# z-prize/2022-entries

Hardware: AMD Instinct MI355X
Metric: BLS12-377 G1 MSM point-scalar pairs/s (higher is better)
Workload: dtype u32

## Files before the change

### 2022-entries_amd/csrc/host_test_api.cpp

```cpp
#include <stdint.h>
#include <stdio.h>

static long g_check_failures = 0;
static char g_first_failure[256];
static void msm_check_fail(const char* file, int line, const char* cond) {
  if (g_check_failures++ == 0) snprintf(g_first_failure, sizeof g_first_failure, "%s:%d %s", file, line, cond);
}
#define MSM_CHECK(cond) do { if (!(cond)) msm_check_fail(__FILE__, __LINE__, #cond); } while (0)
#define MSM_CHECK_COL_BEGIN() unsigned __int128 chk_col_ = col
#define MSM_CHECK_COL_ADD(x) chk_col_ += (x)
#define MSM_CHECK_COL_END(col) MSM_CHECK(chk_col_ == (unsigned __int128)(col))

#include "host_curve.hpp"
#include "te.hpp"

using namespace msm;

template <class F>
static void t_fe_mul(const uint8_t* a, const uint8_t* b, uint8_t* out) {
  Modulus<F> md;
  Fe x, y, z;
  uint32_t wa[12], wb[12], wo[12];
  memcpy(wa, a, 48);
  memcpy(wb, b, 48);
// ... 2498 lines not shown
}
}

#include "expr.hpp"

template <class FR>
static int t_expr(unsigned flags, const uint32_t* nodes, uint64_t n_nodes, const uint8_t* consts, uint64_t n_consts, uint64_t n_chal, uint64_t n_cols,
                  const uint8_t* const* cols, const uint64_t* lens, uint64_t len, uint64_t rot_step, const uint8_t* challenges, uint8_t* out, uint64_t* info,
                  char* msg, uint64_t msg_len) {
  const bool normal = (flags & kExprNormal) != 0;
  ExprProgram pr;
  if (!expr_check_dag(nodes, n_nodes, n_consts, n_chal, n_cols, msg, msg_len)) return -1;
  const bool ok = expr_compile(pr, nodes, n_nodes, n_consts, n_chal, n_cols, expr_store_limit<FR>(), msg, msg_len);
  if (info) {
    info[0] = pr.n_nodes;
    info[1] = pr.ninstr();
    info[2] = pr.slots;
    info[3] = pr.products;
    info[4] = pr.reduces;
    info[5] = expr_lds_bytes(pr.slots);
    info[6] = pr.used_cols;
    info[7] = pr.rot0_only;
  }
  if (!ok) return -1;
  if (!out || len == 0) return 0;
  for (uint64_t j = 0; j < n_cols; j++)
    if (lens[j] == 0 || len % lens[j]) return -3;
  std::vector<uint32_t> cw(n_consts * 8 + 1), hw(n_chal * 8 + 1), dst(len * 8), slots((size_t)pr.slots * 8 + 1);
  std::vector<std::vector<uint32_t>> colw(n_cols);
  auto words = [&](uint32_t* w8, const uint8_t* b32) {
    Fr x;
    uint32_t w[8];
    poly_scalar<FR>(x, b32, normal);
    fr_pack(w, x);
    memcpy(w8, w, 32);
  };
  for (uint64_t k = 0; k < n_consts; k++) words(cw.data() + k * 8, consts + k * 32);
  for (uint64_t k = 0; k < n_chal; k++) words(hw.data() + k * 8, challenges + k * 32);
  for (uint64_t j = 0; j < n_cols; j++) {
    colw[j].resize(lens[j] * 8);
    memcpy(colw[j].data(), cols[j], lens[j] * 32);
  }
  std::vector<ExprColRef> refs(pr.refs.size() + 1);
  for (size_t k = 0; k < pr.refs.size(); k++)
    refs[k] = ExprColRef{colw[pr.refs[k].first].data(), (uint32_t)lens[pr.refs[k].first], expr_shift(pr.refs[k].second, rot_step, len)};
  ExprRun p{};
  p.prog = pr.code.data();
  p.refs = refs.data();
  p.consts = cw.data();
  p.chals = hw.data();
  p.out = dst.data();
  p.ninstr = pr.ninstr();
  p.len = (uint32_t)len;
  p.normal = normal ? 1u : 0u;
  const ExprSlots<1> st{slots.data()};
  for (uint64_t i = 0; i < len; i++) expr_row<FR>(st, p, (uint32_t)i);
  memcpy(out, dst.data(), len * 32);
  return 0;
}

extern "C" {
int ht_expr(int field, unsigned flags, const uint32_t* nodes, uint64_t n_nodes, const uint8_t* consts, uint64_t n_consts, uint64_t n_chal, uint64_t n_cols,
            const uint8_t* const* cols, const uint64_t* lens, uint64_t len, uint64_t rot_step, const uint8_t* challenges, uint8_t* out, uint64_t* info,
            char* msg, uint64_t msg_len) {
  if ((flags & ~kExprNormal) || !nodes || !msg || msg_len < 64 || len > ((uint64_t)1 << 22) || (n_consts && !consts)) return -2;
  if (out && len && ((n_cols && (!cols || !lens)) || (n_chal && !challenges))) return -2;
  msg[0] = 0;
  return POLY_FIELD(t_expr, flags, nodes, n_nodes, consts, n_consts, n_chal, n_cols, cols, lens, len, rot_step, challenges, out, info, msg, msg_len);
}
unsigned ht_expr_max_slots(void) { return EXPR_MAX_SLOTS; }
}

#include "seg_msm.hpp"

template <class C>
static int t_sm_segments(const uint8_t* points, size_t stride, const uint8_t* scalars, const uint64_t* offsets, size_t nseg, uint64_t shared_len, uint32_t c,
                         uint32_t tile, unsigned flags, uint8_t* out, size_t out_stride) {
  using E = typename C::E;
  using El = typename E::T;
  typename E::Md md;
  std::vector<XyzzDevT<El>> res(nseg);
  std::vector<uint32_t> sc;
  for (size_t s = 0; s < nseg; s++) {
    uint64_t p0, s0, len;
    sm_segment_span(p0, s0, len, offsets, s, shared_len, 0);
    if (len == 0) {
      xyzz_set_inf<E>(res[s].p);
      continue;
    }
    sc.resize(8 * len);
    memcpy(sc.data(), scalars + 32 * s0, 32 * len);
    sm_serial_segment<E>(res[s].p, points + p0 * stride, stride, sc.data(), len, c ? c : sm_window_for(len), tile, (flags & 1) != 0, md);
  }
  pm_host_output<E>(res, (flags & 8) ? 2u : 0u, out, out_stride, md);
  return 0;
}

extern "C" {
int ht_sm_digits(const uint8_t* scalar, int c, int32_t* out, int32_t* out_mem) {
  if (!scalar || !out || !out_mem || c < 1 || c > (int)SM_MAX_WINDOW) return -1;
  uint32_t s[8];
  memcpy(s, scalar, 32);
  const uint32_t nd = sm_digits((uint32_t)c);
  for (uint32_t j = 0; j < nd; j++) {
    out[j] = sm_digit(s, j, (uint32_t)c);
    out_mem[j] = sm_digit_mem(s, j, (uint32_t)c);
  }
  return (int)nd;
}
int ht_sm_segments(int curve, const uint8_t* points, size_t stride, const uint8_t* scalars, const uint64_t* offsets, size_t nseg, uint64_t shared_len, int c,
                   int tile, unsigned flags, uint8_t* out, size_t out_stride) {
  if ((flags & ~13u) || c < 0 || c > (int)SM_MAX_WINDOW || tile < (int)SM_MIN_TILE || (tile & (tile - 1)) || out_stride % 4 || (nseg && !out)) return -1;
  if (((flags & 4) != 0) != (offsets == nullptr)) return -1;
  DISPATCH_C(curve, t_sm_segments, points, stride, scalars, offsets, nseg, shared_len, (uint32_t)c, (uint32_t)tile, flags, out, out_stride)
}
long ht_sm_plan(const uint64_t* offsets, size_t nseg, uint64_t shared_len, int force_c, int tile_opt, size_t max_segs, size_t work_limit, size_t xyzz_bytes,
                size_t el_bytes, uint64_t* classes, size_t max_classes, uint32_t* ids, size_t max_ids, uint64_t* chunk_bounds, size_t max_chunks,
                uint64_t* summary) {
  if (force_c < 0 || force_c > (int)SM_MAX_WINDOW || !classes || !ids || !summary || !chunk_bounds) return -1;
  SmPlan plan;
  sm_plan(plan, offsets, nseg, shared_len, (uint32_t)force_c, (uint32_t)tile_opt, max_segs, work_limit, xyzz_bytes, el_bytes);
  if (!plan.fits) return -2;
  size_t nc = 0, ni = 0;
  if (plan.chunks.size() > max_chunks) return -1;
  for (size_t k = 0; k < plan.chunks.size(); k++) {
    const SmChunk& ch = plan.chunks[k];
    chunk_bounds[3 * k] = ch.s0;
    chunk_bounds[3 * k + 1] = ch.s1;
    chunk_bounds[3 * k + 2] = ch.work_bytes;
    if (ni + ch.ids.size() > max_ids) return -1;
    for (const SmClass& cl : ch.classes) {
      if (nc >= max_classes) return -1;
      const uint64_t row[11] = {k, ch.s0, ch.s1, cl.c, cl.nwin, cl.tile, cl.nseg, ni + cl.ids_at, cl.wsum_at, ch.work_bytes, ch.wsum_records};
      memcpy(classes + 11 * nc++, row, sizeof row);
    }
    if (!ch.ids.empty()) memcpy(ids + ni, ch.ids.data(), 4 * ch.ids.size());
    ni += ch.ids.size();
  }
  summary[0] = plan.chunks.size();
  summary[1] = plan.max_segs;
  summary[2] = plan.max_wsum_records;
  return (long)nc;
}
int ht_sm_geometry(int c, int tile_opt, uint64_t maxlen, int xyzz_words, uint32_t* out) {
  if (c < 1 || c > (int)SM_MAX_WINDOW || !out) return -1;
  out[0] = sm_slices((uint32_t)c);
  out[1] = sm_block_threads((uint32_t)c);
  out[3] = sm_tile_for((uint32_t)c, (uint32_t)tile_opt, maxlen);
  out[2] = sm_lds_words((uint32_t)c, out[3], (uint32_t)xyzz_words);
  return 0;
}
int ht_sm_window_for(uint64_t len) { return (int)sm_window_for(len); }
}
```

### 2022-entries_amd/csrc/launch.hpp

```cpp
#pragma once
#include <hip/hip_runtime.h>

#include "host_curve.hpp"
#include "msm_types.hpp"
#include "partition_plan.hpp"
#include "te.hpp"

namespace msm {

template <class E>
struct SwLaw;
template <class F>
struct TeLaw;
template <class F, int NB>
struct SwPairLaw;

template <class G>
struct LawMem;
template <class E>
struct LawMem<SwLaw<E>> {
  using MemT = typename E::T;
  using BaseDev = AffineDevT<MemT>;
};
template <class F>
struct LawMem<TeLaw<F>> {
  using MemT = Fe;
  using BaseDev = TeAffineDev;
};
template <class F, int NB>
struct LawMem<SwPairLaw<F, NB>> {
  using MemT = Fe2;
  using BaseDev = AffineDevT<Fe2>;
};

template <class G>
struct PairedForm {
  using L = G;
};
template <class F, int NB>
struct PairedForm<SwLaw<Fp2El<F, NB>>> {
  using L = SwPairLaw<F, NB>;
};

template <class G>
struct WalkLaunch {
  using El = typename LawMem<G>::MemT;
  using BaseDev = typename LawMem<G>::BaseDev;
  static hipError_t accumulate(const uint2* entries, const uint32_t* n_real, uint32_t K, const BaseDev* bases, SegOutT<El> out, uint32_t nlanes,
                               uint32_t* flags, hipStream_t st);
  static hipError_t sum_bases(const BaseDev* bases, const uint8_t* inf, uint32_t first, uint32_t n, uint32_t per_lane, SegOutT<El> out, uint32_t nlanes,
                              uint32_t* flags, hipStream_t st);
  static hipError_t segreduce(const XyzzDevT<El>* in_slots, const uint32_t* in_keys, uint32_t n_in, uint32_t K, SegOutT<El> out, uint32_t nlanes,
                              uint32_t quad_limit, uint32_t* flags, hipStream_t st);
  static hipError_t bucket_reduce(bool first, const XyzzDevT<El>* in_a, const XyzzDevT<El>* in_x, uint32_t n_per_win, uint32_t L, uint32_t chunks,
                                  uint32_t windows, uint32_t out_stride, XyzzDevT<El>* out_a, XyzzDevT<El>* out_x, uint32_t* flags, hipStream_t st,
                                  uint32_t run_win = 0xffffffffu);
  static hipError_t reduce_scan_step(const XyzzDevT<El>* in, const XyzzDevT<El>* in2, XyzzDevT<El>* out, uint32_t nb, uint32_t windows, uint32_t d,
                                     uint32_t mode, uint32_t quad_limit, uint32_t* flags, hipStream_t st);
  static hipError_t bucket_merge(XyzzDevT<El>* total, const XyzzDevT<El>* part, uint32_t n, uint32_t* flags, hipStream_t st);
};

template <class E>
struct Launch {
  using El = typename E::T;
  static hipError_t convert_bases(const uint8_t* in, size_t stride, uint32_t n, bool serialized, AffineDevT<El>* out, uint8_t* inf,
                                  hipStream_t st);
  static hipError_t pre_double(const AffineDevT<El>* in, const uint8_t* inf_in, uint32_t n, uint32_t c, XyzzDevT<El>* out, hipStream_t st);
  static hipError_t pre_normalize(const XyzzDevT<El>* in, uint32_t n, uint32_t J, El* prefix, AffineDevT<El>* out, uint8_t* inf_out,
                                  hipStream_t st);
  static hipError_t check_points(const uint8_t* in, size_t stride, uint32_t n, bool serialized, bool exact, uint8_t* status, hipStream_t st);
};

struct LaunchTe {
  static constexpr uint32_t kDefaultQuadLimit = 1u << 18;
  static hipError_t convert(const AffineDev* in, const uint8_t* inf, uint32_t n, uint32_t J, Fe* prefix, TeAffineDev* out, uint32_t* flags,
                            hipStream_t st);
};

struct PartLaunch {
  static int run(int scalar_field, int scalar_mode, const uint32_t* d_scalars, const uint8_t* d_inf, const PartPlan& p, const PartBuffers& b,
                 hipStream_t st, hipEvent_t mid, hipError_t& err);
  static hipError_t debug_finish(const PartPlan& p, const PartBuffers& b, const uint32_t* slot_keys, uint32_t nslots, hipStream_t st, char* what,
                                 size_t what_len, uint64_t* checks_done);
};

extern template struct Launch<Bls12_377_G1::E>;
extern template struct Launch<Bls12_381_G1::E>;
extern template struct Launch<Bls12_377_G2::E>;
extern template struct Launch<Bls12_381_G2::E>;

}
```

### 2022-entries_amd/csrc/launch_impl.hpp

```cpp
#pragma once
#include <type_traits>
#include "launch.hpp"
#include "msm_kernels.hpp"

namespace msm {

inline uint32_t launch_blocks(uint64_t n) { return (uint32_t)((n + 255) / 256); }

template <class E>
hipError_t Launch<E>::convert_bases(const uint8_t* in, size_t stride, uint32_t n, bool serialized, AffineDevT<El>* out, uint8_t* inf,
                                    hipStream_t st) {
  if (serialized)
    hipLaunchKernelGGL((k_convert_bases<E, true>), dim3(launch_blocks(n)), dim3(256), 0, st, in, stride, n, out, inf);
  else
    hipLaunchKernelGGL((k_convert_bases<E, false>), dim3(launch_blocks(n)), dim3(256), 0, st, in, stride, n, out, inf);
  return hipGetLastError();
}

template <class E>
hipError_t Launch<E>::pre_double(const AffineDevT<El>* in, const uint8_t* inf_in, uint32_t n, uint32_t c, XyzzDevT<El>* out, hipStream_t st) {
  hipLaunchKernelGGL((k_pre_double<E>), dim3(launch_blocks(n)), dim3(256), 0, st, in, inf_in, n, c, out);
  return hipGetLastError();
}

template <class E>
hipError_t Launch<E>::pre_normalize(const XyzzDevT<El>* in, uint32_t n, uint32_t J, El* prefix, AffineDevT<El>* out, uint8_t* inf_out,
                                    hipStream_t st) {
  hipLaunchKernelGGL((k_pre_normalize<E>), dim3(launch_blocks(((uint64_t)n + J - 1) / J)), dim3(256), 0, st, in, n, J, prefix, out, inf_out);
  return hipGetLastError();
}

template <class G>
struct QuadOf {
  using Q = void;
};
template <class E>
struct QuadOf<SwLaw<E>> {
  using Q = SwQuad<E>;
};
template <class F>
struct QuadOf<TeLaw<F>> {
  using Q = TeQuad<F>;
};
template <class G>
inline constexpr bool kHasQuad = !std::is_void_v<typename QuadOf<G>::Q>;

template <class G>
inline constexpr bool kIsSwLaw = false;
template <class E>
inline constexpr bool kIsSwLaw<SwLaw<E>> = true;

template <class G>
uint32_t walk_blocks(uint64_t walkers) {
  static_assert(std::is_same_v<typename LawMem<G>::MemT, typename G::MemT> && std::is_same_v<typename LawMem<G>::BaseDev, typename G::BaseDev>,
                "LawMem (launch.hpp) restates the law's memory types");
  return launch_blocks(G::LANES * walkers);
}

template <class G>
hipError_t WalkLaunch<G>::accumulate(const uint2* entries, const uint32_t* n_real, uint32_t K, const BaseDev* bases, SegOutT<El> out, uint32_t nlanes,
                                     uint32_t* flags, hipStream_t st) {
#ifndef MSM_GATHER
#define MSM_GATHER 2
#endif
  if constexpr (MSM_GATHER == 2 || !kIsSwLaw<G>)
    hipLaunchKernelGGL((k_accumulate_glds<G>), dim3(walk_blocks<G>(nlanes)), dim3(256), 0, st, entries, n_real, K, bases, out, nlanes, flags);
  else
    hipLaunchKernelGGL((k_accumulate<G>), dim3(walk_blocks<G>(nlanes)), dim3(256), 0, st, entries, n_real, K, bases, out, nlanes, flags);
  return hipGetLastError();
}

template <class G>
hipError_t WalkLaunch<G>::sum_bases(const BaseDev* bases, const uint8_t* inf, uint32_t first, uint32_t n, uint32_t per_lane, SegOutT<El> out,
                                    uint32_t nlanes, uint32_t* flags, hipStream_t st) {
  if constexpr (G::LANES != 1) {
    return hipErrorNotSupported;
  } else {
    hipLaunchKernelGGL((k_sum_bases<G>), dim3(walk_blocks<G>(nlanes)), dim3(256), 0, st, bases, inf, first, n, per_lane, out, nlanes, flags);
    return hipGetLastError();
  }
}

template <class G>
hipError_t WalkLaunch<G>::segreduce(const XyzzDevT<El>* in_slots, const uint32_t* in_keys, uint32_t n_in, uint32_t K, SegOutT<El> out, uint32_t nlanes,
                                    uint32_t quad_limit, uint32_t* flags, hipStream_t st) {
  if constexpr (kHasQuad<G>) {
    if (nlanes <= quad_limit) {
      hipLaunchKernelGGL((k_segreduce_quad<typename QuadOf<G>::Q>), dim3(launch_blocks(4ull * nlanes)), dim3(256), 0, st, in_slots, in_keys, n_in, K, out,
                         nlanes, flags);
      return hipGetLastError();
    }
  }
  hipLaunchKernelGGL((k_segreduce<G>), dim3(walk_blocks<G>(nlanes)), dim3(256), 0, st, in_slots, in_keys, n_in, K, out, nlanes, flags);
  return hipGetLastError();
}

template <class G>
hipError_t WalkLaunch<G>::bucket_reduce(bool first, const XyzzDevT<El>* in_a, const XyzzDevT<El>* in_x, uint32_t n_per_win, uint32_t L, uint32_t chunks,
                                        uint32_t windows, uint32_t out_stride, XyzzDevT<El>* out_a, XyzzDevT<El>* out_x, uint32_t* flags, hipStream_t st,
                                        uint32_t run_win) {
  dim3 grid(walk_blocks<G>((uint64_t)windows * chunks));
  if (first)
    hipLaunchKernelGGL((k_bucket_reduce<G, true>), grid, dim3(256), 0, st, in_a, in_x, n_per_win, L, chunks, windows, out_stride, out_a, out_x, flags, run_win);
  else
    hipLaunchKernelGGL((k_bucket_reduce<G, false>), grid, dim3(256), 0, st, in_a, in_x, n_per_win, L, chunks, windows, out_stride, out_a, out_x, flags, run_win);
  return hipGetLastError();
}

template <class G>
hipError_t WalkLaunch<G>::reduce_scan_step(const XyzzDevT<El>* in, const XyzzDevT<El>* in2, XyzzDevT<El>* out, uint32_t nb, uint32_t windows, uint32_t d,
                                           uint32_t mode, uint32_t quad_limit, uint32_t* flags, hipStream_t st) {
  const uint64_t threads = (uint64_t)windows * (mode == 1 ? d : nb);
  if constexpr (kHasQuad<G>) {
    if (threads <= quad_limit) {
      hipLaunchKernelGGL((k_reduce_scan_step_quad<typename QuadOf<G>::Q>), dim3(launch_blocks(4 * threads)), dim3(256), 0, st, in, in2, out, nb, windows, d,
                         mode, flags);
      return hipGetLastError();
    }
  }
  hipLaunchKernelGGL((k_reduce_scan_step<G>), dim3(walk_blocks<G>(threads)), dim3(256), 0, st, in, in2, out, nb, windows, d, mode, flags);
  return hipGetLastError();
}

template <class G>
hipError_t WalkLaunch<G>::bucket_merge(XyzzDevT<El>* total, const XyzzDevT<El>* part, uint32_t n, uint32_t* flags, hipStream_t st) {
  if constexpr (G::CARRY_IN) {
    return hipErrorNotSupported;
  } else {
    hipLaunchKernelGGL((k_bucket_merge<G>), dim3(walk_blocks<G>(n)), dim3(256), 0, st, total, part, n, flags);
    return hipGetLastError();
  }
}

#define MSM_INSTANTIATE_SW_LAUNCHERS(E)                                                                                                          \
  using A_ = AffineDevT<E::T>;                                                                                                                   \
  using X_ = XyzzDevT<E::T>;                                                                                                                     \
  using S_ = SegOutT<E::T>;                                                                                                                      \
  using W_ = WalkLaunch<SwLaw<E>>;                                                                                                               \
  template hipError_t Launch<E>::convert_bases(const uint8_t*, size_t, uint32_t, bool, A_*, uint8_t*, hipStream_t);                              \
  template hipError_t W_::accumulate(const uint2*, const uint32_t*, uint32_t, const A_*, S_, uint32_t, uint32_t*, hipStream_t);                  \
  template hipError_t W_::segreduce(const X_*, const uint32_t*, uint32_t, uint32_t, S_, uint32_t, uint32_t, uint32_t*, hipStream_t);             \
  template hipError_t Launch<E>::pre_double(const A_*, const uint8_t*, uint32_t, uint32_t, X_*, hipStream_t);                                    \
  template hipError_t Launch<E>::pre_normalize(const X_*, uint32_t, uint32_t, E::T*, A_*, uint8_t*, hipStream_t);                                \
  template hipError_t W_::bucket_reduce(bool, const X_*, const X_*, uint32_t, uint32_t, uint32_t, uint32_t, uint32_t, X_*, X_*, uint32_t*, hipStream_t, uint32_t); \
  template hipError_t W_::reduce_scan_step(const X_*, const X_*, X_*, uint32_t, uint32_t, uint32_t, uint32_t, uint32_t, uint32_t*, hipStream_t); \
  template hipError_t W_::bucket_merge(X_*, const X_*, uint32_t, uint32_t*, hipStream_t);                                                        \
  template hipError_t W_::sum_bases(const A_*, const uint8_t*, uint32_t, uint32_t, uint32_t, S_, uint32_t, uint32_t*, hipStream_t);

}
```

### 2022-entries_amd/csrc/msm_engine.hip

```cpp
#include <hip/hip_runtime.h>

#include <algorithm>
#include <cstdarg>
#include <cstdio>
#include <cstdlib>
#include <cstring>
#include <string.h>
#include <strings.h>

#include <dlfcn.h>

#include <chrono>
#include <condition_variable>
#include <deque>
#include <functional>
#include <memory>
#include <mutex>
#include <stdexcept>
#include <thread>
#include <type_traits>
#include <string>
#include <vector>

#include "../../include/mi355_msm.h"
// ... 116 lines not shown
      if (e == hipSuccess) {
        e = hipMemMap(g->va, g->mapped, 0, g->handle, 0);
        if (e == hipSuccess) {
          hipMemAccessDesc acc{};
          acc.location = prop.location;
          acc.flags = hipMemAccessFlagsProtReadWrite;
          e = hipMemSetAccess(g->va, g->mapped, &acc, 1);
          if (e != hipSuccess) (void)hipMemUnmap(g->va, g->mapped);
        }
        if (e != hipSuccess) (void)hipMemRelease(g->handle);
      }
      if (e != hipSuccess) (void)hipMemAddressFree(g->va, g->va_bytes);
    }
    if (e != hipSuccess) {
      delete g;
      return e;
    }
    guard = g;
    p = (char*)g->va + (g->mapped - used);
    return hipSuccess;
  }
  void reserve(size_t need) {
    if (need <= bytes) return;
    release();
    hipError_t e = guard_tail_mode() ? guarded_alloc(need) : hipMalloc(&p, need);
    if (e == hipErrorOutOfMemory) {
      (void)hipGetLastError();
      if (reclaim_idle_device_memory()) e = guard_tail_mode() ? guarded_alloc(need) : hipMalloc(&p, need);
    }
    if (e != hipSuccess) {
      p = nullptr;
      (void)hipGetLastError();
      char buf[256];
      snprintf(buf, sizeof buf, "hipMalloc of %zu MiB failed: %s", need >> 20, hipGetErrorString(e));
      throw HipFailure((int)e, buf);
    }
    bytes = need;
  }
  void release() {
    if (guard) {
      (void)hipMemUnmap(guard->va, guard->mapped);
      (void)hipMemRelease(guard->handle);
      delete guard;
      guard = nullptr;
    } else if (p) {
      (void)hipFree(p);
    }
    p = nullptr;
    bytes = 0;
  }
  template <class T>
  T* as() const { return reinterpret_cast<T*>(p); }
};

struct ScratchBuf : private DevBuf {
  using DevBuf::as;
  using DevBuf::bytes;
  using DevBuf::p;
  using DevBuf::reserve;
  ScratchBuf() = default;
  explicit ScratchBuf(hipStream_t st) : stream(st), in_flight(true) {}
  ScratchBuf(const ScratchBuf&) = delete;
  ScratchBuf& operator=(const ScratchBuf&) = delete;
  ~ScratchBuf() {
    if (!p) return;
    if (in_flight) (void)hipStreamSynchronize(stream);
    release();
  }
  DevBuf detach() {
    const DevBuf b = *this;
    p = nullptr;
    bytes = 0;
    guard = nullptr;
    return b;
  }

 private:
  hipStream_t stream = nullptr;
  bool in_flight = false;
};

inline uint32_t ceil_div(uint64_t a, uint64_t b) { return (uint32_t)((a + b - 1) / b); }
inline uint32_t ilog2_floor(uint64_t v) { uint32_t r = 0; while (v >>= 1) r++; return r; }

constexpr uint32_t kNoAnchor = 0xffffffffu;
void eff_windows(int scalar_bits, int c, double& plain, double& anchored) {
  const int full = scalar_bits / c, rem = scalar_bits - full * c;
  const double q = scalar_bits == 253 ? 0.857 : 0.552;
  const double top_clear = rem == 0 ? 1.0 : std::min(1.0, q * std::ldexp(1.0, 1 - rem));
  plain = full + (rem == 0 ? 1.0 - q : 1.0 - 0.5 * top_clear);
  anchored = full + (1.0 - top_clear);
}
uint32_t anchor_window(int c, int scalar_bits, bool always = false) {
  const int full = scalar_bits / c;
  if (full < 1) return kNoAnchor;
  double plain, anchored;
  eff_windows(scalar_bits, c, plain, anchored);
  return (always || (plain - anchored) >= 0.01 * plain) ? (uint32_t)(full - 1) : kNoAnchor;
}

bool anchor_wide_fits(uint32_t anchor, int c, int scalar_bits) {
  if (anchor == kNoAnchor) return false;
  return scalar_bits - (int)(anchor + 1) * c == 1 && (257 + c - 1) / c == (int)anchor + 2;
}
double wide_eff_windows(uint32_t anchor, int c) { return (double)(anchor + 1) * (1.0 - std::ldexp(1.0, -c)); }

int choose_window_bits(size_t n, int scalar_bits, bool shared_buckets, bool fold = false, int levels = 0, int anchor_min_c = 0, bool anchor_wide = false) {
  if (!shared_buckets && n > ((size_t)1 << 12)) {
    if (n < ((size_t)3 << 14)) return 8;
    if (n < ((size_t)3 << (scalar_bits > 253 ? 16 : 17))) return 11;
  }
  const int free_wins = shared_buckets ? (257 + choose_window_bits(n, scalar_bits, false, fold) - 1) / choose_window_bits(n, scalar_bits, false, fold) : 0;
  int best = 2;
  double best_cost = 1e300;
  for (int c = 2; c <= (shared_buckets ? 24 : 23); c++) {
    if (shared_buckets && c < 24 && (257 + c - 1) / c >= free_wins) continue;
    if (shared_buckets && c == 22) continue;
    const int bits = (fold && n >= ((size_t)1 << 25)) ? scalar_bits - 1 : scalar_bits;
    const int full = bits / c, rem = bits - full * c;
    double eff = full + (rem >= 2 ? 1.0 : (bits != scalar_bits && rem == 0 ? (scalar_bits == 253 ? 0.145 : 0.448) : 0.55));
    if (anchor_min_c > 0 && !fold && c >= anchor_min_c && anchor_window(c, scalar_bits) != kNoAnchor) {
      double plain;
      eff_windows(scalar_bits, c, plain, eff);
      if (anchor_wide && !shared_buckets && anchor_wide_fits(anchor_window(c, scalar_bits), c, scalar_bits)) eff = wide_eff_windows(anchor_window(c, scalar_bits), c);
    }
    const int wins = (257 + c - 1) / c;
    const double alloc = shared_buckets ? (double)(levels > 0 ? (wins + std::min(levels, wins) - 1) / std::min(levels, wins) : 1) : (double)wins;
    const double group = c >= 22 ? 0.06 : 0.0;
    const double cost = (eff + group * wins) * (double)n * 10.0 + alloc * (double)(1ull << (c - 1)) * 50.0;
    if (cost < best_cost) { best_cost = cost; best = c; }
  }
  return best;
}

struct TableShape {
  uint32_t c, levels, bsets;
};
TableShape table_shape(size_t n, int scalar_bits, long opt_window_bits, int want_levels) {
  TableShape t{};
  t.c = opt_window_bits ? (uint32_t)opt_window_bits : (uint32_t)choose_window_bits(n, scalar_bits, true, false, want_levels);
  const uint32_t all_windows = (257 + t.c - 1) / t.c;
  t.levels = want_levels > 0 ? std::min<uint32_t>((uint32_t)want_levels, all_windows) : all_windows;
  t.bsets = ceil_div(all_windows, t.levels);
  t.levels = ceil_div(all_windows, t.bsets);
  return t;
}

struct Plan {
  uint32_t c, windows, half, keybits;
  uint32_t bucket_windows;
  uint32_t levels;
  uint32_t anchor;
  bool wide;
  uint64_t entries;
  uint32_t K, nlanes;
  uint32_t segK;
  uint32_t logL0, logL;
  uint32_t T0;
  uint32_t L0;
  uint32_t scan_nb;
  bool reduce_scan;
  bool scan_direct;
};

}

#ifndef MSM_G2_PAIRED_DEFAULT
#define MSM_G2_PAIRED_DEFAULT 31
#endif
constexpr long kDefaultG2Paired = MSM_G2_PAIRED_DEFAULT;

struct RcclState;

struct mi355_msm_ctx {
  int curve = 0;
  int device = 0;
  hipStream_t own_stream = nullptr;
  hipStream_t copy_stream = nullptr;
  struct AsyncWorker* async = nullptr;
  hipEvent_t copy_ev[9] = {};
  size_t nbases = 0;
  DevBuf bases, inf;
  DevBuf stateless_raw[3];
  DevBuf scalars, entries[2], buckets, slots[2], slot_keys[2], red_a[2], red_x[2];
  DevBuf carry_buckets;
  std::vector<hipEvent_t> carry_ev;
  long opt_first_piece_div = 0;
  long opt_carry = 1;
  DevBuf part_matrix, part_partial, part_segs[2], part_subjobs, part_counts, part_totals;
  void* pinned = nullptr;
  size_t pinned_bytes = 0;
  hipEvent_t ev[8] = {};
  long opt_window_bits = 0, opt_lane_entries = 0, opt_max_chunk = 0, opt_seg_entries = 0, opt_scalars_montgomery = 0, opt_reduce_scan_log = 0;
  long opt_scalars_to_montgomery = 0;
  long opt_precompute = 0;
  long opt_table_levels = 0;
  long opt_validate_bases = 0;
  bool bases_validated = false;
  long opt_codec_chunk = 0;
  DevBuf codec_in, codec_out, codec_stat[2];
  long opt_mul_chunk = 0, opt_mul_window = 0;
  DevBuf pm_stage, pm_rec, pm_prefix, pm_inf;
  DevBuf pm_points, pm_scalars, pm_out;
  hipEvent_t pm_ev[2] = {nullptr, nullptr};
  uint64_t last_mul_us = 0, last_mul_device_us = 0;
  long opt_seg_window = 0, opt_seg_tile = 0, opt_seg_chunk = 0;
  DevBuf sg_wsum, sg_stage, sg_prefix, sg_ids, sg_offs;
  DevBuf sg_points, sg_scalars, sg_out;
  hipEvent_t sg_ev[2] = {nullptr, nullptr};
  uint64_t last_segments_us = 0, last_segments_device_us = 0;
  long opt_fft_points_chunk = 0;
  DevBuf gf_stage, gf_rec, gf_prefix, gf_inf;
  DevBuf gf_vec[2];
  DevBuf gf_points, gf_out;
  hipEvent_t gf_ev[2] = {nullptr, nullptr};
  uint64_t last_fft_points_us = 0, last_fft_points_device_us = 0;
  long opt_assume_subgroup = 0;
  long opt_anchor = 1;
  bool anchor_armed = false;
  struct AnchorSum {
    size_t n;
    int shift;
    std::vector<uint8_t> pt;
  };
  std::vector<AnchorSum> anchor_sums;
  uint64_t anchor_sums_computed = 0;
  float anchor_sum_ms = 0;
  uint32_t last_anchor = kNoAnchor;
  long opt_anchor_wide = 1;
  bool wide_suppress = false;
  bool wide_overflowed = false;
  bool wide_off = false;
  uint32_t wide_streak = 0;
  uint64_t wide_fallbacks = 0, wide_demotions = 0;
  bool last_wide = false;
  DevBuf wide_flag, wide_r;
  uint32_t* h_wide_flag = nullptr;
  long opt_reduce_log_chunk = 0, opt_reduce_log_chunk0 = 0;
  long opt_reduce_scan = -1;
  long opt_reduce_fill = 0;
  long opt_twisted_edwards = 1;
  DevBuf te_bases, flags;
  uint32_t* h_flags = nullptr;
  bool te_active = false;
  bool sw_level0_only = false;
  uint64_t te_fallbacks = 0;
  uint32_t te_fallback_streak = 0;
  uint64_t te_demotions = 0;
  uint64_t oom_backoffs = 0;
  uint64_t peer_stagings = 0;
  long opt_force_peer_staging = 0;
  uint32_t last_bucket_windows = 0, last_l1_bits = 0, last_l1_bins = 0, last_passes = 0;
  uint32_t last_reduce_path = 0, last_reduce_chunks = 0, last_reduce_row = 0;
  uint32_t auto_levels = 0;
  uint64_t debug_checks = 0;
  size_t chunk_cap = 0;
  size_t fitted_chunk = 0;
  bool fitted_tables = false;
  uint32_t fitted_c = 0;
  long opt_mem_limit = 0;
  long inject_alloc_failures = 0;
  uint32_t quad_limit = LaunchTe::kDefaultQuadLimit;
  long opt_g2_paired = kDefaultG2Paired;
  std::vector<mi355_msm_ctx*> shards;
  std::vector<size_t> shard_lo;
  long opt_combine = 0;
  RcclState* rccl = nullptr;
  uint64_t rccl_exchanges = 0;
  uint32_t pre_c = 0, pre_windows = 0;
  bool bases_serialized = false;
  float last_ms[MI355_T_COUNT] = {};
  uint64_t last_info[8] = {};

  int scalar_bits() const { return (curve == MI355_BLS12_381_G1 || curve == MI355_BLS12_381_G2) ? 255 : 253; }
  int anchor_min_c() const { return curve == MI355_BLS12_381_G1 ? 2 : 21; }
  bool anchor_wanted(size_t n_batch) const {
    return opt_anchor != 0 && opt_carry != 0 && opt_assume_subgroup == 0 && n_batch >= (opt_anchor == 2 ? (size_t)1 : (size_t)1 << 20);
  }
  bool wide_wanted() const { return opt_anchor_wide != 0 && !wide_off && !wide_suppress; }

  Plan plan(size_t n, bool use_tables = true, uint32_t force_c = 0) const {
    Plan p{};
    const bool tables = pre_c && use_tables;
    if (tables)
      p.c = pre_c;
    else if (force_c)
      p.c = force_c;
    else
      p.c = (opt_window_bits && !pre_c) ? (uint32_t)opt_window_bits
                                        : (uint32_t)choose_window_bits(n, scalar_bits(), false, opt_assume_subgroup != 0, 0, anchor_wanted(n) ? anchor_min_c() : 0, wide_wanted());
    p.anchor = anchor_armed ? anchor_window((int)p.c, scalar_bits(), opt_anchor == 2) : kNoAnchor;
    p.wide = wide_wanted() && !tables && anchor_wide_fits(p.anchor, (int)p.c, scalar_bits());
    p.windows = (257 + p.c - 1) / p.c;
    p.levels = tables ? std::min<uint32_t>(pre_windows, p.windows) : 1;
    p.bucket_windows = ceil_div(p.windows, p.levels);
    p.levels = ceil_div(p.windows, p.bucket_windows);
    p.half = 1u << (p.c - 1);
    p.keybits = ilog2_floor(p.bucket_windows * p.half) + 1;
    p.entries = (uint64_t)p.windows * n;
    const uint64_t k_auto = std::max<uint64_t>({p.entries >= (3u << 20) ? 24u : (p.entries < (1u << 18) ? 4u : 8u), p.entries >> 20, std::min<uint64_t>(64, p.entries >> 19)});
    uint32_t K = opt_lane_entries ? (uint32_t)opt_lane_entries : (uint32_t)std::min<uint64_t>(512, k_auto);
    if (!opt_lane_entries && !opt_assume_subgroup && K >= 64) {
      K = (K + 7) & ~7u;
      double plain, anchored;
      eff_windows(scalar_bits(), (int)p.c, plain, anchored);
      const bool anchor_expected = (anchor_armed || anchor_wanted(n)) && anchor_window((int)p.c, scalar_bits(), opt_anchor == 2) != kNoAnchor;
      const uint32_t a_expected = anchor_expected ? anchor_window((int)p.c, scalar_bits(), opt_anchor == 2) : kNoAnchor;
      const bool wide_expected = wide_wanted() && !tables && anchor_wide_fits(a_expected, (int)p.c, scalar_bits());
      const double adds = (wide_expected ? wide_eff_windows(a_expected, (int)p.c) : anchor_expected ? anchored : plain) * (double)n;
      const double per_group = ((curve == MI355_BLS12_377_G2 || curve == MI355_BLS12_381_G2) && (opt_g2_paired & 1) ? 128.0 : 256.0) * 256.0;
      auto fill = [&](long k) {
        const double g = adds / ((double)k * per_group);
        return g / std::ceil(g);
      };
      if (adds / ((double)K * per_group) >= 6.0) {
        long best = (long)K;
        double best_fill = fill(best);
        for (long step = 8; step <= 96 && best_fill < 0.985; step += 8)
          for (long k : {(long)K - step, (long)K + step})
            if (k >= 64 && fill(k) > best_fill + 0.004) {
              best = k;
              best_fill = fill(k);
            }
        K = (uint32_t)best;
      }
    }
    p.K = K >= 8 ? (K + 7) & ~7u : (K + 3) & ~3u;
    p.nlanes = ceil_div(p.entries, p.K);
    p.segK = opt_seg_entries >= 4 ? (uint32_t)opt_seg_entries : (p.entries < (2u << 20) ? 4 : 8);
    uint64_t nb = (uint64_t)p.bucket_windows * p.half;
    uint32_t l0 = nb > (1u << 18) ? ilog2_floor(nb >> 18) : 0;
    p.logL0 = std::min<uint32_t>(7, std::max<uint32_t>(2, l0));
    p.logL = 2;
    if (opt_reduce_log_chunk) p.logL0 = p.logL = (uint32_t)opt_reduce_log_chunk;
    if (opt_reduce_log_chunk0) p.logL0 = (uint32_t)opt_reduce_log_chunk0;
    p.logL0 = std::min<uint32_t>(p.logL0, p.c - 1 ? p.c - 1 : 1);
    p.reduce_scan = opt_reduce_scan != 0;
    const uint32_t scan_log = opt_reduce_scan_log ? (uint32_t)opt_reduce_scan_log : 12;
    p.scan_direct = p.reduce_scan && p.half <= (1u << scan_log);
    if (p.reduce_scan && !p.scan_direct) {
      const uint32_t need = ilog2_floor(p.half) - scan_log;
      if (need > 9 || (need > 8 && p.bucket_windows < 8))
        p.reduce_scan = false;
      else if (p.logL0 < need)
        p.logL0 = need;
    }
    p.L0 = 1u << p.logL0;
    p.T0 = ceil_div(p.half, p.L0);
    p.scan_nb = p.T0;
    if (p.reduce_scan && !p.scan_direct && !opt_reduce_log_chunk && !opt_reduce_log_chunk0) {
      const uint64_t kSimds = 1024;
      const uint64_t fill = opt_reduce_fill > 0 ? (uint64_t)opt_reduce_fill : 1;
      const uint64_t waves = ((uint64_t)p.bucket_windows * p.T0 + 63) / 64;
      if (waves < fill * kSimds && p.T0 >= 1024) {
        const uint32_t t_fit = (uint32_t)(fill * kSimds * 64 / p.bucket_windows);
        if (t_fit > p.T0 && t_fit < 2 * fill * p.T0) {
          const uint32_t L = ceil_div(p.half, t_fit);
          if (L >= 8 && L < p.L0) {
            p.L0 = L;
            p.T0 = ceil_div(p.half, L);
            while (p.scan_nb < p.T0) p.scan_nb *= 2;
          }
        }
      }
    }
    return p;
  }
};

namespace {

void ensure_device(mi355_msm_ctx* ctx) { HIP_OK(hipSetDevice(ctx->device)); }

uint32_t pmul_window(const mi355_msm_ctx* ctx);
size_t pmul_chunk(const mi355_msm_ctx* ctx);
size_t gfft_chunk(const mi355_msm_ctx* ctx);

int require_device() {
  int count = 0;
  hipError_t e = hipGetDeviceCount(&count);
  if (e != hipSuccess || count == 0) {
    (void)hipGetLastError();
    throw HipFailure((int)(e != hipSuccess ? e : hipErrorNoDevice), "mi355_msm: no HIP device visible (this library has no CPU fallback)");
  }
  return count;
}

hipStream_t create_copy_stream() {
  hipStream_t s = nullptr;
  int least = 0, greatest = 0;
  if (hipDeviceGetStreamPriorityRange(&least, &greatest) == hipSuccess && greatest < least &&
      hipStreamCreateWithPriority(&s, hipStreamNonBlocking, greatest) == hipSuccess)
    return s;
  (void)hipGetLastError();
  HIP_OK(hipStreamCreateWithFlags(&s, hipStreamNonBlocking));
  return s;
}

uint64_t work_bytes(const Plan& p, uint64_t el, bool carry = false) {
  const PartPlan pp = part_plan((uint32_t)(p.entries / p.windows), p.c, p.windows, p.levels, 0, 0);
  const PartScratchSizes ps = part_scratch_sizes(pp);
  return p.entries * 16 + ps.matrix + ps.partial + ps.segs_a + ps.segs_b + ps.subjob_first + ps.counts + ps.totals +
         (uint64_t)p.bucket_windows * p.half * 224 * el * (carry ? 2 : 1) + 2 * (2ull * p.nlanes) * (224 * el + 4) + (p.scan_direct ? (uint64_t)p.bucket_windows * p.half : 4ull * (p.bucket_windows + (p.wide ? 1 : 0)) * p.scan_nb) * 224 * el;
}

DevBuf* const* work_buffers(mi355_msm_ctx* ctx, size_t& count) {
  static thread_local DevBuf* bufs[24];
  DevBuf* list[] = {&ctx->entries[0], &ctx->entries[1], &ctx->part_matrix, &ctx->part_partial, &ctx->part_segs[0], &ctx->part_segs[1],
                    &ctx->part_subjobs, &ctx->part_counts, &ctx->part_totals, &ctx->buckets, &ctx->slots[0], &ctx->slots[1],
                    &ctx->slot_keys[0], &ctx->slot_keys[1], &ctx->red_a[0], &ctx->red_a[1], &ctx->red_x[0], &ctx->red_x[1], &ctx->carry_buckets};
  count = sizeof list / sizeof list[0];
  for (size_t i = 0; i < count; i++) bufs[i] = list[i];
  return bufs;
}

struct WorkBytes {
  size_t b[19] = {};
  void max_with(const WorkBytes& o) {
    for (int i = 0; i < 19; i++) b[i] = std::max(b[i], o.b[i]);
  }
};

WorkBytes chunk_work_bytes(const Plan& p, size_t n, bool use_tables, size_t xyzz, bool carry = false) {
  WorkBytes w;
  const PartPlan gp = part_plan((uint32_t)n, p.c, p.windows, use_tables ? p.levels : 1, 0, 0);
  const PartScratchSizes gs = part_scratch_sizes(gp);
  const size_t nbuckets = (size_t)p.bucket_windows * p.half, nslots0 = 2 * (size_t)p.nlanes;
  const size_t red0 = p.scan_direct ? nbuckets : (size_t)(p.bucket_windows + (p.wide ? 1 : 0)) * p.scan_nb;
  w.b[0] = w.b[1] = p.entries * 8 + 64;
  w.b[2] = gs.matrix;
  w.b[3] = gs.partial;
  w.b[4] = gs.segs_a;
  w.b[5] = gs.segs_b;
  w.b[6] = gs.subjob_first;
  w.b[7] = gs.counts;
  w.b[8] = gs.totals;
  w.b[9] = nbuckets * xyzz;
  w.b[10] = w.b[11] = nslots0 * xyzz;
  w.b[12] = w.b[13] = nslots0 * 4;
  w.b[14] = red0 * xyzz;
  w.b[15] = p.scan_direct ? 0 : red0 * xyzz;
  w.b[16] = w.b[17] = p.scan_direct ? 0 : red0 * xyzz;
  w.b[18] = carry ? nbuckets * xyzz : 0;
  return w;
}

void reserve_work(mi355_msm_ctx* ctx, const WorkBytes& w) {
  size_t nb = 0;
  DevBuf* const* wb = work_buffers(ctx, nb);
  for (size_t i = 0; i < nb; i++)
    if (w.b[i]) wb[i]->reserve(w.b[i]);
}

size_t fit_chunk(mi355_msm_ctx* ctx, size_t want, bool use_tables, uint32_t force_c = 0) {
  size_t free_b = 0, total_b = 0;
  HIP_OK(hipMemGetInfo(&free_b, &total_b));
  size_t held = 0, nb = 0;
  DevBuf* const* wb = work_buffers(ctx, nb);
  for (size_t i = 0; i < nb; i++) held += wb[i]->bytes;
  uint64_t avail = (uint64_t)free_b + held;
  if (ctx->opt_mem_limit > 0 && (uint64_t)ctx->opt_mem_limit < avail) avail = (uint64_t)ctx->opt_mem_limit;
  const uint64_t el = is_g2(ctx->curve) ? 2 : 1;
  size_t cn = want;
  while (cn > 1024) {
    const Plan p = ctx->plan(cn, use_tables, force_c);
    if (p.entries < (1ull << 32) && work_bytes(p, el, force_c != 0) + (work_bytes(p, el, force_c != 0) >> 5) <= avail) break;
    cn = (cn + 1) / 2;
  }
  return cn;
}

void release_work_buffers(mi355_msm_ctx* ctx, bool keep_carry = false) {
  ctx->fitted_chunk = 0;
  size_t nb = 0;
  DevBuf* const* wb = work_buffers(ctx, nb);
  for (size_t i = 0; i < nb; i++)
    if (!(keep_carry && (wb[i] == &ctx->carry_buckets || wb[i] == &ctx->buckets))) wb[i]->release();
}

size_t ctx_device_bytes(mi355_msm_ctx* ctx) {
  size_t nb = 0, total = 0;
  DevBuf* const* wb = work_buffers(ctx, nb);
  for (size_t i = 0; i < nb; i++) total += wb[i]->bytes;
  total += ctx->bases.bytes + ctx->inf.bytes + ctx->scalars.bytes;
  for (const DevBuf& r : ctx->stateless_raw) total += r.bytes;
  return total;
}

template <class Fn>
void with_curve(int curve, Fn&& fn) {
  switch (curve) {
    case MI355_BLS12_377_G1: fn.template operator()<Bls12_377_G1>(); break;
    case MI355_BLS12_381_G1: fn.template operator()<Bls12_381_G1>(); break;
    case MI355_BLS12_377_G2: fn.template operator()<Bls12_377_G2>(); break;
    case MI355_BLS12_381_G2: fn.template operator()<Bls12_381_G2>(); break;
    default: bad_arg("unknown curve id %d", curve);
  }
}
bool known_curve(int c) { return c >= MI355_BLS12_377_G1 && c <= MI355_BLS12_381_G2; }
size_t coord_bytes(int curve) { return is_g2(curve) ? 96 : 48; }

template <class C>
void convert_bases(mi355_msm_ctx* ctx, const uint8_t* d_raw, size_t n, size_t stride, hipStream_t st) {
  using E = typename C::E;
  using AD = AffineDevT<typename E::T>;
  ctx->bases.reserve(n * sizeof(AD));
  ctx->inf.reserve(n);
  HIP_OK(Launch<E>::convert_bases(d_raw, stride, (uint32_t)n, ctx->bases_serialized, ctx->bases.as<AD>(), ctx->inf.as<uint8_t>(), st));
}

template <class C>
void build_tables(mi355_msm_ctx* ctx, const uint8_t* d_raw, size_t n, size_t stride, int want_levels, hipStream_t st) {
  using E = typename C::E;
  using El = typename E::T;
  using AD = AffineDevT<El>;
  using XD = XyzzDevT<El>;
  if (ctx->opt_precompute == 2 && ctx->inject_alloc_failures > 0) {
    ctx->inject_alloc_failures--;
    throw HipFailure((int)hipErrorOutOfMemory, "table allocation failed: out of memory (injected by the inject_alloc_failures test hook)");
  }
  const TableShape ts = table_shape(n, C::SCALAR_BITS, ctx->opt_window_bits, want_levels);
  const uint32_t c = ts.c, windows = ts.levels , bsets = ts.bsets;
  const uint32_t level_shift = c * bsets;
  if ((uint64_t)windows * n >= (1ull << 31)) bad_arg("precompute: %u tables of %zu points exceed the 2^31 index range", windows, n);
  const size_t table_bytes = (size_t)windows * n * sizeof(AD);
  size_t free_b = 0, total_b = 0;
  HIP_OK(hipMemGetInfo(&free_b, &total_b));
  if (table_bytes + n * (sizeof(XD) + sizeof(El)) > free_b + ctx->bases.bytes)
    bad_arg("precompute: %u tables of %zu points need %zu MiB, only %zu MiB free", windows, n, table_bytes >> 20, free_b >> 20);
  ctx->bases.reserve(table_bytes);
  ctx->inf.reserve((size_t)windows * n);
  HIP_OK(Launch<E>::convert_bases(d_raw, stride, (uint32_t)n, ctx->bases_serialized, ctx->bases.as<AD>(), ctx->inf.as<uint8_t>(), st));
  ScratchBuf xyzz(st), prefix(st);
  xyzz.reserve(n * sizeof(XD));
  prefix.reserve(n * sizeof(El));
  const uint32_t J = 64;
  for (uint32_t w = 1; w < windows; w++) {
    AD* prev = ctx->bases.as<AD>() + (size_t)(w - 1) * n;
    AD* next = ctx->bases.as<AD>() + (size_t)w * n;
    uint8_t* inf_prev = ctx->inf.as<uint8_t>() + (size_t)(w - 1) * n;
    uint8_t* inf_next = ctx->inf.as<uint8_t>() + (size_t)w * n;
    HIP_OK(Launch<E>::pre_double(prev, inf_prev, (uint32_t)n, level_shift, xyzz.as<XD>(), st));
    HIP_OK(Launch<E>::pre_normalize(xyzz.as<XD>(), (uint32_t)n, J, prefix.as<El>(), next, inf_next, st));
  }
  HIP_OK(hipStreamSynchronize(st));
  ctx->pre_c = c;
  ctx->pre_windows = windows;
}

void build_te(mi355_msm_ctx* ctx, size_t n, hipStream_t st) {
  const size_t levels = ctx->pre_c ? ctx->pre_windows : 1;
  const size_t total = levels * n;
  size_t free_b = 0, total_b = 0;
  HIP_OK(hipMemGetInfo(&free_b, &total_b));
  const size_t need = total * sizeof(TeAffineDev) + n * sizeof(Fe) + ((size_t)1 << 30);
  if (need > free_b + ctx->te_bases.bytes) return;
  ctx->te_bases.reserve(total * sizeof(TeAffineDev));
  ctx->flags.reserve(2 * sizeof(uint32_t));
  if (!ctx->h_flags) HIP_OK(hipHostMalloc((void**)&ctx->h_flags, 2 * sizeof(uint32_t), hipHostMallocDefault));
  HIP_OK(hipMemsetAsync(ctx->flags.p, 0, 2 * sizeof(uint32_t), st));
  {
    ScratchBuf prefix(st);
    prefix.reserve(n * sizeof(Fe));
    for (size_t w = 0; w < levels; w++)
      HIP_OK(LaunchTe::convert(ctx->bases.as<AffineDev>() + w * n, ctx->inf.as<uint8_t>() + w * n, (uint32_t)n, 64, prefix.as<Fe>(),
                               ctx->te_bases.as<TeAffineDev>() + w * n, ctx->flags.as<uint32_t>(), st));
    HIP_OK(hipMemcpyAsync(ctx->h_flags, ctx->flags.p, 2 * sizeof(uint32_t), hipMemcpyDeviceToHost, st));
    HIP_OK(hipStreamSynchronize(st));
  }
  if (ctx->h_flags[0] != 0) {
    ctx->te_bases.release();
    return;
  }
  ctx->te_active = true;
  if (levels > 1) {
    ScratchBuf level0(st);
    level0.reserve(n * sizeof(AffineDev));
    HIP_OK(hipMemcpyAsync(level0.p, ctx->bases.p, n * sizeof(AffineDev), hipMemcpyDeviceToDevice, st));
    HIP_OK(hipStreamSynchronize(st));
    ctx->bases.release();
    ctx->bases = level0.detach();
    ctx->sw_level0_only = true;
  }
}

int precompute_auto_levels(mi355_msm_ctx* ctx, size_t n) {
  const bool mid = n < ((size_t)1 << 24);
  if (mid) {
    const size_t upper = is_g2(ctx->curve) ? ((size_t)3 << 20) : (is_381(ctx->curve) ? ((size_t)3 << 18) : ((size_t)3 << 19));
    if (n < ((size_t)1 << 18) || n >= upper) return -1;
  }
  size_t free_b = 0, total_b = 0;
  HIP_OK(hipMemGetInfo(&free_b, &total_b));
  size_t held = ctx->bases.bytes + ctx->te_bases.bytes + ctx->inf.bytes, nb = 0;
  DevBuf* const* wb = work_buffers(ctx, nb);
  for (size_t i = 0; i < nb; i++) held += wb[i]->bytes;
  uint64_t avail = (uint64_t)free_b + held;
  const uint64_t reserve = total_b / 10;
  avail = avail > reserve ? avail - reserve : 0;
  if (ctx->opt_mem_limit > 0 && (uint64_t)ctx->opt_mem_limit < avail) avail = (uint64_t)ctx->opt_mem_limit;
  const uint64_t el = is_g2(ctx->curve) ? 2 : 1;
  const bool te = ctx->curve == MI355_BLS12_377_G1 && ctx->opt_twisted_edwards;
  static const int kG1[] = {0, 6, 4, 3}, kG2[] = {0, 6}, kMid[] = {6};
  const int* cand = mid ? kMid : (el == 2 ? kG2 : kG1);
  const int ncand = mid ? 1 : (el == 2 ? 2 : 4);
  for (int ci = 0; ci < ncand; ci++) {
    const int want = cand[ci];
    const TableShape ts = table_shape(n, ctx->scalar_bits(), ctx->opt_window_bits, want);
    if (want > 0 && ts.levels > (uint32_t)want) continue;
    if ((uint64_t)ts.levels * n >= (1ull << 31) || ts.levels < 2) continue;
    const uint64_t sw = (uint64_t)ts.levels * n * 128 * el, inf = (uint64_t)ts.levels * n;
    const uint64_t te_b = te ? (uint64_t)ts.levels * n * sizeof(TeAffineDev) : 0;
    const uint64_t build = te ? 3 * n * 128 + te_b + n * (224 + 56) : sw + n * (224 + 56) * el;
    mi355_msm_ctx tmp;
    tmp.curve = ctx->curve;
    tmp.pre_c = ts.c;
    tmp.pre_windows = ts.levels;
    tmp.opt_window_bits = ctx->opt_window_bits;
    tmp.opt_assume_subgroup = ctx->opt_assume_subgroup;
    tmp.opt_anchor = ctx->opt_anchor;
    tmp.opt_anchor_wide = ctx->opt_anchor_wide;
    tmp.opt_carry = ctx->opt_carry;
    tmp.opt_lane_entries = ctx->opt_lane_entries;
    tmp.opt_seg_entries = ctx->opt_seg_entries;
    tmp.opt_reduce_scan = ctx->opt_reduce_scan;
    tmp.opt_reduce_fill = ctx->opt_reduce_fill;
    const Plan p = tmp.plan(std::min(n, (size_t)1 << 26));
    const uint64_t steady = (te ? n * 128 * el + te_b : sw) + inf + work_bytes(p, el) + n * 32;
    const uint64_t need = std::max(build + inf, steady);
    if (need + (need >> 4) <= avail) return want;
  }
  return -1;
}

bool build_tables_te_streamed(mi355_msm_ctx* ctx, const uint8_t* d_raw, size_t n, size_t stride, int want_levels, hipStream_t st) {
  using C = Bls12_377_G1;
  using E = C::E;
  if (ctx->opt_precompute == 2 && ctx->inject_alloc_failures > 0) {
    ctx->inject_alloc_failures--;
    throw HipFailure((int)hipErrorOutOfMemory, "table allocation failed: out of memory (injected by the inject_alloc_failures test hook)");
  }
  const TableShape ts = table_shape(n, C::SCALAR_BITS, ctx->opt_window_bits, want_levels);
  const uint32_t levels = ts.levels, level_shift = ts.c * ts.bsets;
  if ((uint64_t)levels * n >= (1ull << 31)) bad_arg("precompute: %u tables of %zu points exceed the 2^31 index range", levels, n);
  if (levels < 2) return false;
  const size_t need = (size_t)levels * n * sizeof(TeAffineDev) + 3 * n * sizeof(AffineDev) + n * (sizeof(XyzzDev) + sizeof(Fe)) + (size_t)levels * n;
  size_t free_b = 0, total_b = 0;
  HIP_OK(hipMemGetInfo(&free_b, &total_b));
  if (need > free_b + ctx->bases.bytes + ctx->te_bases.bytes + ctx->inf.bytes)
    bad_arg("precompute: %u table levels of %zu points need %zu MiB, only %zu MiB free", levels, n, need >> 20, free_b >> 20);
  bool ok = false;
  try {
    ScratchBuf xyzz(st), prefix(st), level0(st);
    ctx->te_bases.reserve((size_t)levels * n * sizeof(TeAffineDev));
    ctx->bases.reserve(3 * n * sizeof(AffineDev));
    ctx->inf.reserve((size_t)levels * n);
    ctx->flags.reserve(2 * sizeof(uint32_t));
    if (!ctx->h_flags) HIP_OK(hipHostMalloc((void**)&ctx->h_flags, 2 * sizeof(uint32_t), hipHostMallocDefault));
    HIP_OK(hipMemsetAsync(ctx->flags.p, 0, 2 * sizeof(uint32_t), st));
    xyzz.reserve(n * sizeof(XyzzDev));
    prefix.reserve(n * sizeof(Fe));
    AffineDev* const slots = ctx->bases.as<AffineDev>();
    uint8_t* const inf = ctx->inf.as<uint8_t>();
    auto slot_of = [&](uint32_t w) { return slots + (size_t)(w == 0 ? 0 : 1 + ((w - 1) & 1)) * n; };
    HIP_OK(Launch<E>::convert_bases(d_raw, stride, (uint32_t)n, ctx->bases_serialized, slot_of(0), inf, st));
    for (uint32_t w = 0; w < levels; w++) {
      if (w > 0) {
        HIP_OK(Launch<E>::pre_double(slot_of(w - 1), inf + (size_t)(w - 1) * n, (uint32_t)n, level_shift, xyzz.as<XyzzDev>(), st));
        HIP_OK(Launch<E>::pre_normalize(xyzz.as<XyzzDev>(), (uint32_t)n, 64, prefix.as<Fe>(), slot_of(w), inf + (size_t)w * n, st));
      }
      HIP_OK(LaunchTe::convert(slot_of(w), inf + (size_t)w * n, (uint32_t)n, 64, prefix.as<Fe>(), ctx->te_bases.as<TeAffineDev>() + (size_t)w * n,
                               ctx->flags.as<uint32_t>(), st));
    }
    HIP_OK(hipMemcpyAsync(ctx->h_flags, ctx->flags.p, 2 * sizeof(uint32_t), hipMemcpyDeviceToHost, st));
    HIP_OK(hipStreamSynchronize(st));
    ok = ctx->h_flags[0] == 0;
    if (ok) {
      level0.reserve(n * sizeof(AffineDev));
      HIP_OK(hipMemcpyAsync(level0.p, ctx->bases.p, n * sizeof(AffineDev), hipMemcpyDeviceToDevice, st));
      HIP_OK(hipStreamSynchronize(st));
      ctx->bases.release();
      ctx->bases = level0.detach();
    }
  } catch (...) {
    ctx->te_bases.release();
    throw;
  }
  if (!ok) {
    ctx->te_bases.release();
    return false;
  }
  ctx->pre_c = ts.c;
  ctx->pre_windows = levels;
  ctx->te_active = true;
  ctx->sw_level0_only = true;
  return true;
}

void anchor_prepare(mi355_msm_ctx* ctx, size_t n, hipStream_t st);

void set_bases_device(mi355_msm_ctx* ctx, const void* d_affine, size_t n, size_t stride) {
  ensure_device(ctx);
  const size_t min_stride = 2 * coord_bytes(ctx->curve) + (ctx->bases_serialized ? 0 : 1);
  if (stride < min_stride || (stride & 3)) bad_arg("affine stride %zu is not a 4-byte multiple >= %zu", stride, min_stride);
  if (n >= (1ull << 31)) bad_arg("npoints %zu exceeds 2^31-1", n);
  ctx->pre_c = ctx->pre_windows = 0;
  ctx->nbases = 0;
  ctx->anchor_sums.clear();
  ctx->fitted_chunk = 0;
  ctx->te_active = false;
  ctx->te_fallback_streak = 0;
  ctx->sw_level0_only = false;
  ctx->auto_levels = 0;
  ctx->bases.release();
  ctx->te_bases.release();
  ctx->inf.release();
  bool te_done = false;
  if (n) {
    bool tables = ctx->opt_precompute == 1;
    int want_levels = (int)ctx->opt_table_levels;
    if (ctx->opt_precompute == 2) {
      want_levels = precompute_auto_levels(ctx, n);
      tables = want_levels >= 0;
    }
    if (tables) {
      try {
        if (ctx->curve == MI355_BLS12_377_G1 && ctx->opt_twisted_edwards)
          te_done = build_tables_te_streamed(ctx, (const uint8_t*)d_affine, n, stride, want_levels, ctx->own_stream);
        if (!te_done)
          with_curve(ctx->curve, [&]<class C>() { build_tables<C>(ctx, (const uint8_t*)d_affine, n, stride, want_levels, ctx->own_stream); });
      } catch (const HipFailure& e) {
        if (ctx->opt_precompute != 2 || (e.code != (int)hipErrorOutOfMemory && e.code != -1)) throw;
        (void)hipGetLastError();
        ctx->pre_c = ctx->pre_windows = 0;
        ctx->bases.release();
        ctx->inf.release();
        tables = false;
      }
    }
    if (!tables)
      with_curve(ctx->curve, [&]<class C>() { convert_bases<C>(ctx, (const uint8_t*)d_affine, n, stride, ctx->own_stream); });
    if (ctx->opt_precompute == 2 && tables) ctx->auto_levels = ctx->pre_windows;
    HIP_OK(hipStreamSynchronize(ctx->own_stream));
    if (ctx->curve == MI355_BLS12_377_G1 && ctx->opt_twisted_edwards && !te_done) build_te(ctx, n, ctx->own_stream);
  }
  ctx->nbases = n;
  if (n) anchor_prepare(ctx, n, ctx->own_stream);
}

template <class F>
const Fp64& fp64_of() {
  static const Fp64 ctx = [] {
    Fp64 f{};
    f.init<F>();
    if constexpr (std::is_same_v<F, Bls12_377_Fq>) {
      f.const_from_device<F>(f.two_d, Bls12_377_Te::K2D);
      f.const_from_device<F>(f.sqrt3, Bls12_377_Te::SQRT3);
      f.const_from_device<F>(f.fsc_sqrt3, Bls12_377_Te::FSC_SQRT3);
    }
    return f;
  }();
  return ctx;
}

template <class F, int NB>
const Fp2_64<NB>& fp2_64_of() {
  static const Fp2_64<NB> ctx{&fp64_of<F>()};
  return ctx;
}

template <class E>
struct HostTail;
template <class F, int NB>
struct HostTail<Fp2El<F, NB>> {
  using Pt = XyzzG64<F2_64>;
  static void set_inf(Pt& a) { sw64_set_inf(a); }
  static void add(Pt& a, const Pt& b) { sw64_add(fp2_64_of<F, NB>(), a, b); }
  static void dbl(Pt& a) { sw64_dbl(fp2_64_of<F, NB>(), a); }
  static void fold(Pt& out, const XyzzT<Fe2>* sums, int windows, int c, int wide_a = -1) { fold_windows64<F>(fp2_64_of<F, NB>(), out, sums, windows, c, wide_a); }
  static void to_abi(uint8_t* out, const Pt& a) { sw64_to_abi(fp2_64_of<F, NB>(), out, a); }
};
template <class F>
struct HostTail<FpEl<F>> {
  using Pt = Xyzz64;
  static void set_inf(Pt& a) { sw64_set_inf(a); }
  static void add(Pt& a, const Pt& b) { sw64_add(fp64_of<F>(), a, b); }
  static void dbl(Pt& a) { sw64_dbl(fp64_of<F>(), a); }
  static void fold(Pt& out, const Xyzz* sums, int windows, int c, int wide_a = -1) { fold_windows64<F>(fp64_of<F>(), out, sums, windows, c, wide_a); }
  static bool fold_te(Pt& out, const Xyzz* sums, int windows, int c, int wide_a = -1) {
    if constexpr (std::is_same_v<F, Bls12_377_Fq>)
      return fold_windows_te64<F, TeFq>(fp64_of<F>(), out, sums, windows, c, wide_a);
    else
      return fold_windows_te64<F>(fp64_of<F>(), out, sums, windows, c, wide_a);
  }
  static void to_abi(uint8_t* out, const Pt& a) { sw64_to_abi(fp64_of<F>(), out, a); }
};

__global__ void __launch_bounds__(256) k_collect_sums(const uint4* __restrict__ src, uint32_t row_stride_u4, uint32_t row_u4, uint32_t rows,
                                                      uint4* __restrict__ dst_host, uint32_t* __restrict__ flags, uint32_t* __restrict__ flags_host,
                                                      const uint4* __restrict__ extra = nullptr, uint32_t* __restrict__ wide_flag = nullptr,
                                                      uint32_t* __restrict__ wide_flag_host = nullptr) {
  const uint32_t i = blockIdx.x * 256 + threadIdx.x;
  if (i < rows * row_u4) {
    const uint32_t r = i / row_u4, c = i - r * row_u4;
    dst_host[i] = src[(size_t)r * row_stride_u4 + c];
  } else if (extra && i < (rows + 1) * row_u4) {
    dst_host[i] = extra[i - rows * row_u4];
  }
  if (wide_flag && i == 0) {
    wide_flag_host[0] = wide_flag[0];
    wide_flag[0] = 0;
  }
  if (flags_host && i == 0) {
    flags_host[0] = flags[0];
    flags_host[1] = flags[1];
    flags[1] = 0;
  }
}

struct BucketCarry {
  uint32_t c;
  uint32_t index;
  bool first, last;
};

hipEvent_t* carry_events(mi355_msm_ctx* ctx, uint32_t index) {
  while (ctx->carry_ev.size() < 7 * ((size_t)index + 1)) {
    hipEvent_t e = nullptr;
    HIP_OK(hipEventCreate(&e));
    ctx->carry_ev.push_back(e);
  }
  return ctx->carry_ev.data() + 7 * (size_t)index;
}

template <class G>
inline constexpr bool kEdwards = false;
template <class F>
inline constexpr bool kEdwards<TeLaw<F>> = true;

template <class G>
const typename LawMem<G>::BaseDev* law_bases(const mi355_msm_ctx* ctx) {
  if constexpr (kEdwards<G>)
    return ctx->te_bases.as<TeAffineDev>();
  else
    return ctx->bases.as<typename LawMem<G>::BaseDev>();
}
template <class G>
uint32_t* law_flags(const mi355_msm_ctx* ctx) {
  return kEdwards<G> ? ctx->flags.as<uint32_t>() : nullptr;
}

template <class G, class Fn>
hipError_t walk_form(const mi355_msm_ctx* ctx, long bit, bool small, Fn&& launch) {
  using P = typename PairedForm<G>::L;
  if constexpr (!std::is_same_v<P, G>) {
    if ((ctx->opt_g2_paired & bit) != 0 && !small) return launch.template operator()<P>();
  }
  return launch.template operator()<G>();
}

void reserve_pinned(mi355_msm_ctx* ctx, size_t rows, size_t row_bytes) {
  const size_t need = std::max<size_t>(64, rows) * row_bytes;
  if (ctx->pinned_bytes >= need) return;
  if (ctx->pinned) (void)hipHostFree(ctx->pinned);
  ctx->pinned_bytes = need;
  HIP_OK(hipHostMalloc(&ctx->pinned, ctx->pinned_bytes, hipHostMallocDefault));
}

const uint2* group_chunk(mi355_msm_ctx* ctx, const uint32_t* d_scalars, const PartPlan& gp, PartBuffers& gb, hipStream_t st, hipEvent_t mid) {
  gb.entries[0] = ctx->entries[0].as<uint2>();
  gb.entries[1] = ctx->entries[1].as<uint2>();
  gb.matrix = ctx->part_matrix.as<uint32_t>();
  gb.partial = ctx->part_partial.as<uint32_t>();
  gb.segs[0] = ctx->part_segs[0].as<PartSeg>();
  gb.segs[1] = ctx->part_segs[1].as<PartSeg>();
  gb.subjob_first = ctx->part_subjobs.as<uint32_t>();
  gb.counts = ctx->part_counts.as<uint32_t>();
  gb.totals = ctx->part_totals.as<uint32_t>();
  hipError_t gerr = hipSuccess;
  const int scalar_mode = ctx->opt_scalars_montgomery ? SCALARS_FROM_MONT : ctx->opt_scalars_to_montgomery ? SCALARS_TO_MONT : SCALARS_PLAIN;
  const int sorted = PartLaunch::run(is_381(ctx->curve) ? 1 : 0, scalar_mode, d_scalars, ctx->inf.as<uint8_t>(), gp, gb, st, mid, gerr);
  HIP_OK(gerr);
  return gb.entries[sorted];
}

template <class G>
void merge_fragments(mi355_msm_ctx* ctx, uint32_t nlanes, uint32_t K, long paired_bit, hipStream_t st) {
  using XyzzDev = XyzzDevT<typename LawMem<G>::MemT>;
  uint32_t n_in = 2 * nlanes;
  for (int cur = 0;; cur ^= 1) {
    const uint32_t nl = ceil_div(n_in, K);
    if (nl > 1 && 2 * (uint64_t)nl >= n_in) bad_arg("fragment merge would not shrink (%u slots, fan-in %u)", n_in, K);
    SegOutT<typename LawMem<G>::MemT> o{ctx->buckets.as<XyzzDev>(), ctx->slots[cur ^ 1].as<XyzzDev>(), ctx->slot_keys[cur ^ 1].as<uint32_t>()};
    HIP_OK(walk_form<G>(ctx, paired_bit, nl <= ctx->quad_limit, [&]<class L>() {
      return WalkLaunch<L>::segreduce(ctx->slots[cur].as<XyzzDev>(), ctx->slot_keys[cur].as<uint32_t>(), n_in, K, o, nl, ctx->quad_limit, law_flags<G>(ctx), st);
    }));
    if (nl == 1) break;
    n_in = 2 * nl;
  }
}

template <class G>
XyzzDevT<typename LawMem<G>::MemT>* accumulate_chunk(mi355_msm_ctx* ctx, const Plan& p, const PartPlan& gp, const PartBuffers& gb, const uint2* entries,
                                                     const BucketCarry* carry, hipStream_t st, hipEvent_t* ev) {
  using El = typename LawMem<G>::MemT;
  using XyzzDev = XyzzDevT<El>;
  const size_t nbuckets = (size_t)p.bucket_windows * p.half;
  const bool carry_in = kEdwards<G> && carry && !carry->first;
  if (!carry_in) HIP_OK(hipMemsetAsync(ctx->buckets.p, 0, nbuckets * sizeof(XyzzDev), st));
  HIP_OK(hipEventRecord(ev[2], st));

  SegOutT<El> so{ctx->buckets.as<XyzzDev>(), ctx->slots[0].as<XyzzDev>(), ctx->slot_keys[0].as<uint32_t>()};
  so.carry_in = carry_in ? 1u : 0u;
  HIP_OK(walk_form<G>(ctx, 1, false, [&]<class L>() {
    return WalkLaunch<L>::accumulate(entries, gb.totals, p.K, law_bases<G>(ctx), so, p.nlanes, law_flags<G>(ctx), st);
  }));
  HIP_OK(hipEventRecord(ev[3], st));
#ifdef MSM_DEBUG
  {
    char what[320];
    HIP_OK(PartLaunch::debug_finish(gp, gb, ctx->slot_keys[0].as<uint32_t>(), 2 * p.nlanes, st, what, sizeof what, &ctx->debug_checks));
    if (what[0]) throw HipFailure(-2, what);
  }
#endif
  if (p.nlanes > 1) merge_fragments<G>(ctx, p.nlanes, p.segK, 4, st);
  if constexpr (!kEdwards<G>) {
    if (carry) {
      if (carry->first) {
        std::swap(ctx->buckets, ctx->carry_buckets);
      } else {
        HIP_OK(walk_form<G>(ctx, 16, false, [&]<class L>() {
          return WalkLaunch<L>::bucket_merge(ctx->carry_buckets.as<XyzzDev>(), ctx->buckets.as<XyzzDev>(), (uint32_t)nbuckets, law_flags<G>(ctx), st);
        }));
      }
      return ctx->carry_buckets.as<XyzzDev>();
    }
  }
  return ctx->buckets.as<XyzzDev>();
}

template <class G>
const XyzzDevT<typename LawMem<G>::MemT>* reduce_buckets(mi355_msm_ctx* ctx, const Plan& p, XyzzDevT<typename LawMem<G>::MemT>* bucket_src, hipStream_t st,
                                                         uint32_t& sums_stride, const XyzzDevT<typename LawMem<G>::MemT>*& r_src) {
  using XyzzDev = XyzzDevT<typename LawMem<G>::MemT>;
  uint32_t* const flags = law_flags<G>(ctx);
  r_src = nullptr;
  const uint32_t run_win = p.wide ? p.anchor + 1 : 0xffffffffu;
  const uint32_t rows = p.bucket_windows + (p.wide ? 1 : 0);
  auto bucket_reduce = [&](bool first, const XyzzDev* in_a, const XyzzDev* in_x, uint32_t n_per_win, uint32_t L, uint32_t chunks, uint32_t out_stride, int to) {
    HIP_OK(walk_form<G>(ctx, 2, false, [&]<class W>() {
      return WalkLaunch<W>::bucket_reduce(first, in_a, in_x, n_per_win, L, chunks, first ? p.bucket_windows : rows, out_stride, ctx->red_a[to].as<XyzzDev>(),
                                          ctx->red_x[to].as<XyzzDev>(), flags, st, first ? run_win : 0xffffffffu);
    }));
  };
  if (p.reduce_scan) {
    uint32_t nb = p.half;
    XyzzDev* bufs[2] = {bucket_src, ctx->red_a[0].as<XyzzDev>()};
    const XyzzDev* a_sums = nullptr;
    if (!p.scan_direct) {
      if (p.scan_nb != p.T0) {
        HIP_OK(hipMemsetAsync(ctx->red_a[0].p, 0, (size_t)rows * p.scan_nb * sizeof(XyzzDev), st));
        HIP_OK(hipMemsetAsync(ctx->red_x[0].p, 0, (size_t)rows * p.scan_nb * sizeof(XyzzDev), st));
      } else if (p.wide) {
        HIP_OK(hipMemsetAsync(ctx->red_x[0].as<XyzzDev>() + (size_t)p.bucket_windows * p.scan_nb, 0, (size_t)p.scan_nb * sizeof(XyzzDev), st));
      }
      bucket_reduce(true, nullptr, bucket_src, p.half, p.L0, p.T0, p.scan_nb, 0);
      nb = p.scan_nb;
      a_sums = ctx->red_a[0].as<XyzzDev>();
      bufs[0] = ctx->red_x[0].as<XyzzDev>();
      bufs[1] = ctx->red_x[1].as<XyzzDev>();
    }
    int cur = 0;
    const uint32_t scan_rows = a_sums ? rows : p.bucket_windows;
    auto step = [&](uint32_t d, uint32_t mode) {
      const bool small = (uint64_t)scan_rows * (mode == 1 ? d : nb) <= ctx->quad_limit;
      HIP_OK(walk_form<G>(ctx, 8, small, [&]<class W>() {
        return WalkLaunch<W>::reduce_scan_step(bufs[cur], a_sums, bufs[cur ^ 1], nb, scan_rows, d, mode, ctx->quad_limit, flags, st);
      }));
      cur ^= 1;
    };
    for (uint32_t d = 1; d < nb; d <<= 1) step(d, 0);
    if (a_sums) step(0, 2);
    if (p.wide && !a_sums) {
      ctx->wide_r.reserve(sizeof(XyzzDev));
      HIP_OK(hipMemcpyAsync(ctx->wide_r.p, bufs[cur] + (size_t)run_win * nb, sizeof(XyzzDev), hipMemcpyDeviceToDevice, st));
      r_src = ctx->wide_r.as<XyzzDev>();
    }
    if (nb & (nb - 1)) bad_arg("scan reduction needs a power-of-two element count per window (%u)", nb);
    for (uint32_t h = nb >> 1; h >= 1; h >>= 1) step(h, 1);
    if (nb == 1 && !a_sums) step(1, 0);
    sums_stride = nb;
    if (p.wide && a_sums) r_src = bufs[cur] + (size_t)p.bucket_windows * nb;
    return bufs[cur];
  }
  uint32_t n_per_win = p.half, logL = p.logL0, chunks = p.T0;
  int rb = 0;
  bucket_reduce(true, nullptr, bucket_src, n_per_win, 1u << logL, chunks, chunks, 0);
  if (p.wide && chunks > 1) HIP_OK(hipMemsetAsync(ctx->red_x[0].as<XyzzDev>() + (size_t)p.bucket_windows * chunks, 0, (size_t)chunks * sizeof(XyzzDev), st));
  while (chunks > 1) {
    n_per_win = chunks;
    logL = p.logL;
    chunks = ceil_div(n_per_win, 1u << logL);
    bucket_reduce(false, ctx->red_a[rb].as<XyzzDev>(), ctx->red_x[rb].as<XyzzDev>(), n_per_win, 1u << logL, chunks, chunks, rb ^ 1);
    rb ^= 1;
  }
  sums_stride = 1;
  if (p.wide) r_src = ctx->red_a[rb].as<XyzzDev>() + p.bucket_windows;
  return ctx->red_a[rb].as<XyzzDev>();
}

template <class G>
void collect_sums(mi355_msm_ctx* ctx, const XyzzDevT<typename LawMem<G>::MemT>* src, uint32_t stride, uint32_t rows, hipStream_t st,
                  const XyzzDevT<typename LawMem<G>::MemT>* r_src = nullptr) {
  using XyzzDev = XyzzDevT<typename LawMem<G>::MemT>;
  static_assert(sizeof(XyzzDev) % 16 == 0, "window sums are collected in 16-byte pieces");
  const uint32_t row_u4 = sizeof(XyzzDev) / 16, total = (rows + (r_src ? 1 : 0)) * row_u4;
  hipLaunchKernelGGL(k_collect_sums, dim3((total + 255) / 256), dim3(256), 0, st, reinterpret_cast<const uint4*>(src), stride * row_u4, row_u4, rows,
                     reinterpret_cast<uint4*>(ctx->pinned), law_flags<G>(ctx), kEdwards<G> ? ctx->h_flags : nullptr,
                     reinterpret_cast<const uint4*>(r_src), r_src ? ctx->wide_flag.as<uint32_t>() : nullptr, r_src ? ctx->h_wide_flag : nullptr);
  HIP_OK(hipGetLastError());
}

template <class C, class G>
bool fold_sums(mi355_msm_ctx* ctx, typename HostTail<typename C::E>::Pt& out, const XyzzT<typename C::E::T>* sums, int windows, int c, int wide_a = -1) {
  if constexpr (kEdwards<G>) {
    return ctx->h_flags[1] == 0 && HostTail<typename C::E>::fold_te(out, sums, windows, c, wide_a);
  } else {
    HostTail<typename C::E>::fold(out, sums, windows, c, wide_a);
    return true;
  }
}

template <class C, class G>
bool finish_chunk(mi355_msm_ctx* ctx, const Plan& p, const XyzzDevT<typename C::E::T>* sums_src, uint32_t sums_stride,
                  const XyzzDevT<typename C::E::T>* r_src, hipStream_t st, hipEvent_t* ev,
                  const BucketCarry* carry, const std::function<void()>* while_gpu_busy, typename HostTail<typename C::E>::Pt& out) {
  using XyzzDev = XyzzDevT<typename C::E::T>;
  collect_sums<G>(ctx, sums_src, sums_stride, p.bucket_windows, st, r_src);
  HIP_OK(hipEventRecord(ev[6], st));
  if (while_gpu_busy) (*while_gpu_busy)();
  if (p.entries < (1ull << 26)) {
    const auto t_spin = std::chrono::steady_clock::now();
    while (hipEventQuery(ev[6]) == hipErrorNotReady) {
      if (std::chrono::steady_clock::now() - t_spin > std::chrono::milliseconds(4)) break;
    }
    (void)hipGetLastError();
  }
  HIP_OK(hipStreamSynchronize(st));

  const uint32_t nsums = p.bucket_windows + (r_src ? 1 : 0);
  std::vector<XyzzT<typename C::E::T>> sums(nsums);
  const XyzzDev* hs = reinterpret_cast<const XyzzDev*>(ctx->pinned);
  for (uint32_t w = 0; w < nsums; w++) sums[w] = hs[w].p;
  const auto t_fold = std::chrono::steady_clock::now();
  ctx->wide_overflowed = r_src && ctx->h_wide_flag[0] != 0;
  const bool ok = !ctx->wide_overflowed && fold_sums<C, G>(ctx, out, sums.data(), (int)p.bucket_windows, (int)p.c, r_src ? (int)p.anchor : -1);
  ctx->last_ms[MI355_T_HOST_FOLD] += std::chrono::duration<float, std::milli>(std::chrono::steady_clock::now() - t_fold).count();

  for (uint32_t k = 0, nk = carry ? carry->index + 1 : 1; k < nk; k++) {
    hipEvent_t* const e = carry ? carry_events(ctx, k) : ctx->ev;
    float ms = 0;
    for (int s = 0; s < 5; s++) {
      HIP_OK(hipEventElapsedTime(&ms, e[s], e[s + 1]));
      ctx->last_ms[s] += ms;
    }
    HIP_OK(hipEventElapsedTime(&ms, e[0], e[6]));
    ctx->last_ms[MI355_T_TOTAL] += ms;
  }
  return ok;
}

template <class C, class G>
bool run_chunk_impl(mi355_msm_ctx* ctx, const uint32_t* d_scalars, size_t base0, size_t n, hipStream_t st,
                    typename HostTail<typename C::E>::Pt& out, const std::function<void()>* while_gpu_busy, const BucketCarry* carry = nullptr) {
  using XyzzDev = XyzzDevT<typename C::E::T>;
  static_assert(std::is_same_v<typename LawMem<G>::MemT, typename C::E::T>, "a law of this curve's coordinates");
  const bool use_tables = ctx->pre_c && (kEdwards<G> || !ctx->sw_level0_only);
  const Plan p = ctx->plan(n, use_tables, carry ? carry->c : 0);
  if (p.entries >= (1ull << 32)) bad_arg("chunk of %zu pairs needs %llu sort entries (>= 2^32)", n, (unsigned long long)p.entries);
  hipEvent_t* const ev = carry ? carry_events(ctx, carry->index) : ctx->ev;
  if (ctx->inject_alloc_failures != 0) {
    const bool fail = ctx->inject_alloc_failures > 0 ? (ctx->inject_alloc_failures--, true) : (++ctx->inject_alloc_failures == 0);
    if (fail) throw HipFailure((int)hipErrorOutOfMemory, "work-buffer reservation failed: out of memory (injected by the inject_alloc_failures test hook)");
  }
  reserve_work(ctx, chunk_work_bytes(p, n, use_tables, sizeof(XyzzDev), carry != nullptr));
  const uint32_t table_stride = use_tables ? (uint32_t)ctx->nbases : 0u;
  const PartPlan gp = part_plan((uint32_t)n, p.c, p.windows, use_tables ? p.levels : 1, (uint32_t)base0, table_stride, ctx->opt_assume_subgroup != 0, p.anchor, p.wide);
  if ((gp.wide != 0) != p.wide) throw HipFailure(-2, "mi355_msm: the plan and the grouping disagree about the wide anchored window (internal error)");
  ctx->last_anchor = gp.anchor;
  ctx->last_wide = p.wide;
  reserve_pinned(ctx, p.windows + 1, sizeof(XyzzDev));
  if (p.wide) {
    if (!ctx->h_wide_flag) {
      HIP_OK(hipHostMalloc((void**)&ctx->h_wide_flag, sizeof(uint32_t), hipHostMallocDefault));
      ctx->h_wide_flag[0] = 0;
    }
    ctx->wide_flag.reserve(sizeof(uint32_t));
    if (!carry || carry->first) HIP_OK(hipMemsetAsync(ctx->wide_flag.p, 0, sizeof(uint32_t), st));
  }

  HIP_OK(hipEventRecord(ev[0], st));
  PartBuffers gb{};
  gb.wide_flag = p.wide ? ctx->wide_flag.as<uint32_t>() : nullptr;
  const uint2* entries = group_chunk(ctx, d_scalars, gp, gb, st, ev[1]);
  XyzzDev* const bucket_src = accumulate_chunk<G>(ctx, p, gp, gb, entries, carry, st, ev);
  HIP_OK(hipEventRecord(ev[4], st));
  ctx->last_info[0] = p.c;
  ctx->last_info[1] = p.windows;
  ctx->last_info[6] = ctx->pre_c ? 1 : 0;
  ctx->last_info[2] = p.entries;
  ctx->last_info[3] = p.K;
  ctx->last_info[4] += 1;
  ctx->last_info[5] = p.nlanes;
  ctx->last_info[7] = kEdwards<G> ? 1 : 0;
  ctx->last_bucket_windows = p.bucket_windows;
  ctx->last_reduce_path = !p.reduce_scan ? 0 : p.scan_direct ? 1 : p.scan_nb == p.T0 ? 2 : 3;
  ctx->last_reduce_chunks = p.T0;
  ctx->last_reduce_row = p.scan_nb;
  ctx->last_l1_bits = gp.hb;
  ctx->last_l1_bins = gp.nbins;
  {
    uint32_t rb_[4];
    ctx->last_passes = (uint32_t)part_pass_bits(gp.lb, rb_);
  }
  if (carry && !carry->last) {
    HIP_OK(hipEventRecord(ev[5], st));
    HIP_OK(hipEventRecord(ev[6], st));
    if (while_gpu_busy) (*while_gpu_busy)();
    HostTail<typename C::E>::set_inf(out);
    return true;
  }
  uint32_t sums_stride = 1;
  const XyzzDev* r_src = nullptr;
  const XyzzDev* sums_src = reduce_buckets<G>(ctx, p, bucket_src, st, sums_stride, r_src);
  HIP_OK(hipEventRecord(ev[5], st));
  return finish_chunk<C, G>(ctx, p, sums_src, sums_stride, r_src, st, ev, carry, while_gpu_busy, out);
}

void te_fell_back(mi355_msm_ctx* ctx) {
  if (++ctx->te_fallback_streak >= 2) {
    ctx->te_active = false;
    ctx->te_demotions++;
    ctx->te_bases.release();
  }
}

void wide_fell_back(mi355_msm_ctx* ctx) {
  ctx->fitted_chunk = 0;
  if (++ctx->wide_streak >= 2) {
    ctx->wide_off = true;
    ctx->wide_demotions++;
  }
}

template <class C>
bool run_chunk_law(mi355_msm_ctx* ctx, const uint32_t* d_scalars, size_t base0, size_t n, hipStream_t st,
               typename HostTail<typename C::E>::Pt& out, const std::function<void()>* while_gpu_busy = nullptr,
               const BucketCarry* carry = nullptr, bool allow_te = true) {
  if constexpr (std::is_same_v<C, Bls12_377_G1>) {
    if (ctx->te_active && allow_te) {
      if (run_chunk_impl<C, TeLaw<TeFq>>(ctx, d_scalars, base0, n, st, out, while_gpu_busy, carry)) {
        if (!carry || carry->last) ctx->te_fallback_streak = 0;
        return true;
      }
      if (ctx->wide_overflowed) return false;
      ctx->te_fallbacks++;
      if (carry) return false;
      run_chunk_impl<C, SwLaw<typename C::E>>(ctx, d_scalars, base0, n, st, out, nullptr);
      te_fell_back(ctx);
      return true;
    }
  }
  return run_chunk_impl<C, SwLaw<typename C::E>>(ctx, d_scalars, base0, n, st, out, while_gpu_busy, carry) || !ctx->wide_overflowed;
}

template <class C>
bool run_chunk(mi355_msm_ctx* ctx, const uint32_t* d_scalars, size_t base0, size_t n, hipStream_t st,
               typename HostTail<typename C::E>::Pt& out, const std::function<void()>* while_gpu_busy = nullptr,
               const BucketCarry* carry = nullptr, bool allow_te = true) {
  ctx->wide_overflowed = false;
  const bool ok = run_chunk_law<C>(ctx, d_scalars, base0, n, st, out, while_gpu_busy, carry, allow_te);
  if (!ctx->wide_overflowed) {
    if (ok && ctx->last_wide && (!carry || carry->last)) ctx->wide_streak = 0;
    return ok;
  }
  ctx->wide_fallbacks++;
  if (carry) return false;
  struct Suppress {
    mi355_msm_ctx* c;
    ~Suppress() { c->wide_suppress = false; }
  } suppress{ctx};
  ctx->wide_suppress = true;
  ctx->wide_overflowed = false;
  run_chunk_law<C>(ctx, d_scalars, base0, n, st, out, nullptr, nullptr, allow_te);
  wide_fell_back(ctx);
  return true;
}

template <class C, class G>
bool sum_bases_impl(mi355_msm_ctx* ctx, size_t n, hipStream_t st, typename HostTail<typename C::E>::Pt& S) {
  using El = typename C::E::T;
  using XyzzDev = XyzzDevT<El>;
  constexpr uint32_t kSegK = 8;
  const uint32_t kPerLane = (uint32_t)std::min<size_t>(512, std::max<size_t>(32, n >> 17));
  const uint32_t nlanes = ceil_div(n, kPerLane);
  ctx->buckets.reserve(sizeof(XyzzDev));
  for (int k = 0; k < 2; k++) {
    ctx->slots[k].reserve(2 * (size_t)nlanes * sizeof(XyzzDev));
    ctx->slot_keys[k].reserve(2 * (size_t)nlanes * sizeof(uint32_t));
  }
  reserve_pinned(ctx, 1, sizeof(XyzzDev));
  HIP_OK(hipMemsetAsync(ctx->buckets.p, 0, sizeof(XyzzDev), st));
  SegOutT<El> so{ctx->buckets.as<XyzzDev>(), ctx->slots[0].as<XyzzDev>(), ctx->slot_keys[0].as<uint32_t>()};
  HIP_OK(WalkLaunch<G>::sum_bases(law_bases<G>(ctx), ctx->inf.as<uint8_t>(), 0, (uint32_t)n, kPerLane, so, nlanes, law_flags<G>(ctx), st));
  merge_fragments<G>(ctx, nlanes, kSegK, 0, st);
  collect_sums<G>(ctx, ctx->buckets.as<XyzzDev>(), 1, 1, st);
  HIP_OK(hipStreamSynchronize(st));
  const XyzzDev* hs = reinterpret_cast<const XyzzDev*>(ctx->pinned);
  bool empty = true;
  for (size_t k = 0; k < sizeof(XyzzDev); k++) empty = empty && reinterpret_cast<const uint8_t*>(hs)[k] == 0;
  if (empty) {
    HostTail<typename C::E>::set_inf(S);
    return !kEdwards<G> || ctx->h_flags[1] == 0;
  }
  const XyzzT<El> sum = hs[0].p;
  return fold_sums<C, G>(ctx, S, &sum, 1, 1);
}

template <class C>
void anchor_sum_of_bases(mi355_msm_ctx* ctx, size_t n, hipStream_t st, typename HostTail<typename C::E>::Pt& S) {
  using E = typename C::E;
  using Pt = typename HostTail<E>::Pt;
  static_assert(std::is_trivially_copyable_v<Pt>, "cached as bytes");
  for (const auto& a : ctx->anchor_sums)
    if (a.n == n && a.shift < 0) {
      memcpy(&S, a.pt.data(), sizeof S);
      return;
    }
  const auto t0 = std::chrono::steady_clock::now();
  bool done = false;
  if constexpr (std::is_same_v<C, Bls12_377_G1>) {
    if (ctx->te_active) done = sum_bases_impl<C, TeLaw<TeFq>>(ctx, n, st, S);
  }
  if (!done) sum_bases_impl<C, SwLaw<typename C::E>>(ctx, n, st, S);
  if (ctx->anchor_sums.size() >= 12) ctx->anchor_sums.erase(ctx->anchor_sums.begin(), ctx->anchor_sums.begin() + 4);
  mi355_msm_ctx::AnchorSum a{n, -1, std::vector<uint8_t>(sizeof S)};
  memcpy(a.pt.data(), &S, sizeof S);
  ctx->anchor_sums.push_back(std::move(a));
  ctx->anchor_sums_computed++;
  ctx->anchor_sum_ms = std::chrono::duration<float, std::milli>(std::chrono::steady_clock::now() - t0).count();
}

template <class C>
bool anchor_ready(mi355_msm_ctx* ctx, size_t n, hipStream_t st, typename HostTail<typename C::E>::Pt& S) {
  if (!ctx->anchor_wanted(n)) return false;
  const bool tables0 = ctx->pre_c && (ctx->te_active || !ctx->sw_level0_only);
// ... 697 lines not shown
    if (!ctx->shards.empty()) return sharded_set_bases(ctx, d_affine, npoints, stride, false, true);
    ensure_device(ctx);
    HIP_OK(hipDeviceSynchronize());
    validate_new_bases(ctx, d_affine, npoints, stride, false, true);
    ctx->bases_validated = false;
    set_bases_device(ctx, d_affine, npoints, stride);
    ctx->bases_validated = ctx->opt_validate_bases != 0;
  });
}

RustError mi355_msm_check_bases(mi355_msm_ctx* ctx, const void* affine, size_t npoints, size_t stride, unsigned flags, uint8_t* status, uint64_t* out) {
  return guarded_dev([&] { check_bases_impl(ctx, affine, npoints, stride, flags, status, out, false); });
}

RustError mi355_msm_check_bases_device(mi355_msm_ctx* ctx, const void* d_affine, size_t npoints, size_t stride, unsigned flags, uint8_t* status,
                                       uint64_t* out) {
  return guarded_dev([&] {
    if (ctx && ctx->shards.empty() && npoints) {
      ensure_device(ctx);
      HIP_OK(hipDeviceSynchronize());
    }
    check_bases_impl(ctx, d_affine, npoints, stride, flags, status, out, true);
  });
}

RustError mi355_msm_run(mi355_msm_ctx* ctx, void* out, const void* scalars, size_t npoints, size_t batches) {
  return guarded_dev([&] {
    if (!ctx) bad_arg("null context");
    if (npoints * batches && !scalars) bad_arg("null scalars pointer");
    if (!ctx->shards.empty()) return sharded_run(ctx, out, scalars, npoints, batches, false, nullptr);
    run_host(ctx, out, scalars, npoints, batches, npoints);
  });
}

RustError mi355_msm_run_device(mi355_msm_ctx* ctx, void* out, const void* d_scalars, size_t npoints, size_t batches,
                               void* stream) {
  return guarded_dev([&] {
    if (!ctx) bad_arg("null context");
    if (npoints * batches && !d_scalars) bad_arg("null scalars pointer");
    if (!ctx->shards.empty()) return sharded_run(ctx, out, d_scalars, npoints, batches, true, (hipStream_t)stream);
    run_device(ctx, out, d_scalars, npoints, batches, npoints, (hipStream_t)stream);
  });
}

RustError mi355_msm_set_option(mi355_msm_ctx* ctx, const char* key, long value) {
  return guarded([&] {
    if (!ctx || !key) bad_arg("null argument");
    std::string k(key);
    if (k == "force_peer_staging") {
      ctx->opt_force_peer_staging = value != 0;
      return;
    }
    if (!ctx->shards.empty() && k == "validate_bases" && value != 0)
      bad_arg("validate_bases is not available on a sharded context (MI355_MSM_VALIDATE_BASES with several MI355_MSM_DEVICES): check the bases "
              "on a single-device context with mi355_msm_check_bases");
    if (!ctx->shards.empty() && k != "combine") {
      for (mi355_msm_ctx* sh : ctx->shards) {
        RustError e = mi355_msm_set_option(sh, key, value);
        if (e.code) {
          std::string m = e.message ? e.message : "";
          free(e.message);
          throw HipFailure(e.code, m);
        }
      }
      return;
    }
    ctx->fitted_chunk = 0;
    if (k == "window_bits") {
      if (value != 0 && (value < 2 || value > 24)) bad_arg("window_bits %ld out of range [2, 24]", value);
      if (ctx->pre_c && value != 0 && (uint32_t)value != ctx->pre_c)
        bad_arg("window_bits is fixed at %u by the precomputed tables of this context", ctx->pre_c);
      ctx->opt_window_bits = value;
    } else if (k == "lane_entries") {
      if (value < 0 || value > (1 << 20)) bad_arg("lane_entries %ld out of range", value);
      ctx->opt_lane_entries = value;
    } else if (k == "max_chunk") {
      if (value < 0 || value > (1L << 27)) bad_arg("max_chunk %ld out of range [1, 2^27]", value);
      ctx->opt_max_chunk = value;
    } else if (k == "seg_entries") {
      if (value != 0 && (value < 4 || value > 4096)) bad_arg("seg_entries %ld out of range [4, 4096]", value);
      ctx->opt_seg_entries = value;
    } else if (k == "reduce_log_chunk") {
      if (value < 0 || value > 7) bad_arg("reduce_log_chunk %ld out of range [1, 7]", value);
      ctx->opt_reduce_log_chunk = value;
    } else if (k == "reduce_scan_log") {
      if (value != 0 && (value < 6 || value > 18)) bad_arg("reduce_scan_log %ld out of range [6, 18]", value);
      ctx->opt_reduce_scan_log = value;
    } else if (k == "quad_limit") {
      if (value < 0 || value > (1L << 24)) bad_arg("quad_limit %ld out of range [0, 2^24]", value);
      ctx->quad_limit = (uint32_t)value;
    } else if (k == "g2_paired") {
      if (value < 0 || value > 31) bad_arg("g2_paired %ld out of range [0, 31]", value);
      ctx->opt_g2_paired = value;
    } else if (k == "reduce_scan") {
      if (value < -1 || value > 1) bad_arg("reduce_scan %ld out of range [-1, 1]", value);
      ctx->opt_reduce_scan = value;
    } else if (k == "reduce_fill") {
      if (value < 0 || value > 4) bad_arg("reduce_fill %ld out of range [0, 4]", value);
      ctx->opt_reduce_fill = value;
    } else if (k == "reduce_log_chunk0") {
      if (value < 0 || value > 7) bad_arg("reduce_log_chunk0 %ld out of range [1, 7]", value);
      ctx->opt_reduce_log_chunk0 = value;
    } else if (k == "twisted_edwards") {
      ctx->opt_twisted_edwards = value != 0;
    } else if (k == "precompute") {
      if (value < 0 || value > 2) bad_arg("precompute %ld out of range [0, 2]", value);
      ctx->opt_precompute = value;
    } else if (k == "table_levels") {
      if (value < 0 || value > 64) bad_arg("table_levels %ld out of range [0, 64]", value);
      ctx->opt_table_levels = value;
    } else if (k == "scalars_montgomery") {
      if (value != 0 && ctx->opt_scalars_to_montgomery) bad_arg("scalars_montgomery and scalars_to_montgomery exclude each other");
      ctx->opt_scalars_montgomery = value != 0;
    } else if (k == "scalars_to_montgomery") {
      if (value != 0 && ctx->opt_scalars_montgomery) bad_arg("scalars_to_montgomery and scalars_montgomery exclude each other");
      ctx->opt_scalars_to_montgomery = value != 0;
    } else if (k == "validate_bases") {
      ctx->opt_validate_bases = value != 0;
    } else if (k == "codec_chunk") {
      if (value < 0 || value >= (1l << 31)) bad_arg("codec_chunk %ld out of range [0, 2^31)", value);
      ctx->opt_codec_chunk = value;
    } else if (k == "mul_chunk") {
      if (value < 0 || value >= (1l << 31)) bad_arg("mul_chunk %ld out of range [0, 2^31)", value);
      ctx->opt_mul_chunk = value;
    } else if (k == "mul_window") {
      if (value < 0 || value > 6) bad_arg("mul_window %ld out of range [1, 6] (0 = the default)", value);
      ctx->opt_mul_window = value;
    } else if (k == "seg_window") {
      if (value < 0 || value > (long)SM_MAX_WINDOW) bad_arg("seg_window %ld out of range [1, %u] (0 = by length)", value, SM_MAX_WINDOW);
      ctx->opt_seg_window = value;
    } else if (k == "seg_tile") {
      if (value != 0 && (value < (long)SM_MIN_TILE || value > (long)SM_MAX_TILE || (value & (value - 1))))
        bad_arg("seg_tile %ld is not a power of two in [%u, %u] (0 = the default)", value, SM_MIN_TILE, SM_MAX_TILE);
      ctx->opt_seg_tile = value;
    } else if (k == "seg_chunk") {
      if (value < 0 || value >= (1l << 31)) bad_arg("seg_chunk %ld out of range [0, 2^31)", value);
      ctx->opt_seg_chunk = value;
    } else if (k == "fft_points_chunk") {
      if (value < 0 || value >= (1l << 31)) bad_arg("fft_points_chunk %ld out of range [0, 2^31)", value);
      ctx->opt_fft_points_chunk = value;
    } else if (k == "assume_subgroup") {
      ctx->opt_assume_subgroup = value != 0;
    } else if (k == "carry") {
      ctx->opt_carry = value != 0;
    } else if (k == "anchor") {
      if (value < 0 || value > 2) bad_arg("anchor %ld out of range [0, 2]", value);
      ctx->opt_anchor = value;
    } else if (k == "anchor_wide") {
      if (value < 0 || value > 1) bad_arg("anchor_wide %ld out of range [0, 1]", value);
      ctx->opt_anchor_wide = value;
      ctx->wide_off = false;
      ctx->wide_streak = 0;
      ctx->fitted_chunk = 0;
    } else if (k == "first_piece_div") {
      if (value != 0 && (value < 2 || value > 64)) bad_arg("first_piece_div %ld out of range [2, 64]", value);
      ctx->opt_first_piece_div = value;
    } else if (k == "combine") {
      if (value < 0 || value > 2) bad_arg("combine %ld out of range [0, 2]", value);
      ctx->opt_combine = value;
    } else if (k == "mem_limit") {
      if (value < 0) bad_arg("mem_limit must be >= 0");
      ctx->opt_mem_limit = value;
      ctx->chunk_cap = 0;
    } else if (k == "inject_alloc_failures") {
      ctx->inject_alloc_failures = value;
    } else {
      bad_arg("unknown option '%s'", key);
    }
  });
}

RustError mi355_msm_last_timings(mi355_msm_ctx* ctx, float* ms, uint64_t* info) {
  return guarded([&] {
    if (!ctx) bad_arg("null context");
    if (!ctx->shards.empty()) {
      memset(ctx->last_ms, 0, sizeof ctx->last_ms);
      for (mi355_msm_ctx* sh : ctx->shards)
        for (int i = 0; i < MI355_T_COUNT; i++) ctx->last_ms[i] = std::max(ctx->last_ms[i], sh->last_ms[i]);
      memcpy(ctx->last_info, ctx->shards[0]->last_info, sizeof ctx->last_info);
    }
    if (ms) memcpy(ms, ctx->last_ms, sizeof ctx->last_ms);
    if (info) memcpy(info, ctx->last_info, sizeof ctx->last_info);
  });
}

RustError mi355_msm_shard_timings(mi355_msm_ctx* ctx, int shard, float* ms, uint64_t* info) {
  return guarded([&] {
    if (!ctx) bad_arg("null context");
    if (ctx->shards.empty()) {
      if (shard != 0) bad_arg("shard %d of an unsharded context", shard);
      if (ms) memcpy(ms, ctx->last_ms, sizeof ctx->last_ms);
      if (info) memcpy(info, ctx->last_info, sizeof ctx->last_info);
      return;
    }
    if (shard < 0 || (size_t)shard >= ctx->shards.size()) bad_arg("shard %d of %zu", shard, ctx->shards.size());
    const mi355_msm_ctx* sh = ctx->shards[(size_t)shard];
    if (ms) memcpy(ms, sh->last_ms, sizeof sh->last_ms);
    if (info) memcpy(info, sh->last_info, sizeof sh->last_info);
  });
}

RustError mi355_msm_query(mi355_msm_ctx* ctx, const char* key, uint64_t* value) {
  return guarded([&] {
    if (!ctx || !key || !value) bad_arg("null argument");
    std::string k(key);
    if (k == "shards") {
      *value = ctx->shards.size();
      return;
    }
    if (k == "rccl_exchanges") {
      *value = ctx->rccl_exchanges;
      return;
    }
    if (k == "peer_stagings") {
      *value = ctx->peer_stagings;
      return;
    }
    if (k == "async_pending") {
      uint64_t v = 0;
      if (ctx->async) {
        std::lock_guard<std::mutex> lk(ctx->async->mu);
        v = ctx->async->submitted - ctx->async->completed;
      }
      *value = v;
      return;
    }
    if (!ctx->shards.empty()) {
      uint64_t sum = 0, all = 1;
      for (mi355_msm_ctx* sh : ctx->shards) {
        uint64_t v = 0;
        RustError e = mi355_msm_query(sh, key, &v);
        if (e.code) {
          std::string m = e.message ? e.message : "";
          free(e.message);
          throw HipFailure(e.code, m);
        }
        sum += v;
        all &= (v != 0);
      }
      static const char* const kAll[] = {"twisted_edwards", "assume_subgroup", "carry"};
      static const char* const kMean[] = {"table_levels", "table_window_bits"};
      static const char* const kFirst[] = {"precompute", "g2_paired", "guard_tail", "te_limb_bits", "anchor", "anchor_wide"};
      static const char* const kMax[] = {"bucket_windows", "l1_bits", "l1_bins", "group_passes", "anchored_window", "anchor_sum_us", "anchor_wide_active",
                                          "reduce_path", "reduce_chunks", "reduce_row"};
      auto in = [&](const char* const* set, size_t n) {
        for (size_t i = 0; i < n; i++)
          if (k == set[i]) return true;
        return false;
      };
      if (in(kAll, 3)) {
        *value = all;
      } else if (in(kMean, 2)) {
        *value = sum / ctx->shards.size();
      } else if (in(kFirst, 6) || in(kMax, 10)) {
        uint64_t first = 0, mx = 0;
        for (size_t g = 0; g < ctx->shards.size(); g++) {
          uint64_t v = 0;
          RustError e = mi355_msm_query(ctx->shards[g], key, &v);
          if (e.code) {
            std::string m = e.message ? e.message : "";
            free(e.message);
            throw HipFailure(e.code, m);
          }
          if (g == 0) first = v;
          mx = std::max(mx, v);
        }
        *value = in(kFirst, 6) ? first : mx;
      } else {
        *value = sum;
      }
      return;
    }
    if (k == "twisted_edwards")
      *value = ctx->te_active ? 1 : 0;
    else if (k == "twisted_edwards_fallbacks")
      *value = ctx->te_fallbacks;
    else if (k == "twisted_edwards_demotions")
      *value = ctx->te_demotions;
    else if (k == "assume_subgroup")
      *value = ctx->opt_assume_subgroup ? 1 : 0;
    else if (k == "validate_bases")
      *value = ctx->opt_validate_bases ? 1 : 0;
    else if (k == "codec_chunk")
      *value = ctx->opt_codec_chunk > 0 ? (uint64_t)ctx->opt_codec_chunk : (uint64_t)1 << 22;
    else if (k == "mul_window")
      *value = pmul_window(ctx);
    else if (k == "mul_chunk")
      *value = pmul_chunk(ctx);
    else if (k == "mul_work_bytes")
      *value = ctx->pm_stage.bytes + ctx->pm_rec.bytes + ctx->pm_prefix.bytes + ctx->pm_inf.bytes + ctx->pm_points.bytes + ctx->pm_scalars.bytes + ctx->pm_out.bytes;
    else if (k == "seg_window")
      *value = (uint64_t)ctx->opt_seg_window;
    else if (k == "seg_tile")
      *value = ctx->opt_seg_tile > 0 ? (uint64_t)ctx->opt_seg_tile : SM_DEFAULT_TILE;
    else if (k == "seg_chunk")
      *value = (uint64_t)ctx->opt_seg_chunk;
    else if (k == "seg_work_bytes")
      *value = ctx->sg_wsum.bytes + ctx->sg_stage.bytes + ctx->sg_prefix.bytes + ctx->sg_ids.bytes + ctx->sg_offs.bytes + ctx->sg_points.bytes +
               ctx->sg_scalars.bytes + ctx->sg_out.bytes;
    else if (k == "last_segments_us")
      *value = ctx->last_segments_us;
    else if (k == "last_segments_device_us")
      *value = ctx->last_segments_device_us;
    else if (k == "fft_points_chunk")
      *value = gfft_chunk(ctx);
    else if (k == "fft_points_work_bytes")
      *value = ctx->gf_stage.bytes + ctx->gf_rec.bytes + ctx->gf_prefix.bytes + ctx->gf_inf.bytes + ctx->gf_vec[0].bytes + ctx->gf_vec[1].bytes +
               ctx->gf_points.bytes + ctx->gf_out.bytes;
    else if (k == "last_fft_points_us")
      *value = ctx->last_fft_points_us;
    else if (k == "last_fft_points_device_us")
      *value = ctx->last_fft_points_device_us;
    else if (k == "last_mul_us")
      *value = ctx->last_mul_us;
    else if (k == "last_mul_device_us")
      *value = ctx->last_mul_device_us;
    else if (k == "bases_validated")
      *value = ctx->bases_validated ? 1 : 0;
    else if (k == "carry")
      *value = ctx->opt_carry ? 1 : 0;
    else if (k == "anchor")
      *value = (uint64_t)ctx->opt_anchor;
    else if (k == "anchor_wide")
      *value = (ctx->opt_anchor_wide && !ctx->wide_off) ? 1 : 0;
    else if (k == "anchor_wide_active")
      *value = ctx->last_wide ? 1 : 0;
    else if (k == "anchor_wide_fallbacks")
      *value = ctx->wide_fallbacks;
    else if (k == "anchor_wide_demotions")
      *value = ctx->wide_demotions;
    else if (k == "anchored_window")
      *value = ctx->last_anchor == kNoAnchor ? 0 : (uint64_t)ctx->last_anchor + 1;
    else if (k == "sorted_entries") {
      uint32_t v = 0;
      if (ctx->part_totals.p) {
        ensure_device(ctx);
        HIP_OK(hipDeviceSynchronize());
        HIP_OK(hipMemcpy(&v, ctx->part_totals.p, sizeof v, hipMemcpyDeviceToHost));
      }
      *value = v;
    } else if (k == "anchor_sums")
      *value = ctx->anchor_sums_computed;
    else if (k == "anchor_sum_us")
      *value = (uint64_t)(ctx->anchor_sum_ms * 1000.0f);
    else if (k == "oom_backoffs")
      *value = ctx->oom_backoffs;
    else if (k == "debug_checks")
      *value = ctx->debug_checks;
    else if (k == "chunk_cap")
      *value = ctx->chunk_cap;
    else if (k == "device")
      *value = (uint64_t)ctx->device;
    else if (k == "bases")
      *value = ctx->nbases;
    else if (k == "table_levels")
      *value = ctx->pre_c ? ctx->pre_windows : (ctx->nbases ? 1 : 0);
    else if (k == "table_window_bits")
      *value = ctx->pre_c;
    else if (k == "base_bytes")
      *value = ctx->bases.bytes + ctx->te_bases.bytes + ctx->inf.bytes;
    else if (k == "bucket_windows")
      *value = ctx->last_bucket_windows;
    else if (k == "reduce_path")
      *value = ctx->last_reduce_path;
    else if (k == "reduce_chunks")
      *value = ctx->last_reduce_chunks;
    else if (k == "reduce_row")
      *value = ctx->last_reduce_row;
    else if (k == "l1_bits")
      *value = ctx->last_l1_bits;
    else if (k == "l1_bins")
      *value = ctx->last_l1_bins;
    else if (k == "group_passes")
      *value = ctx->last_passes;
    else if (k == "precompute")
      *value = (uint64_t)ctx->opt_precompute;
    else if (k == "g2_paired")
      *value = (uint64_t)ctx->opt_g2_paired;
    else if (k == "guard_tail")
      *value = guard_tail_mode() ? 1 : 0;
    else if (k == "te_limb_bits")
      *value = (uint64_t)TeFq::B;
    else
      bad_arg("unknown query '%s'", key);
  });
}

RustError mi355_msm(int curve, void* out, const void* affine, size_t npoints, const void* scalars, size_t ffi_affine_sz) {
  return guarded_dev([&] {
    if (!known_curve(curve)) bad_arg("unknown curve id %d", curve);
    if (!out) bad_arg("null output pointer");
    (void)require_device();
    std::vector<int> devs{-1};
    const char* env = getenv("MI355_MSM_DEVICES");
    if (env && *env) {
      try {
        devs = parse_device_list(env);
      } catch (const std::exception& e) {
        throw HipFailure(-1, e.what());
      }
    }
    const size_t G = devs.size(), pb = 3 * coord_bytes(curve);
    const char* sub_env = getenv("MI355_MSM_ASSUME_SUBGROUP");
    const long assume_sub = (sub_env && *sub_env && atol(sub_env) != 0) ? 1 : 0;
    if (G == 1) {
      StatelessLease ws(curve, devs[0]);
      take(mi355_msm_set_option(ws.ctx, "assume_subgroup", assume_sub));
      stateless_run(ws.ctx, out, affine, npoints, scalars, ffi_affine_sz);
      ws.keep();
      return;
    }
    std::vector<uint8_t> partials(G * pb);
    std::vector<std::string> errors(G);
    std::vector<int> codes(G, 0);
    std::vector<StatelessStats> stats(G);
    std::vector<std::thread> threads;
    for (size_t g = 0; g < G; g++)
      threads.emplace_back([&, g] {
        try {
          size_t lo, hi;
          shard_bounds(npoints, G, g, lo, hi);
          StatelessLease ws(curve, devs[g]);
          take(mi355_msm_set_option(ws.ctx, "assume_subgroup", assume_sub));
          stateless_run(ws.ctx, partials.data() + g * pb, (const uint8_t*)affine + lo * ffi_affine_sz, hi - lo, (const uint8_t*)scalars + lo * 32,
                        ffi_affine_sz);
          ws.keep();
          stats[g] = g_last_stateless;
        } catch (const HipFailure& e) {
          codes[g] = e.code ? e.code : -1;
          errors[g] = e.what();
        } catch (const std::exception& e) {
          codes[g] = -1;
          errors[g] = e.what();
        }
      });
    for (auto& t : threads) t.join();
    for (size_t g = 0; g < G; g++)
      if (codes[g]) throw HipFailure(codes[g], "shard " + std::to_string(g) + " (device " + std::to_string(devs[g]) + "): " + errors[g]);
    take(mi355_msm_fold(curve, out, partials.data(), G));
    g_last_stateless = *std::max_element(stats.begin(), stats.end(), [](const StatelessStats& a, const StatelessStats& b) { return a.total_ms < b.total_ms; });
  });
}

RustError mi355_msm_last_stateless(double* out, size_t count) {
  return guarded([&] {
    if (!out) bad_arg("null output");
    const StatelessStats& s = g_last_stateless;
    const double v[10] = {s.total_ms, s.setup_ms, s.wait_upload_ms, s.compute_ms, s.tail_ms, s.slices, s.threads, s.bytes, s.dma_done_ms, s.first_dma_ms};
    for (size_t i = 0; i < count && i < 10; i++) out[i] = v[i];
  });
}

RustError mi355_msm_trim(void) {
  return guarded_dev([&] {
    std::vector<StageRing*> rings;
    {
      std::lock_guard<std::mutex> lk(g_ring_mu);
      rings.swap(g_rings_idle);
    }
    for (StageRing* r : rings) {
      (void)hipSetDevice(r->device);
      ring_destroy(r);
    }
    (void)reclaim_idle_device_memory();
  });
}

RustError mi355_msm_pool_stats(uint64_t* out, size_t count) {
  return guarded([&] {
    if (!out) bad_arg("null output");
    uint64_t v[4] = {0, 0, 0, 0};
    {
      std::lock_guard<std::mutex> lk(g_ring_mu);
      v[0] = g_stateless_idle.size();
      for (mi355_msm_ctx* c : g_stateless_idle) v[1] += ctx_device_bytes(c);
      v[2] = g_rings_idle.size();
      v[3] = v[2] * StageRing::SLOTS * StageRing::PIECE;
    }
    for (size_t i = 0; i < count && i < 4; i++) out[i] = v[i];
// ... 101 lines not shown
```

### 2022-entries_amd/csrc/msm_kernels.hpp

```cpp
#pragma once
#include "curve.hpp"
#include "laws.hpp"
#include "msm_types.hpp"

namespace msm {

template <class E, bool SERIALIZED>
__global__ void __launch_bounds__(256) k_convert_bases(const uint8_t* __restrict__ in, size_t stride, uint32_t n,
                                                       AffineDevT<typename E::T>* __restrict__ out, uint8_t* __restrict__ inf) {
  uint32_t i = blockIdx.x * 256 + threadIdx.x;
  if (i >= n) return;
  typename E::Md md;
  constexpr int W = E::WORDS;
  const uint32_t* src = reinterpret_cast<const uint32_t*>(in + (size_t)i * stride);
  uint32_t w[2 * W];
#pragma unroll
  for (int k = 0; k < 2 * W; k++) w[k] = src[k];
  uint8_t flag;
  if (SERIALIZED) {
    flag = (w[2 * W - 1] >> 30) & 1;
    w[2 * W - 1] &= 0x3fffffffu;
  } else {
    flag = in[(size_t)i * stride + 8 * W];
  }
  AffineDevT<typename E::T> o;
  if (flag) {
    E::zero(o.p.x);
    E::zero(o.p.y);
  } else if (SERIALIZED) {
    E::from_plain(o.p.x, w, md);
    E::from_plain(o.p.y, w + W, md);
    E::reduce(o.p.x);
    E::reduce(o.p.y);
  } else {
    E::from_abi(o.p.x, w, md);
    E::from_abi(o.p.y, w + W, md);
    E::reduce(o.p.x);
    E::reduce(o.p.y);
  }
  out[i] = o;
  inf[i] = flag ? 1 : 0;
}

template <class G>
__device__ __forceinline__ void seg_flush(const SegOutT<typename G::MemT>& o, uint32_t t, uint32_t nlanes, uint32_t key,
                                          const XyzzT<typename G::T>& acc, bool is_first, bool is_last, uint32_t half = 0) {
  const bool complete = (!is_first || t == 0) && (!is_last || t == nlanes - 1);
  if (complete) {
    G::store_pt(o.buckets + key, acc, half);
  } else {
    const size_t s = 2 * (size_t)t + (is_first ? 0 : 1);
    G::store_pt(o.slots + s, acc, half);
    o.slot_keys[s] = key;
  }
}

template <class G>
__device__ __forceinline__ void carry_begin_run(const SegOutT<typename G::MemT>& o, uint32_t key, XyzzT<typename G::T>& acc, bool& fresh, uint32_t half) {
  acc = G::load_pt(o.buckets + key, half);
  fresh = G::nothing(acc);
  if (fresh) G::begin_run(acc);
}

template <class G>
__global__ void __launch_bounds__(256, G::ACC_WAVES) k_accumulate(const uint2* __restrict__ entries, const uint32_t* __restrict__ n_real,
                                                    uint32_t K, const typename G::BaseDev* __restrict__ bases,
                                                    SegOutT<typename G::T> out, uint32_t nlanes, uint32_t* __restrict__ flags) {
  using E = typename G::E;
  static_assert(G::LANES == 1, "the one-lane-per-record walk has no paired form");
  const uint32_t t = blockIdx.x * 256 + threadIdx.x;
  if (t >= nlanes) return;
  typename E::Md md;
  out.slot_keys[2 * (size_t)t] = KEY_NONE;
  out.slot_keys[2 * (size_t)t + 1] = KEY_NONE;
  const uint32_t n_entries = *n_real;
  const uint64_t beg64 = (uint64_t)t * K;
  if (beg64 >= n_entries) return;
  const uint32_t beg = (uint32_t)beg64;
  const uint32_t end = (n_entries - beg > K) ? beg + K : n_entries;

  uint2 ent_c = entries[beg], ent_n = make_uint2(0, KEY_NONE);
  if (end - beg > 1) ent_n = entries[beg + 1];
  typename G::Base p_c;
  if (G::PREFETCH_BASE) p_c = G::from_dev(bases[ent_c.x & IDX_MASK]);

  uint32_t cur = KEY_NONE;
  bool first = true, fresh = true, bad = false;
  XyzzT<typename G::T> acc;
  G::set_identity(acc);
  for (uint32_t e = beg; e < end; e++) {
    const uint32_t key = ent_c.y, val = ent_c.x;
    if (!G::PREFETCH_BASE) p_c = G::from_dev(bases[val & IDX_MASK]);
    const typename G::Base p = p_c;
    ent_c = ent_n;
    if (G::PREFETCH_BASE && end - e > 1) p_c = G::from_dev(bases[ent_c.x & IDX_MASK]);
    if (end - e > 2) ent_n = entries[e + 2];
    if (key != cur) {
      if (cur != KEY_NONE) {
        seg_flush<G>(out, t, nlanes, cur, acc, first, false);
        first = false;
      }
      cur = key;
      fresh = true;
      G::begin_run(acc);
    }
    G::madd(acc, p, (val >> 31) != 0, fresh, md);
    if (G::CHECKS) bad |= G::failed(acc);
    fresh = false;
  }
  if (cur != KEY_NONE) seg_flush<G>(out, t, nlanes, cur, acc, first, true);
  if (G::CHECKS && bad) flags[1] = 1;
}

typedef __attribute__((address_space(3))) void* msm_lds_ptr_t;
typedef const __attribute__((address_space(1))) void* msm_gbl_ptr_t;

template <class G>
__global__ void __launch_bounds__(256, G::ACC_WAVES) k_accumulate_glds(const uint2* __restrict__ entries, const uint32_t* __restrict__ n_real,
                                                         uint32_t K, const typename G::BaseDev* __restrict__ bases,
                                                         SegOutT<typename G::MemT> out, uint32_t nlanes, uint32_t* __restrict__ flags) {
  using E = typename G::E;
  using Base = typename G::Base;
  constexpr int LANES = G::LANES, RPQ = 4 / LANES;
  constexpr int SECT = G::GATHER_SECTORS;
  constexpr int RS = 1024;
#ifndef MSM_ACC_LDS_PAD
#define MSM_ACC_LDS_PAD 0
#endif
#ifndef MSM_ACC_IDX_AND
#define MSM_ACC_IDX_AND 0xffffffffu
#endif
#ifndef MSM_ACC_IDX_SHL
#define MSM_ACC_IDX_SHL 0
#endif
#ifndef MSM_ACC_PRIO
#define MSM_ACC_PRIO 0
#endif
  constexpr int WAVE_LDS = RPQ * SECT * RS + 256 + MSM_ACC_LDS_PAD;
  static_assert(sizeof(typename G::BaseDev) % 64 == 0 && SECT >= 2 && SECT <= 4 && SECT * 64 <= (int)sizeof(typename G::BaseDev), "record layout");
  __shared__ __attribute__((aligned(16))) unsigned char lds[4 * WAVE_LDS];
  const uint32_t t = (blockIdx.x * 256 + threadIdx.x) / LANES, half = threadIdx.x % LANES;
  const uint32_t lane = threadIdx.x & 63, sub = lane & 3, quad = lane >> 2;
  const uint32_t wave = __builtin_amdgcn_readfirstlane(threadIdx.x >> 6);
  unsigned char* wave_lds = lds + wave * WAVE_LDS;
  const unsigned char* rec = wave_lds + (sub / LANES) * (SECT * RS + 64) + quad * 64;
  typename E::Md md;
  const bool lane_ok = t < nlanes;
  if (lane_ok) {
    out.slot_keys[2 * (size_t)t] = KEY_NONE;
    out.slot_keys[2 * (size_t)t + 1] = KEY_NONE;
  }
  const uint32_t n_entries = *n_real;
  const uint64_t beg64 = (uint64_t)t * K;
  const bool has_work = lane_ok && beg64 < n_entries;
  const uint32_t beg = has_work ? (uint32_t)beg64 : 0;
  const uint32_t end = has_work ? ((n_entries - beg > K) ? beg + K : n_entries) : 0;

  constexpr int EQ = G::ENTRY_Q;
  uint4 q[EQ > 0 ? EQ : 1];
  uint32_t q_left = 0;
#define MSM_Q_REFILL(first_entry)                                                   \
  do {                                                                              \
    const uint4* src_ = reinterpret_cast<const uint4*>(entries + (first_entry));    \
    _Pragma("unroll") for (int j_ = 0; j_ < EQ; j_++) q[j_] = src_[j_];             \
  } while (0)
#define MSM_Q_POP(key_out, val_out)                                                 \
  do {                                                                              \
    key_out = q[0].y;                                                               \
    val_out = q[0].x;                                                               \
    _Pragma("unroll") for (int j_ = 0; j_ < EQ; j_++) {                             \
      q[j_].x = q[j_].z;                                                            \
      q[j_].y = q[j_].w;                                                            \
      if (j_ + 1 < EQ) {                                                            \
        q[j_].z = q[j_ + 1].x;                                                      \
        q[j_].w = q[j_ + 1].y;                                                      \
      }                                                                             \
    }                                                                               \
  } while (0)
  uint32_t key_c = KEY_NONE, val_c = 0, key_n = KEY_NONE, val_n = 0;
  if constexpr (EQ > 0) {
    if (end > beg) MSM_Q_REFILL(beg);
    MSM_Q_POP(key_c, val_c);
    MSM_Q_POP(key_n, val_n);
    q_left = 2 * EQ - 2;
    if (q_left == 0) {
      if (end - beg > 2 && end > beg) MSM_Q_REFILL(beg + 2);
      q_left = 2 * EQ;
    }
    if (end <= beg) key_c = key_n = KEY_NONE;
  } else if (end > beg) {
    const uint2 e0 = entries[beg];
    key_c = e0.y;
    val_c = e0.x;
    if (end - beg > 1) {
      const uint2 e1 = entries[beg + 1];
      key_n = e1.y;
      val_n = e1.x;
    }
  }
  bool alive = end > beg;

#define MSM_GLDS_ONE(i, ctrl)                                                                                            \
  do {                                                                                                                   \
    const uint4* s_ = reinterpret_cast<const uint4*>(bases + (uint32_t)__builtin_amdgcn_update_dpp(0, mine_, ctrl, 0xf, 0xf, true)) + sub; \
    _Pragma("unroll") for (int c_ = 0; c_ < SECT; c_++)                                                                  \
      __builtin_amdgcn_global_load_lds((msm_gbl_ptr_t)(s_ + 4 * c_), (msm_lds_ptr_t)(wave_lds + (i) * (SECT * RS + 64) + c_ * RS), 16, 0, 0); \
  } while (0)
#define MSM_GLDS_ISSUE(val, valid)                                \
  do {                                                            \
    const int mine_ = (valid) ? (int)((((val) & IDX_MASK & MSM_ACC_IDX_AND)) << MSM_ACC_IDX_SHL) : 0; \
    if constexpr (LANES == 1) {                                   \
      MSM_GLDS_ONE(0, 0x00);                                      \
      MSM_GLDS_ONE(1, 0x55);                                      \
      MSM_GLDS_ONE(2, 0xaa);                                      \
      MSM_GLDS_ONE(3, 0xff);                                      \
    } else {    \
      MSM_GLDS_ONE(0, 0x00);                                      \
      MSM_GLDS_ONE(1, 0xaa);                                      \
    }                                                             \
  } while (0)

  MSM_GLDS_ISSUE(val_c, alive);
  uint32_t cur = KEY_NONE;
  bool first = true, fresh = true, bad = false;
  XyzzT<typename G::T> acc;
  G::set_identity(acc);
#if MSM_ACC_PRIO == 3
  if (wave & 1) __builtin_amdgcn_s_sleep(127);
#endif
  uint32_t trips = K;
  if constexpr (G::ITER_BARRIER) {
    const uint64_t b0 = (uint64_t)blockIdx.x * (256 / LANES) * K;
    trips = b0 < n_entries ? (uint32_t)((n_entries - b0 < K) ? n_entries - b0 : K) : 0;
  }
  for (uint32_t k = 0; k < trips; k++) {
    if constexpr (G::ITER_BARRIER)
      __builtin_amdgcn_s_barrier();
    else if (__builtin_amdgcn_ballot_w64(alive) == 0)
      break;
    Base p;
#if MSM_ACC_PRIO == 2
    __builtin_amdgcn_s_setprio(2);
#endif
    asm volatile("s_waitcnt vmcnt(0)" ::: "memory");
    __builtin_amdgcn_wave_barrier();
    G::load_sectors(p, rec, RS, alive && (val_c >> 31) != 0, half);
    asm volatile("s_waitcnt lgkmcnt(0)" ::: "memory");
    __builtin_amdgcn_wave_barrier();
    const uint32_t key = key_c, val = val_c, e = beg + k;
    const bool add_now = alive;
    key_c = key_n;
    val_c = val_n;
    alive = add_now && (end - e > 1);
#ifndef MSM_ACC_NO_GATHER
    MSM_GLDS_ISSUE(val_c, alive);
#endif
    if constexpr (EQ > 0) {
      MSM_Q_POP(key_n, val_n);
      if (--q_left == 0) {
        if (add_now && end - e > 3) MSM_Q_REFILL(e + 3);
        q_left = 2 * EQ;
      }
    } else if (add_now && end - e > 2) {
      const uint2 e2 = entries[e + 2];
      key_n = e2.y;
      val_n = e2.x;
    }
#if MSM_ACC_PRIO == 2
    __builtin_amdgcn_s_setprio(0);
#endif
    if (add_now) {
      if (key != cur) {
        const bool lane_first = cur == KEY_NONE;
        if (cur != KEY_NONE) {
#ifndef MSM_ACC_NO_FLUSH
          seg_flush<G>(out, t, nlanes, cur, acc, first, false, half);
#endif
          first = false;
        }
        cur = key;
        fresh = true;
        G::begin_run(acc);
        if constexpr (G::CARRY_IN) {
          if (out.carry_in && !(lane_first && t > 0 && entries[beg - 1].y == key)) carry_begin_run<G>(out, key, acc, fresh, half);
        }
      }
#if MSM_ACC_PRIO == 1
      __builtin_amdgcn_s_setprio(2);
#endif
      if (G::madd_loaded(acc, p, (val >> 31) != 0, fresh, md)) {
        const Base again = G::from_dev_lane(bases[val & IDX_MASK], half);
        G::madd_same_x(acc, again, (val >> 31) != 0, md);
      }
#if MSM_ACC_PRIO == 1
      __builtin_amdgcn_s_setprio(0);
#endif
      if (G::CHECKS) bad |= G::failed(acc);
      fresh = false;
    }
  }
  if (cur != KEY_NONE) seg_flush<G>(out, t, nlanes, cur, acc, first, true, half);
  if (G::CHECKS && bad) flags[1] = 1;
#undef MSM_GLDS_ISSUE
#undef MSM_GLDS_ONE
#undef MSM_Q_REFILL
#undef MSM_Q_POP
}

template <class G>
__global__ void __launch_bounds__(256, G::ACC_WAVES) k_sum_bases(const typename G::BaseDev* __restrict__ bases, const uint8_t* __restrict__ inf,
                                                   uint32_t first, uint32_t n, uint32_t per_lane, SegOutT<typename G::T> out, uint32_t nlanes,
                                                   uint32_t* __restrict__ flags) {
  using E = typename G::E;
  static_assert(G::LANES == 1, "one lane per point");
  const uint32_t t = blockIdx.x * 256 + threadIdx.x;
  if (t >= nlanes) return;
  typename E::Md md;
  const uint64_t beg64 = (uint64_t)t * per_lane;
  const uint32_t beg = beg64 < n ? (uint32_t)beg64 : n, end = (n - beg > per_lane) ? beg + per_lane : n;
  bool fresh = true, bad = false;
  XyzzT<typename G::T> acc;
  G::set_identity(acc);
  G::begin_run(acc);
  typename G::Base p_n;
  if (beg < end) p_n = G::from_dev(bases[first + beg]);
  for (uint32_t i = beg; i < end; i++) {
    const typename G::Base p = p_n;
    const bool dead = inf[first + i] != 0;
    if (i + 1 < end) p_n = G::from_dev(bases[first + i + 1]);
    if (dead) continue;
    G::madd(acc, p, false, fresh, md);
    if (G::CHECKS) bad |= G::failed(acc);
    fresh = false;
  }
  out.slot_keys[2 * (size_t)t + 1] = KEY_NONE;
  if (fresh) {
    out.slot_keys[2 * (size_t)t] = KEY_NONE;
  } else {
    G::store_pt(out.slots + 2 * (size_t)t, acc, 0);
    out.slot_keys[2 * (size_t)t] = 0;
  }
  if (G::CHECKS && bad) flags[1] = 1;
}

template <class G>
__global__ void __launch_bounds__(256) k_segreduce(const XyzzDevT<typename G::MemT>* __restrict__ in_slots,
                                                   const uint32_t* __restrict__ in_keys, uint32_t n_in, uint32_t K,
                                                   SegOutT<typename G::MemT> out, uint32_t nlanes, uint32_t* __restrict__ flags) {
  using E = typename G::E;
  const uint32_t t = (blockIdx.x * 256 + threadIdx.x) / G::LANES, half = threadIdx.x % G::LANES;
  if (t >= nlanes) return;
  typename E::Md md;
  out.slot_keys[2 * (size_t)t] = KEY_NONE;
  out.slot_keys[2 * (size_t)t + 1] = KEY_NONE;
  const uint64_t beg = (uint64_t)t * K;
  const uint64_t end = (beg + K < n_in) ? beg + K : n_in;
  uint32_t cur = KEY_NONE;
  bool first = true, bad = false;
  XyzzT<typename G::T> acc;
  G::set_identity(acc);
  for (uint64_t e = beg; e < end; e++) {
    const uint32_t key = in_keys[e];
    if (key == KEY_NONE) continue;
    const XyzzT<typename G::T> v = G::load_pt(in_slots + e, half);
    if (key != cur) {
      if (cur != KEY_NONE) {
        seg_flush<G>(out, t, nlanes, cur, acc, first, false, half);
        first = false;
      }
      cur = key;
      acc = v;
    } else {
      G::add(acc, v, md);
      if (G::CHECKS) bad |= G::failed(acc);
    }
  }
  if (cur != KEY_NONE) seg_flush<G>(out, t, nlanes, cur, acc, first, true, half);
  if (G::CHECKS && bad) flags[1] = 1;
}

template <class G, bool FIRST>
__global__ void __launch_bounds__(256, G::ACC_WAVES) k_bucket_reduce(const XyzzDevT<typename G::MemT>* __restrict__ in_a,
                                                       const XyzzDevT<typename G::MemT>* __restrict__ in_x,
                                                       uint32_t n_per_win, uint32_t L, uint32_t chunks_per_win,
                                                       uint32_t windows, uint32_t out_stride, XyzzDevT<typename G::MemT>* __restrict__ out_a,
                                                       XyzzDevT<typename G::MemT>* __restrict__ out_x, uint32_t* __restrict__ flags,
                                                       uint32_t run_win) {
  using E = typename G::E;
  using XD = XyzzDevT<typename G::MemT>;
  const uint32_t g = (blockIdx.x * 256 + threadIdx.x) / G::LANES, half = threadIdx.x % G::LANES;
  if (g >= windows * chunks_per_win) return;
  typename E::Md md;
  const uint32_t w = g / chunks_per_win, t = g % chunks_per_win;
  const uint32_t lo = t * L;
  const uint32_t hi = (lo + L < n_per_win) ? lo + L : n_per_win;
  const XD* x = in_x + (size_t)w * n_per_win;
  XyzzT<typename G::T> run, wsum;
  bool bad = false;
  G::set_identity(run);
  G::set_identity(wsum);
#ifndef MSM_REDUCE_PREFETCH
#define MSM_REDUCE_PREFETCH 0
#endif
#if MSM_REDUCE_PREFETCH
  XyzzT<typename G::T> v_next;
  if (hi > lo) v_next = G::load_pt(x + hi - 1, half);
  for (uint32_t j = hi; j-- > lo;) {
    const XyzzT<typename G::T> v = v_next;
    if (j > lo) v_next = G::load_pt(x + j - 1, half);
    G::add(run, v, md);
    if (G::CHECKS) bad |= G::failed(run);
    if (FIRST || j > lo) {
      G::add(wsum, run, md);
      if (G::CHECKS) bad |= G::failed(wsum);
    }
  }
#else
  for (uint32_t j = hi; j-- > lo;) {
    const XyzzT<typename G::T> v = G::load_pt(x + j, half);
    G::add(run, v, md);
    if (G::CHECKS) bad |= G::failed(run);
    if (FIRST || j > lo) {
      G::add(wsum, run, md);
      if (G::CHECKS) bad |= G::failed(wsum);
    }
  }
#endif
  if (!FIRST) {
    const XD* a = in_a + (size_t)w * n_per_win;
    for (uint32_t j = lo; j < hi; j++) {
      const XyzzT<typename G::T> v = G::load_pt(a + j, half);
      G::add(wsum, v, md);
      if (G::CHECKS) bad |= G::failed(wsum);
    }
  }
  const size_t at = (size_t)w * out_stride + t;
  G::store_pt(out_a + at, wsum, half);
  if (FIRST && w == run_win) G::store_pt(out_a + (size_t)windows * out_stride + t, run, half);
  if ((L & (L - 1)) == 0) {
    G::mul_pow2(run, 31 - __builtin_clz(L), md);
    if (G::CHECKS) bad |= G::failed(run);
  } else {
    const XyzzT<typename G::T> one = run;
    for (int b = 30 - __builtin_clz(L); b >= 0; b--) {
// ... 283 lines not shown
```

### 2022-entries_amd/csrc/msm_types.hpp

```cpp
#pragma once
#include "curve.hpp"

namespace msm {

constexpr uint32_t KEY_NONE = 0xffffffffu;
constexpr uint32_t IDX_MASK = 0x7fffffffu;

template <class T>
struct alignas(128) AffineDevT {
  AffineT<T> p;
};
template <class T>
struct alignas(16) XyzzDevT {
  XyzzT<T> p;
};
using AffineDev = AffineDevT<Fe>;
using XyzzDev = XyzzDevT<Fe>;
static_assert(sizeof(AffineDev) == 128 && sizeof(AffineDevT<Fe2>) == 256, "device affine layout");
static_assert(sizeof(XyzzDev) == 224 && sizeof(XyzzDevT<Fe2>) == 448, "device xyzz layout");

template <class T>
struct SegOutT {
  XyzzDevT<T>* buckets;
  XyzzDevT<T>* slots;
  uint32_t* slot_keys;
  uint32_t carry_in = 0;
};
using SegOut = SegOutT<Fe>;

}
```

### 2022-entries_amd/csrc/partition.hpp

```cpp
#pragma once
#include <hip/hip_runtime.h>
#include <stdint.h>

#include <algorithm>

#include "digits.hpp"
#include "partition_plan.hpp"

namespace msm {

__device__ __forceinline__ void lds_barrier() {
#ifdef PART_FULL_BARRIER
  __syncthreads();
#else
  asm volatile("s_waitcnt lgkmcnt(0)\n\ts_barrier" ::: "memory");
#endif
}

__device__ __forceinline__ uint32_t wave_incl_scan(uint32_t v) {
#pragma unroll
  for (int d = 1; d < 64; d <<= 1) {
    const uint32_t u = __shfl_up(v, d, 64);
    if ((int)(threadIdx.x & 63) >= d) v += u;
  }
  return v;
}
template <bool TAIL_BARRIER = true>
__device__ __forceinline__ uint32_t block_excl_scan(uint32_t v, uint32_t* tmp, uint32_t& total) {
  const uint32_t incl = wave_incl_scan(v);
  const uint32_t wave = threadIdx.x >> 6, lane = threadIdx.x & 63, nw = blockDim.x >> 6;
  if (lane == 63) tmp[wave] = incl;
  lds_barrier();
  if (wave == 0) {
    uint32_t w = lane < nw ? tmp[lane] : 0;
    const uint32_t wi = wave_incl_scan(w);
    if (lane < nw) tmp[lane] = wi - w;
    if (lane == nw - 1) tmp[16] = wi;
  }
  lds_barrier();
  const uint32_t r = tmp[wave] + incl - v;
  total = tmp[16];
  if (TAIL_BARRIER) lds_barrier();
  return r;
}

struct ScalarDigits {
  uint32_t s[8];
  uint32_t carry;
};
template <int L>
__device__ __forceinline__ uint32_t scalar_bits_at(const uint32_t (&s)[8], uint32_t sh) {
  if constexpr (L >= 8) {
    return 0;
  } else {
    const uint32_t hi = L < 7 ? s[L < 7 ? L + 1 : 7] : 0u;
    return __builtin_amdgcn_alignbit(hi, s[L], sh);
  }
}
__device__ __forceinline__ uint32_t scalar_window(const uint32_t (&s)[8], uint32_t o) {
  const uint32_t sh = o & 31;
  switch (o >> 5) {
    case 0: return scalar_bits_at<0>(s, sh);
    case 1: return scalar_bits_at<1>(s, sh);
    case 2: return scalar_bits_at<2>(s, sh);
    case 3: return scalar_bits_at<3>(s, sh);
    case 4: return scalar_bits_at<4>(s, sh);
    case 5: return scalar_bits_at<5>(s, sh);
    case 6: return scalar_bits_at<6>(s, sh);
    case 7: return scalar_bits_at<7>(s, sh);
    default: return 0;
  }
}
template <bool FOLD>
__device__ __forceinline__ void next_digit(ScalarDigits& st, uint32_t u, uint32_t c, uint32_t half, uint32_t wmask, bool flip, uint32_t rwin,
                                           uint32_t& mag, bool& neg, bool anchor = false, uint32_t wide = 0) {
  if constexpr (FOLD) {
    const uint32_t sub = u + ((st.carry >> 1) & 1u);
    const bool borrow = flip && rwin < sub;
    u = flip ? ((rwin - sub) & wmask) : u;
    const uint32_t v = u + (st.carry & 1u);
    const bool over = v > half;
    mag = over ? (1u << c) - v : v;
    neg = over != flip;
    st.carry = (over ? 1u : 0u) | (borrow ? 2u : 0u);
  } else {
    const uint32_t v = u + st.carry;
    if (wide) {
      const uint32_t full = 1u << c;
      neg = v < full;
      const uint32_t m = neg ? full - v : v - full;
      mag = wide == 1 ? (m <= half ? m : 0u) : (m > half ? m - half : 0u);
    } else if (anchor) {
      neg = v < half;
      mag = neg ? half - v : v - half;
      st.carry = 0;
    } else {
      neg = v > half;
      mag = neg ? (1u << c) - v : v;
      st.carry = neg ? 1u : 0u;
    }
  }
}

__device__ __forceinline__ uint32_t step_wide(const PartPlan& p, uint32_t w) { return (p.wide && w >= p.anchor) ? w - p.anchor + 1 : 0u; }
__device__ __forceinline__ uint32_t step_offset(const PartPlan& p, uint32_t w) { return (p.wide && w > p.anchor ? p.anchor : w) * p.c; }
__device__ __forceinline__ uint32_t step_mask(const PartPlan& p, uint32_t w) { return (p.wide && w >= p.anchor) ? (2u << p.c) - 1 : (1u << p.c) - 1; }
__device__ __forceinline__ bool scalar_bits_from(const uint32_t (&s)[8], uint32_t top) {
  uint32_t any = 0;
#pragma unroll
  for (int j = 0; j < 8; j++) {
    if ((uint32_t)j == (top >> 5)) any |= s[j] >> (top & 31);
    if ((uint32_t)j > (top >> 5)) any |= s[j];
  }
  return any != 0;
}

template <class FR>
__device__ __forceinline__ uint32_t fr_window(uint32_t w, uint32_t c, uint32_t wmask) {
  const uint32_t o = w * c, limb = o >> 5, sh = o & 31;
  if (limb >= 8) return 0;
  uint32_t lo = 0, hi = 0;
#pragma unroll
  for (int j = 0; j < 8; j++) {
    if ((uint32_t)j == limb) lo = FR::R[j];
    if ((uint32_t)j == limb + 1) hi = FR::R[j];
  }
  return ((lo >> sh) | (sh ? hi << (32 - sh) : 0u)) & wmask;
}

template <class FR>
__device__ __forceinline__ bool fold_decision(const ScalarDigits& st) {
  return st.s[7] > (FR::R[7] >> 1) && st.s[7] < FR::R[7];
}

struct ScalarWords {
  uint32_t w[8];
};
template <class FR>
__device__ __noinline__ ScalarWords fr_to_montgomery_call(ScalarWords a) {
  fr_to_montgomery<FR>(a.w);
  return a;
}

template <class FR, int MODE>
__device__ __forceinline__ void load_scalar(ScalarDigits& st, const uint32_t* __restrict__ scalars, uint32_t i) {
  const uint4* sp = reinterpret_cast<const uint4*>(scalars) + 2 * (size_t)i;
  const uint4 lo = sp[0], hi = sp[1];
  uint32_t s[8] = {lo.x, lo.y, lo.z, lo.w, hi.x, hi.y, hi.z, hi.w};
  if constexpr (MODE == SCALARS_FROM_MONT) fr_from_montgomery<FR>(s);
  if constexpr (MODE == SCALARS_TO_MONT) {
    const ScalarWords w = fr_to_montgomery_call<FR>(ScalarWords{{s[0], s[1], s[2], s[3], s[4], s[5], s[6], s[7]}});
#pragma unroll
    for (int j = 0; j < 8; j++) s[j] = w.w[j];
  }
#pragma unroll
  for (int j = 0; j < 8; j++) st.s[j] = s[j];
  st.carry = 0;
}

// ... 303 lines not shown
      where[k] = 0xffffffffu;
      const uint32_t bucket = ok ? mag - 1 : 0, hi = bucket >> p.lb;
      uint32_t rank = 0;
      if (few)
        rank = few_bins_rank(cnt, p.b1, ok, hi);
      else if (ok)
        rank = atomicAdd(&cnt[hi], 1u);
      if (ok) {
        where[k] = (hi << 16) | rank;
        low[k] = (bucket & lowmask) | (neg ? 0x80000000u : 0u);
      }
    }
    lds_barrier();
    {
      const uint32_t v = threadIdx.x < p.b1 ? cnt[threadIdx.x] : 0;
      uint32_t tot;
      const uint32_t ex = block_excl_scan<false>(v, tmp, tot);
      if (threadIdx.x < p.b1) {
        tstart[threadIdx.x] = ex;
        offs[threadIdx.x] = offs_next - ex;
        cnt[threadIdx.x] = 0;
        if (w + 1 < w_hi) offs_next = row[l1_bin_of(p, w + 1, threadIdx.x)];
      }
      if (threadIdx.x == 0) tstart[p.b1] = tot;
    }
    lds_barrier();
#pragma unroll
    for (int k = 0; k < PART_PER_THREAD; k++)
      if (where[k] != 0xffffffffu) {
        const uint32_t idx = l1_base_index(p, i0 + threadIdx.x + k * PART_THREADS, w);
        stage[tstart[where[k] >> 16] + (where[k] & 0xffffu)] = make_uint2(idx | (low[k] & 0x80000000u), (low[k] & 0xffffu) | (where[k] & 0xffff0000u));
      }
    lds_barrier();
    const uint32_t total = tstart[p.b1];
    for (uint32_t j = threadIdx.x; j < total; j += PART_THREADS) {
      uint2 e = stage[j];
      const uint32_t hi = e.y >> 16;
      e.y &= 0xffffu;
#ifdef PART_EXP_L1_NOSTORE
      if (e.x == 0x12345678u && e.y == 0x9abcu) out[0] = e;
#elif defined(PART_EXP_L1_OUT4)
      reinterpret_cast<uint32_t*>(out)[offs[hi] + j] = e.x;
#else
      out[offs[hi] + j] = e;
#endif
    }
  }
}


__device__ __forceinline__ bool subjob_range(const PartSeg* __restrict__ segs, const uint32_t* __restrict__ subjob_first, uint32_t nsegs,
                                             uint32_t j, uint32_t& seg, uint32_t& beg, uint32_t& end) {
  if (j >= subjob_first[nsegs]) return false;
  uint32_t lo = 0, hi = nsegs;
  while (hi - lo > 1) {
    const uint32_t mid = (lo + hi) >> 1;
    if (subjob_first[mid] <= j) lo = mid; else hi = mid;
  }
  while (lo + 1 < nsegs && subjob_first[lo + 1] <= j) lo++;
  seg = lo;
  const PartSeg s = segs[seg];
  const uint32_t k = j - subjob_first[seg];
  beg = s.start + k * PART_SUBJOB;
  end = min(s.start + s.len, beg + PART_SUBJOB);
  return beg < end;
}

__global__ void __launch_bounds__(1024) k_pass_hist(const uint2* __restrict__ in, const PartSeg* __restrict__ segs,
                                                    const uint32_t* __restrict__ subjob_first, PassPlan pp, uint32_t* __restrict__ counts) {
  __shared__ uint32_t hist[1 << PART_MAX_RB];
  const uint32_t nb = 1u << pp.rb, shift = pp.rem - pp.rb;
  const uint32_t nsub = subjob_first[pp.nsegs];
  for (uint32_t j = blockIdx.x; j < nsub; j += gridDim.x) {
    uint32_t seg, beg, end;
    const bool live = subjob_range(segs, subjob_first, pp.nsegs, j, seg, beg, end);
    if (!live || part_fused_takes(segs[seg].len)) continue;
    for (uint32_t b = threadIdx.x; b < nb; b += 1024) hist[b] = 0;
    __syncthreads();
    for (uint32_t e = beg + threadIdx.x; e < end; e += 1024) atomicAdd(&hist[(in[e].y >> shift) & (nb - 1)], 1u);
    __syncthreads();
    uint32_t* row = counts + (size_t)j * nb;
    for (uint32_t b = threadIdx.x; b < nb; b += 1024) row[b] = hist[b];
    __syncthreads();
  }
}

__global__ void __launch_bounds__(1024) k_pass_scan(const PartSeg* __restrict__ segs, const uint32_t* __restrict__ subjob_first, PassPlan pp,
                                                    uint32_t* __restrict__ counts, PartSeg* __restrict__ out_segs) {
  __shared__ uint32_t tmp[32];
  const uint32_t s = blockIdx.x, nb = 1u << pp.rb, b = threadIdx.x;
  const PartSeg sg = segs[s];
  if (part_fused_takes(sg.len)) return;
  const uint32_t j0 = subjob_first[s], j1 = subjob_first[s + 1];
  uint32_t tot_b = 0;
  if (b < nb)
    for (uint32_t j = j0; j < j1; j++) tot_b += counts[(size_t)j * nb + b];
  uint32_t tot;
  const uint32_t before = block_excl_scan(tot_b, tmp, tot);
  if (b < nb) {
    uint32_t run = sg.start + before;
    if (out_segs) out_segs[(size_t)s * nb + b] = PartSeg{run, tot_b, sg.key_base + (b << (pp.rem - pp.rb)), 0};
    for (uint32_t j = j0; j < j1; j++) {
      const size_t at = (size_t)j * nb + b;
      const uint32_t v = counts[at];
      counts[at] = run;
      run += v;
    }
  }
}

__global__ void __launch_bounds__(1024) k_pass_subjobs(const PartSeg* __restrict__ segs, uint32_t nsegs, uint32_t* __restrict__ subjob_first,
                                                       uint32_t* __restrict__ totals) {
  __shared__ uint32_t tmp[32];
  __shared__ uint32_t carry;
  if (threadIdx.x == 0) carry = 0;
  __syncthreads();
  for (uint32_t s0 = 0; s0 < nsegs; s0 += 1024) {
    const uint32_t s = s0 + threadIdx.x;
    const uint32_t nsj = s < nsegs ? part_subjobs_of(segs[s].len) : 0;
    uint32_t tot;
    const uint32_t before = block_excl_scan(nsj, tmp, tot);
    const uint32_t base = carry;
    if (s < nsegs) subjob_first[s] = base + before;
    __syncthreads();
    if (threadIdx.x == 0) carry = base + tot;
    __syncthreads();
  }
  if (threadIdx.x == 0) {
    subjob_first[nsegs] = carry;
    totals[1] = carry;
  }
}

#ifdef PART_EXP_PS_CACHEDLOAD
#define PART_LD(e) ((e) & 0x3fffu)
#else
#define PART_LD(e) (e)
#endif
#ifdef PART_EXP_PS_IN4
__device__ __forceinline__ uint2 part_in(const uint2* __restrict__ in, uint32_t e) {
  const uint32_t v = reinterpret_cast<const uint32_t*>(in)[e];
  return make_uint2(v, (v * 2654435761u) >> 16);
}
#define PART_IN(in, e) part_in(in, e)
#else
#define PART_IN(in, e) ((in)[e])
#endif
struct PassLds {
  uint2 stage[PART_PTILE];
  uint32_t cur[1 << PART_MAX_RB], cnt[1 << PART_MAX_RB], tstart[(1 << PART_MAX_RB) + 1], dst[1 << PART_MAX_RB];
  uint32_t tmp[32];
};

__device__ __forceinline__ void pass_scatter_tiles(PassLds& L, const uint2* __restrict__ in, uint2* __restrict__ out, uint32_t beg, uint32_t end,
                                                   const PassPlan& pp, uint32_t key_base) {
  const uint32_t nb = 1u << pp.rb, shift = pp.rem - pp.rb, keepmask = (1u << shift) - 1;
  constexpr int PER = PART_PTILE / 1024;
  uint2 nxt[PER];
#pragma unroll
  for (int k = 0; k < PER; k++) {
    const uint32_t e = beg + threadIdx.x + k * 1024;
    if (e < end) nxt[k] = PART_IN(in, PART_LD(e));
  }
  for (uint32_t t0 = beg; t0 < end; t0 += PART_PTILE) {
    uint2 ent[PER];
#pragma unroll
    for (int k = 0; k < PER; k++) {
      ent[k] = nxt[k];
      const uint32_t e = t0 + PART_PTILE + threadIdx.x + k * 1024;
      if (e < end) nxt[k] = PART_IN(in, PART_LD(e));
    }
    uint32_t where[PER];
#pragma unroll
    for (int k = 0; k < PER; k++) {
      const uint32_t e = t0 + threadIdx.x + k * 1024;
      where[k] = 0xffffffffu;
      if (e < end) {
        const uint32_t bin = (ent[k].y >> shift) & (nb - 1);
        const uint32_t rank = atomicAdd(&L.cnt[bin], 1u);
        where[k] = (bin << 16) | rank;
        ent[k].y = (ent[k].y & keepmask) | (bin << 16);
      }
    }
    lds_barrier();
    {
      const uint32_t v = threadIdx.x < nb ? L.cnt[threadIdx.x] : 0;
      uint32_t tot;
      const uint32_t ex = block_excl_scan<false>(v, L.tmp, tot);
      if (threadIdx.x < nb) {
        const uint32_t c0 = L.cur[threadIdx.x];
        L.tstart[threadIdx.x] = ex;
#ifdef PART_EXP_PS_ALIGNED
        L.dst[threadIdx.x] = (c0 & ~15u) - ex;
#else
        L.dst[threadIdx.x] = c0 - ex;
#endif
        L.cur[threadIdx.x] = c0 + v;
        L.cnt[threadIdx.x] = 0;
      }
      if (threadIdx.x == 0) L.tstart[nb] = tot;
    }
    lds_barrier();
#pragma unroll
    for (int k = 0; k < PER; k++)
      if (where[k] != 0xffffffffu) L.stage[L.tstart[where[k] >> 16] + (where[k] & 0xffffu)] = ent[k];
    lds_barrier();
    const uint32_t total = L.tstart[nb];
    for (uint32_t j = threadIdx.x; j < total; j += 1024) {
      uint2 e = L.stage[j];
      const uint32_t bin = e.y >> 16;
      e.y = pp.last ? key_base + bin : (e.y & 0xffffu);
#if defined(PART_EXP_PS_NOSTORE)
      if (e.x == 0x12345678u && e.y == 0x9abcu) out[0] = e;
#elif defined(PART_EXP_PS_L2STORE)
      out[(L.dst[bin] + j) & 0x1ffffu] = e;
#elif defined(PART_EXP_PS_OUT4)
      reinterpret_cast<uint32_t*>(out)[L.dst[bin] + j] = e.x;
#else
      out[L.dst[bin] + j] = e;
#endif
    }
  }
}

__global__ void __launch_bounds__(1024, PART_PASS_OCC) k_pass_scatter(const uint2* __restrict__ in, const PartSeg* __restrict__ segs,
                                                          const uint32_t* __restrict__ subjob_first, PassPlan pp, uint32_t gen,
                                                          const uint32_t* __restrict__ positions, uint2* __restrict__ out,
                                                          PartSeg* __restrict__ out_segs) {
  __shared__ PassLds L;
  const uint32_t nb = 1u << pp.rb, shift = pp.rem - pp.rb;
  if (blockIdx.x < gen) {
    const uint32_t nsub = subjob_first[pp.nsegs];
    for (uint32_t j = blockIdx.x; j < nsub; j += gen) {
      uint32_t seg, beg, end;
      const bool live = subjob_range(segs, subjob_first, pp.nsegs, j, seg, beg, end);
      if (!live) continue;
      const PartSeg sg = segs[seg];
      if (part_fused_takes(sg.len)) continue;
      const uint32_t* row = positions + (size_t)j * nb;
      lds_barrier();
      for (uint32_t b = threadIdx.x; b < nb; b += 1024) {
        L.cur[b] = row[b];
        L.cnt[b] = 0;
      }
      lds_barrier();
      pass_scatter_tiles(L, in, out, beg, end, pp, sg.key_base);
    }
    return;
  }
  const uint32_t s = blockIdx.x - gen;
  const PartSeg sg = segs[s];
  if (!part_fused_takes(sg.len)) return;
  if (sg.len == 0) {
    if (out_segs)
      for (uint32_t b = threadIdx.x; b < nb; b += 1024) out_segs[(size_t)s * nb + b] = PartSeg{sg.start, 0, sg.key_base + (b << shift), 0};
    return;
  }
  const uint32_t beg = sg.start, end = sg.start + sg.len;
  for (uint32_t b = threadIdx.x; b < nb; b += 1024) L.cnt[b] = 0;
  lds_barrier();
  {
    uint32_t e = beg + threadIdx.x;
    for (; e + 3 * 1024 < end; e += 4 * 1024) {
      const uint32_t k0 = PART_IN(in, e).y, k1 = PART_IN(in, e + 1024).y, k2 = PART_IN(in, e + 2048).y, k3 = PART_IN(in, e + 3072).y;
      atomicAdd(&L.cnt[(k0 >> shift) & (nb - 1)], 1u);
      atomicAdd(&L.cnt[(k1 >> shift) & (nb - 1)], 1u);
      atomicAdd(&L.cnt[(k2 >> shift) & (nb - 1)], 1u);
      atomicAdd(&L.cnt[(k3 >> shift) & (nb - 1)], 1u);
    }
    for (; e < end; e += 1024) atomicAdd(&L.cnt[(PART_IN(in, e).y >> shift) & (nb - 1)], 1u);
  }
  lds_barrier();
  {
    const uint32_t v = threadIdx.x < nb ? L.cnt[threadIdx.x] : 0;
    uint32_t tot;
    const uint32_t ex = block_excl_scan(v, L.tmp, tot);
    if (threadIdx.x < nb) {
      L.cur[threadIdx.x] = beg + ex;
      L.cnt[threadIdx.x] = 0;
      if (out_segs) out_segs[(size_t)s * nb + threadIdx.x] = PartSeg{beg + ex, v, sg.key_base + (threadIdx.x << shift), 0};
    }
  }
  lds_barrier();
  pass_scatter_tiles(L, in, out, beg, end, pp, sg.key_base);
}

}

namespace msm {

#ifdef MSM_DEBUG
enum { DBG_DIGITS = 0, DBG_SEG_GAP = 1, DBG_SEG_END = 2, DBG_KEY_BITS = 3, DBG_UNSORTED = 4, DBG_KEY_RANGE = 5, DBG_VALUE_RANGE = 6,
       DBG_SLOT_KEY = 7, DBG_CHECKS = 8, DBG_WORDS = 12 };

template <class FR, int MODE, bool FOLD>
__global__ void __launch_bounds__(256) k_dbg_count_digits(const uint32_t* __restrict__ scalars, const uint8_t* __restrict__ inf, PartPlan p,
                                                          uint32_t* __restrict__ dbg) {
  const uint32_t i = blockIdx.x * 256 + threadIdx.x;
  uint32_t count = 0;
  if (i < p.n) {
    ScalarDigits st;
    load_scalar<FR, MODE>(st, scalars, i);
    const bool flip = FOLD ? fold_decision<FR>(st) : false;
    const uint32_t wmask = (1u << p.c) - 1;
    for (uint32_t w = 0; w < p.windows; w++) {
      const uint32_t wide = step_wide(p, w);
      const uint32_t u = st.s[0] & step_mask(p, w);
      if (wide != 1) {
        for (int j = 0; j < 7; j++) st.s[j] = (st.s[j] >> p.c) | (st.s[j + 1] << (32 - p.c));
        st.s[7] >>= p.c;
      }
      uint32_t mag;
      bool neg;
      next_digit<FOLD>(st, u, p.c, p.half, wmask, flip, FOLD ? fr_window<FR>(w, p.c, wmask) : 0u, mag, neg, w == p.anchor, wide);
      const bool dead = inf[l1_base_index(p, i, w)] != 0;
      if (mag != 0 && !dead) count++;
    }
  }
  for (int d = 32; d > 0; d >>= 1) count += __shfl_down(count, d, 64);
  if ((threadIdx.x & 63) == 0 && count) atomicAdd(&dbg[DBG_DIGITS], count);
}

__global__ void __launch_bounds__(256) k_dbg_check_level(const uint2* __restrict__ entries, const PartSeg* __restrict__ segs, uint32_t nsegs, uint32_t rem,
                                                         const uint32_t* __restrict__ totals, uint32_t* __restrict__ dbg) {
  const uint32_t s = blockIdx.x;
  const PartSeg sg = segs[s];
  if (threadIdx.x == 0) {
    const uint32_t expect = s ? segs[s - 1].start + segs[s - 1].len : 0u;
    if (sg.start != expect) atomicAdd(&dbg[DBG_SEG_GAP], 1u);
    if (s + 1 == nsegs && sg.start + sg.len != totals[0]) atomicAdd(&dbg[DBG_SEG_END], 1u);
  }
  uint32_t bad = 0;
  for (uint32_t e = sg.start + threadIdx.x; e < sg.start + sg.len; e += 256)
    if (rem < 32 && (entries[e].y >> rem) != 0) bad++;
  if (bad) atomicAdd(&dbg[DBG_KEY_BITS], bad);
}

__global__ void __launch_bounds__(256) k_dbg_check_sorted(const uint2* __restrict__ entries, const uint32_t* __restrict__ totals, uint32_t key_limit,
                                                          uint32_t idx_lo, uint32_t idx_hi, uint32_t* __restrict__ dbg) {
  const uint32_t n = totals[0];
  for (uint32_t i = blockIdx.x * 256 + threadIdx.x; i < n; i += gridDim.x * 256) {
    const uint2 e = entries[i];
    if (i + 1 < n && entries[i + 1].y < e.y) atomicAdd(&dbg[DBG_UNSORTED], 1u);
    if (e.y >= key_limit) atomicAdd(&dbg[DBG_KEY_RANGE], 1u);
    const uint32_t idx = e.x & 0x7fffffffu;
    if (idx < idx_lo || idx >= idx_hi) atomicAdd(&dbg[DBG_VALUE_RANGE], 1u);
  }
}

__global__ void __launch_bounds__(256) k_dbg_check_slots(const uint32_t* __restrict__ keys, uint32_t n, uint32_t key_limit, uint32_t* __restrict__ dbg) {
  const uint32_t i = blockIdx.x * 256 + threadIdx.x;
  if (i < n && keys[i] != 0xffffffffu && keys[i] >= key_limit) atomicAdd(&dbg[DBG_SLOT_KEY], 1u);
  if (i == 0) atomicAdd(&dbg[DBG_CHECKS], 1u);
}

__global__ void k_dbg_corrupt(uint2* __restrict__ entries, const uint32_t* __restrict__ totals) {
  const uint32_t n = totals[0];
  for (uint32_t i = 0; i + 1 < n; i++)
    if (entries[i].y != entries[i + 1].y) {
      const uint32_t k = entries[i].y;
      entries[i].y = entries[i + 1].y;
      entries[i + 1].y = k;
      return;
    }
}
#endif


#ifndef PART_GEN_GRID
#define PART_GEN_GRID 512u
#endif
struct PartProbe {
  static constexpr int MAX = 32;
  hipEvent_t ev[MAX + 1];
  const char* name[MAX];
  int n = 0;
  void mark(const char* what, hipStream_t st) {
    if (n < MAX) {
      name[n] = what;
      (void)hipEventRecord(ev[++n], st);
    }
  }
};
#define PART_MARK(what) do { if (probe) probe->mark(what, st); } while (0)

template <class FR, int MODE>
inline int part_run(const uint32_t* d_scalars, const uint8_t* d_inf, const PartPlan& p, const PartBuffers& b, hipStream_t st,
                    hipEvent_t mid, hipError_t& err, PartProbe* probe = nullptr) {
  err = hipSuccess;
  if (probe) {
    probe->n = 0;
    (void)hipEventRecord(probe->ev[0], st);
  }
#ifdef MSM_DEBUG
  uint32_t* const dbg = b.totals + 4;
  (void)hipMemsetAsync(dbg, 0, DBG_WORDS * 4, st);
#define PART_DBG_LEVEL(ENT, SEGS, NSEGS, REM)                                                                              \
  do {                                                                                                                     \
    hipLaunchKernelGGL(k_dbg_check_level, dim3((uint32_t)(NSEGS)), dim3(256), 0, st, ENT, SEGS, (uint32_t)(NSEGS), REM, b.totals, dbg); \
    hipLaunchKernelGGL(k_dbg_check_slots, dim3(1), dim3(256), 0, st, b.totals, 0u, 0u, dbg);           \
  } while (0)
#else
#define PART_DBG_LEVEL(ENT, SEGS, NSEGS, REM) do { } while (0)
#endif
  const uint64_t entries = (uint64_t)p.n * p.windows;
  const dim3 scan_grid(part_ceil_div(p.nbins, 256), PART_SCAN_GROUPS);
  const uint32_t l1_grid = 8 * ((p.ntiles + 7) / 8) * p.wgroups;
  if (p.fold)
    hipLaunchKernelGGL((k_l1_hist<FR, MODE, true>), dim3(l1_grid), dim3(PART_THREADS), p.nbins * 4, st, d_scalars, d_inf, p, b.matrix, b.wide_flag);
  else
    hipLaunchKernelGGL((k_l1_hist<FR, MODE, false>), dim3(l1_grid), dim3(PART_THREADS), p.nbins * 4, st, d_scalars, d_inf, p, b.matrix, b.wide_flag);
  PART_MARK("l1_hist");
  hipLaunchKernelGGL(k_l1_scan_a, scan_grid, dim3(256), 0, st, b.matrix, p, b.partial);
  hipLaunchKernelGGL(k_l1_scan_b, dim3(1), dim3(1024), 0, st, b.partial, p, b.segs[0], b.subjob_first, b.totals);
  hipLaunchKernelGGL(k_l1_scan_c, scan_grid, dim3(256), 0, st, b.matrix, p, b.partial);
  PART_MARK("l1_scan");
  int seg_cur = 0;
  uint64_t nsegs = p.nbins;
  if (p.shared) {
    hipLaunchKernelGGL(k_l1_merge_shared, dim3(1), dim3(256), 0, st, b.segs[0], p, b.segs[1], b.subjob_first, b.totals);
    seg_cur = 1;
    nsegs = (uint64_t)p.bsets * p.b1;
  }
  if (p.fold)
    hipLaunchKernelGGL((k_l1_scatter<FR, MODE, true>), dim3(l1_grid), dim3(PART_THREADS), 0, st, d_scalars, d_inf, p, b.matrix, b.entries[0]);
  else
    hipLaunchKernelGGL((k_l1_scatter<FR, MODE, false>), dim3(l1_grid), dim3(PART_THREADS), 0, st, d_scalars, d_inf, p, b.matrix, b.entries[0]);
  PART_MARK("l1_scatter");
  PART_DBG_LEVEL(b.entries[0], b.segs[seg_cur], nsegs, p.lb);
  if (mid) (void)hipEventRecord(mid, st);
  uint32_t rb[4];
  const int np = part_pass_bits(p.lb, rb);
  uint32_t rem = p.lb;
  int cur = 0;
  for (int i = 0; i < np; i++) {
    PassPlan pp{};
    pp.nsegs = (uint32_t)nsegs;
    pp.rem = rem;
    pp.rb = rb[i];
    pp.last = (i == np - 1) ? 1 : 0;
    pp.max_subjobs = part_max_subjobs(entries, nsegs);
    PartSeg* out_segs = pp.last ? nullptr : b.segs[seg_cur ^ 1];
    const bool long_segs = !part_fused_takes((uint32_t)std::min<uint64_t>((uint64_t)p.n * p.levels, 0xffffffffu));
    const uint32_t gen = long_segs ? std::min<uint32_t>(pp.max_subjobs, PART_GEN_GRID) : 0;
    if (long_segs) {
      hipLaunchKernelGGL(k_pass_hist, dim3(std::min<uint32_t>(pp.max_subjobs, 2048u)), dim3(1024), 0, st, b.entries[cur], b.segs[seg_cur], b.subjob_first, pp,
                         b.counts);
      PART_MARK("pass_hist");
      hipLaunchKernelGGL(k_pass_scan, dim3(pp.nsegs), dim3(1024), 0, st, b.segs[seg_cur], b.subjob_first, pp, b.counts, out_segs);
      PART_MARK("pass_scan");
    }
    hipLaunchKernelGGL(k_pass_scatter, dim3(gen + pp.nsegs), dim3(1024), 0, st, b.entries[cur], b.segs[seg_cur], b.subjob_first, pp, gen, b.counts,
                       b.entries[cur ^ 1], out_segs);
    PART_MARK("pass_scatter");
    cur ^= 1;
    rem -= rb[i];
    if (!pp.last) {
      nsegs <<= rb[i];
      seg_cur ^= 1;
      hipLaunchKernelGGL(k_pass_subjobs, dim3(1), dim3(1024), 0, st, b.segs[seg_cur], (uint32_t)nsegs, b.subjob_first, b.totals);
      PART_DBG_LEVEL(b.entries[cur], b.segs[seg_cur], nsegs, rem);
    }
  }
#ifdef MSM_DEBUG
  {
    const uint32_t key_limit = p.bsets * p.half;
    const uint32_t idx_hi = p.idx0 + p.n + (p.levels - 1) * p.table_stride;
    if (getenv("MI355_MSM_DEBUG_CORRUPT")) hipLaunchKernelGGL(k_dbg_corrupt, dim3(1), dim3(1), 0, st, b.entries[cur], b.totals);
    hipLaunchKernelGGL(k_dbg_check_sorted, dim3(2048), dim3(256), 0, st, b.entries[cur], b.totals, key_limit, p.idx0, idx_hi, dbg);
    if (p.fold)
      hipLaunchKernelGGL((k_dbg_count_digits<FR, MODE, true>), dim3(part_ceil_div(p.n, 256)), dim3(256), 0, st, d_scalars, d_inf, p, dbg);
    else
      hipLaunchKernelGGL((k_dbg_count_digits<FR, MODE, false>), dim3(part_ceil_div(p.n, 256)), dim3(256), 0, st, d_scalars, d_inf, p, dbg);
    hipLaunchKernelGGL(k_dbg_check_slots, dim3(1), dim3(256), 0, st, b.totals, 0u, 0u, dbg);
  }
#endif
  err = hipGetLastError();
  return cur;
}

}
```

### 2022-entries_amd/csrc/partition_plan.hpp

```cpp
#pragma once
#include <hip/hip_runtime.h>
#include <stddef.h>
#include <stdint.h>

#include <algorithm>

namespace msm {

enum ScalarMode : int {
  SCALARS_PLAIN = 0,
  SCALARS_FROM_MONT = 1,
  SCALARS_TO_MONT = 2,
};

constexpr int PART_TILE = 8192;
constexpr int PART_THREADS = 1024;
constexpr int PART_PER_THREAD = PART_TILE / PART_THREADS;
#ifndef PART_MAX_HB_V
#define PART_MAX_HB_V 10
#endif
constexpr int PART_MAX_HB = PART_MAX_HB_V;
constexpr int PART_MAX_RB = 10;
constexpr uint32_t PART_SUBJOB = 192u << 10;
#ifndef PART_PTILE_V
#define PART_PTILE_V 16384
#endif
#ifndef PART_PASS_OCC
#define PART_PASS_OCC 4
#endif
constexpr int PART_PTILE = PART_PTILE_V;
constexpr int PART_SCAN_GROUPS = 64;

struct PartSeg {
  uint32_t start, len;
  uint32_t key_base;
  uint32_t pad;
};

struct PartPlan {
  uint32_t n, c, windows, half;
  uint32_t shared;
  uint32_t levels, bsets;
  uint32_t idx0, table_stride;
  uint32_t hb, lb;
  uint32_t b1;
  uint32_t nbins;
  uint32_t ntiles;
  uint32_t tiles_per_group;
  uint32_t wgroups, wper;
  uint32_t fold;
  uint32_t anchor;
  uint32_t wide;
  uint32_t wide_top;
};
constexpr uint32_t PART_NO_ANCHOR = 0xffffffffu;

struct PassPlan {
  uint32_t nsegs;
  uint32_t rem, rb;
  uint32_t last;
  uint32_t max_subjobs;
};


inline uint32_t part_ceil_div(uint64_t a, uint64_t b) { return (uint32_t)((a + b - 1) / b); }

inline PartPlan part_plan(uint32_t n, uint32_t c, uint32_t windows, uint32_t levels, uint32_t idx0, uint32_t table_stride, bool fold = false,
                          uint32_t anchor = 0xffffffffu, bool wide = false) {
  PartPlan p{};
  p.fold = fold ? 1 : 0;
  p.anchor = fold ? 0xffffffffu : anchor;
  p.wide = (wide && p.anchor != 0xffffffffu && levels <= 1 && p.anchor + 2 == windows) ? 1 : 0;
  p.wide_top = p.wide ? (p.anchor + 1) * c + 1 : 0;
  p.n = n;
  p.c = c;
  p.windows = windows;
  p.half = 1u << (c - 1);
  p.levels = levels > 1 ? std::min(levels, windows) : 1;
  p.bsets = part_ceil_div(windows, p.levels);
  p.levels = part_ceil_div(windows, p.bsets);
  p.shared = p.levels > 1 ? 1 : 0;
  p.idx0 = idx0;
  p.table_stride = table_stride;
  const uint32_t bits = c - 1;
  uint32_t lg = 0;
  while ((2ull << lg) <= (uint64_t)n) lg++;
  const uint32_t by_size = lg > 15 ? lg - 15 : 0;
  p.hb = std::min<uint32_t>(std::min<uint32_t>(bits, (uint32_t)PART_MAX_HB), by_size);
  if (bits - p.hb > 15) p.hb = bits - 15;
  if (bits - p.hb > (uint32_t)PART_MAX_RB && bits - (uint32_t)PART_MAX_RB <= (uint32_t)PART_MAX_HB && bits - p.hb <= 2 * (uint32_t)PART_MAX_RB)
    p.hb = bits - (uint32_t)PART_MAX_RB;
  p.lb = bits - p.hb;
  p.b1 = 1u << p.hb;
  p.nbins = p.bsets * p.levels * p.b1;
  p.ntiles = part_ceil_div(n, PART_TILE);
  if (p.ntiles == 0) p.ntiles = 1;
  p.tiles_per_group = part_ceil_div(p.ntiles, PART_SCAN_GROUPS);
  const uint32_t want = p.ntiles >= 256 ? 1 : part_ceil_div(256, p.ntiles);
  p.wgroups = std::min<uint32_t>(windows, want);
  p.wper = part_ceil_div(windows, p.wgroups);
  p.wgroups = part_ceil_div(windows, p.wper);
  return p;
}

inline int part_pass_bits(uint32_t lb, uint32_t (&rb)[4]) {
  int np = (int)((lb + PART_MAX_RB - 1) / PART_MAX_RB);
  if (np == 0) np = 1;
  uint32_t last = lb < (uint32_t)PART_MAX_RB ? lb : (uint32_t)PART_MAX_RB;
  uint32_t left = lb - last;
  for (int i = 0; i < np - 1; i++) {
    rb[i] = (left + (uint32_t)(np - 1 - i) - 1) / (uint32_t)(np - 1 - i);
    left -= rb[i];
  }
  rb[np - 1] = last;
  return np;
}

#ifdef PART_NO_FUSED_PASS
__host__ __device__ inline bool part_fused_takes(uint32_t) { return false; }
__host__ __device__ inline uint32_t part_subjobs_of(uint32_t len) { return (len + PART_SUBJOB - 1) / PART_SUBJOB; }
inline uint32_t part_max_subjobs(uint64_t entries, uint64_t nsegs) { return (uint32_t)(entries / PART_SUBJOB + nsegs + 1); }
#else
__host__ __device__ inline bool part_fused_takes(uint32_t len) { return len <= PART_SUBJOB; }
__host__ __device__ inline uint32_t part_subjobs_of(uint32_t len) { return len > PART_SUBJOB ? (len + PART_SUBJOB - 1) / PART_SUBJOB : 0; }
inline uint32_t part_max_subjobs(uint64_t entries, uint64_t ) { return (uint32_t)(2 * entries / PART_SUBJOB + 2); }
#endif

struct PartScratchSizes {
  size_t matrix, partial, segs_a, segs_b, subjob_first, counts, totals;
};
inline PartScratchSizes part_scratch_sizes(const PartPlan& p) {
  PartScratchSizes s{};
  const uint64_t entries = (uint64_t)p.n * p.windows;
  s.matrix = (size_t)p.ntiles * p.nbins * 4;
  s.partial = (size_t)PART_SCAN_GROUPS * p.nbins * 4;
  uint32_t rb[4];
  const int np = part_pass_bits(p.lb, rb);
  uint64_t nsegs = p.shared ? (uint64_t)p.bsets * p.b1 : p.nbins, max_segs = p.nbins, max_counts = 0, max_sj = 0;
  for (int i = 0; i < np; i++) {
    const uint64_t sj = part_max_subjobs(entries, nsegs);
    max_counts = std::max<uint64_t>(max_counts, sj << rb[i]);
    max_sj = std::max<uint64_t>(max_sj, nsegs + 1);
    nsegs <<= rb[i];
    if (i + 1 < np) max_segs = std::max<uint64_t>(max_segs, nsegs);
  }
  max_sj = std::max<uint64_t>(max_sj, max_segs + 1);
  s.segs_a = s.segs_b = (size_t)max_segs * sizeof(PartSeg);
  s.subjob_first = (size_t)(max_sj + 1) * 4;
  s.counts = (size_t)max_counts * 4;
  s.totals = 64;
  return s;
}

struct PartBuffers {
  uint2* entries[2];
  uint32_t* matrix;
  uint32_t* partial;
  PartSeg* segs[2];
  uint32_t* subjob_first;
  uint32_t* counts;
  uint32_t* totals;
  uint32_t* wide_flag;
};


}
```

Measured before the change: 667.5 million.

## Pack sorted MSM entries into 32-bit words with delta-encoded bucket keys

Adds a compact 32-bit entry format for the sorted (bucket key, point index) list. Each word holds the point index, a sign bit and a small key-step code, and escaped or lane-start keys go to a side run_keys array. The last partition scatter pass writes this format and the accumulate kernels decode keys on the fly. The aim is to halve entry memory traffic in the scatter and bucket-accumulate stages, at the cost of extra decode logic, K being rounded to multiples of 16, and the format only applying when tables are off and n fits the index bits.

```diff
diff --git a/2022-entries_amd/csrc/host_test_api.cpp b/2022-entries_amd/csrc/host_test_api.cpp
--- a/2022-entries_amd/csrc/host_test_api.cpp
+++ b/2022-entries_amd/csrc/host_test_api.cpp
@@ -2674,3 +2674,53 @@
 }
 int ht_sm_window_for(uint64_t len) { return (int)sm_window_for(len); }
 }
+
+#include "msm_types.hpp"
+
+extern "C" {
+long ht_e32_encode(const uint32_t* keys, const uint32_t* values, size_t n, uint32_t K, const uint32_t* seg_keys, const uint8_t* seg_subjobs, size_t nseg,
+                   uint32_t* words, uint32_t* run_keys) {
+  if (K == 0 || nseg == 0 || !seg_keys || (n && (!keys || !values || !words || !run_keys))) return -1;
+  long escapes = 0;
+  size_t seg = 0, prev_seg = (size_t)-1;
+  for (size_t i = 0; i < n; i++) {
+    if (i && keys[i] < keys[i - 1]) return -1;
+    if (keys[i] < seg_keys[0]) return -1;
+    while (seg + 1 < nseg && seg_keys[seg + 1] <= keys[i]) seg++;
+    uint32_t step = 0;
+    if (i == 0 || keys[i] != keys[i - 1]) {
+      const bool first_of_segment = seg != prev_seg;
+      step = e32_step_of_gap(first_of_segment ? 0u : keys[i] - keys[i - 1], first_of_segment || (seg_subjobs && seg_subjobs[seg]));
+      prev_seg = seg;
+    }
+    words[i] = e32_pack(values[i], step);
+    if (step == E32_ESCAPE) {
+      run_keys[i] = keys[i];
+      escapes++;
+    }
+  }
+  for (size_t i = 0; i < n;) {
+    size_t j = i;
+    while (j < n && keys[j] == keys[i]) j++;
+    for (uint64_t q = e32_first_lane_start((uint32_t)i, K); q < j; q += K) run_keys[q] = keys[i];
+    i = j;
+  }
+  return escapes;
+}
+int ht_e32_decode(const uint32_t* words, const uint32_t* run_keys, size_t n, uint32_t K, uint32_t* keys_out, uint32_t* values_out, uint8_t* continued) {
+  if (K == 0) return -1;
+  for (size_t beg = 0, t = 0; beg < n; beg += K, t++) {
+    const size_t end = beg + K < n ? beg + K : n;
+    uint32_t cur = run_keys[beg];
+    if (continued) continued[t] = e32_step(words[beg]) == 0;
+    for (size_t i = beg; i < end; i++) {
+      if (i > beg) cur = e32_next_key(cur, words[i], run_keys, (uint32_t)i);
+      keys_out[i] = cur;
+      values_out[i] = (words[i] & 0x80000000u) | e32_index(words[i]);
+    }
+  }
+  return 0;
+}
+uint32_t ht_e32_run_keys_offset(uint64_t capacity) { return e32_run_keys_offset(capacity); }
+int ht_e32_applies(uint64_t idx0, uint64_t n, uint32_t table_levels) { return e32_applies(idx0, n, table_levels) ? 1 : 0; }
+}
diff --git a/2022-entries_amd/csrc/launch.hpp b/2022-entries_amd/csrc/launch.hpp
--- a/2022-entries_amd/csrc/launch.hpp
+++ b/2022-entries_amd/csrc/launch.hpp
@@ -47,7 +47,7 @@
   using El = typename LawMem<G>::MemT;
   using BaseDev = typename LawMem<G>::BaseDev;
   static hipError_t accumulate(const uint2* entries, const uint32_t* n_real, uint32_t K, const BaseDev* bases, SegOutT<El> out, uint32_t nlanes,
-                               uint32_t* flags, hipStream_t st);
+                               uint32_t* flags, uint32_t e32_rk_off, hipStream_t st);
   static hipError_t sum_bases(const BaseDev* bases, const uint8_t* inf, uint32_t first, uint32_t n, uint32_t per_lane, SegOutT<El> out, uint32_t nlanes,
                               uint32_t* flags, hipStream_t st);
   static hipError_t segreduce(const XyzzDevT<El>* in_slots, const uint32_t* in_keys, uint32_t n_in, uint32_t K, SegOutT<El> out, uint32_t nlanes,
diff --git a/2022-entries_amd/csrc/launch_impl.hpp b/2022-entries_amd/csrc/launch_impl.hpp
--- a/2022-entries_amd/csrc/launch_impl.hpp
+++ b/2022-entries_amd/csrc/launch_impl.hpp
@@ -59,10 +59,19 @@
 
 template <class G>
 hipError_t WalkLaunch<G>::accumulate(const uint2* entries, const uint32_t* n_real, uint32_t K, const BaseDev* bases, SegOutT<El> out, uint32_t nlanes,
-                                     uint32_t* flags, hipStream_t st) {
+                                     uint32_t* flags, uint32_t e32_rk_off, hipStream_t st) {
 #ifndef MSM_GATHER
 #define MSM_GATHER 2
 #endif
+  if (e32_rk_off) {
+    const uint32_t* const words = reinterpret_cast<const uint32_t*>(entries);
+    const Entries32Ptr e32{words, words + e32_rk_off};
+    if constexpr (MSM_GATHER == 2 || !kIsSwLaw<G>)
+      hipLaunchKernelGGL((k_accumulate_glds<G, Entries32>), dim3(walk_blocks<G>(nlanes)), dim3(256), 0, st, e32, n_real, K, bases, out, nlanes, flags);
+    else
+      hipLaunchKernelGGL((k_accumulate<G, Entries32>), dim3(walk_blocks<G>(nlanes)), dim3(256), 0, st, e32, n_real, K, bases, out, nlanes, flags);
+    return hipGetLastError();
+  }
   if constexpr (MSM_GATHER == 2 || !kIsSwLaw<G>)
     hipLaunchKernelGGL((k_accumulate_glds<G>), dim3(walk_blocks<G>(nlanes)), dim3(256), 0, st, entries, n_real, K, bases, out, nlanes, flags);
   else
@@ -138,7 +147,7 @@
   using S_ = SegOutT<E::T>;                                                                                                                      \
   using W_ = WalkLaunch<SwLaw<E>>;                                                                                                               \
   template hipError_t Launch<E>::convert_bases(const uint8_t*, size_t, uint32_t, bool, A_*, uint8_t*, hipStream_t);                              \
-  template hipError_t W_::accumulate(const uint2*, const uint32_t*, uint32_t, const A_*, S_, uint32_t, uint32_t*, hipStream_t);                  \
+  template hipError_t W_::accumulate(const uint2*, const uint32_t*, uint32_t, const A_*, S_, uint32_t, uint32_t*, uint32_t, hipStream_t);        \
   template hipError_t W_::segreduce(const X_*, const uint32_t*, uint32_t, uint32_t, S_, uint32_t, uint32_t, uint32_t*, hipStream_t);             \
   template hipError_t Launch<E>::pre_double(const A_*, const uint8_t*, uint32_t, uint32_t, X_*, hipStream_t);                                    \
   template hipError_t Launch<E>::pre_normalize(const X_*, uint32_t, uint32_t, E::T*, A_*, uint8_t*, hipStream_t);                                \
diff --git a/2022-entries_amd/csrc/msm_engine.hip b/2022-entries_amd/csrc/msm_engine.hip
--- a/2022-entries_amd/csrc/msm_engine.hip
+++ b/2022-entries_amd/csrc/msm_engine.hip
@@ -292,6 +292,7 @@
   uint32_t levels;
   uint32_t anchor;
   bool wide;
+  bool e32;
   uint64_t entries;
   uint32_t K, nlanes;
   uint32_t segK;
@@ -304,6 +305,10 @@
 };
 
 }
+
+#ifndef MSM_ENTRIES32_DEFAULT
+#define MSM_ENTRIES32_DEFAULT 1
+#endif
 
 #ifndef MSM_G2_PAIRED_DEFAULT
 #define MSM_G2_PAIRED_DEFAULT 31
@@ -374,6 +379,8 @@
   uint32_t wide_streak = 0;
   uint64_t wide_fallbacks = 0, wide_demotions = 0;
   bool last_wide = false;
+  long opt_entries32 = MSM_ENTRIES32_DEFAULT;
+  bool last_e32 = false;
   DevBuf wide_flag, wide_r;
   uint32_t* h_wide_flag = nullptr;
   long opt_reduce_log_chunk = 0, opt_reduce_log_chunk0 = 0;
@@ -432,6 +439,7 @@
     p.anchor = anchor_armed ? anchor_window((int)p.c, scalar_bits(), opt_anchor == 2) : kNoAnchor;
     p.wide = wide_wanted() && !tables && anchor_wide_fits(p.anchor, (int)p.c, scalar_bits());
     p.windows = (257 + p.c - 1) / p.c;
+    p.e32 = opt_entries32 != 0 && !tables && n <= ((size_t)1 << E32_IDX_BITS);
     p.levels = tables ? std::min<uint32_t>(pre_windows, p.windows) : 1;
     p.bucket_windows = ceil_div(p.windows, p.levels);
     p.levels = ceil_div(p.windows, p.bucket_windows);
@@ -458,7 +466,7 @@
         double best_fill = fill(best);
         for (long step = 8; step <= 96 && best_fill < 0.985; step += 8)
           for (long k : {(long)K - step, (long)K + step})
-            if (k >= 64 && fill(k) > best_fill + 0.004) {
+            if (k >= 64 && (!p.e32 || k % 16 == 0) && fill(k) > best_fill + 0.004) {
               best = k;
               best_fill = fill(k);
             }
@@ -466,6 +474,7 @@
       }
     }
     p.K = K >= 8 ? (K + 7) & ~7u : (K + 3) & ~3u;
+    if (p.e32 && !opt_lane_entries && p.K >= 16) p.K = (p.K + 15) & ~15u;
     p.nlanes = ceil_div(p.entries, p.K);
     p.segK = opt_seg_entries >= 4 ? (uint32_t)opt_seg_entries : (p.entries < (2u << 20) ? 4 : 8);
     uint64_t nb = (uint64_t)p.bucket_windows * p.half;
@@ -540,7 +549,7 @@
 uint64_t work_bytes(const Plan& p, uint64_t el, bool carry = false) {
   const PartPlan pp = part_plan((uint32_t)(p.entries / p.windows), p.c, p.windows, p.levels, 0, 0);
   const PartScratchSizes ps = part_scratch_sizes(pp);
-  return p.entries * 16 + ps.matrix + ps.partial + ps.segs_a + ps.segs_b + ps.subjob_first + ps.counts + ps.totals +
+  return p.entries * 16 + 256 + ps.matrix + ps.partial + ps.segs_a + ps.segs_b + ps.subjob_first + ps.counts + ps.totals +
          (uint64_t)p.bucket_windows * p.half * 224 * el * (carry ? 2 : 1) + 2 * (2ull * p.nlanes) * (224 * el + 4) + (p.scan_direct ? (uint64_t)p.bucket_windows * p.half : 4ull * (p.bucket_windows + (p.wide ? 1 : 0)) * p.scan_nb) * 224 * el;
 }
 
@@ -567,7 +576,7 @@
   const PartScratchSizes gs = part_scratch_sizes(gp);
   const size_t nbuckets = (size_t)p.bucket_windows * p.half, nslots0 = 2 * (size_t)p.nlanes;
   const size_t red0 = p.scan_direct ? nbuckets : (size_t)(p.bucket_windows + (p.wide ? 1 : 0)) * p.scan_nb;
-  w.b[0] = w.b[1] = p.entries * 8 + 64;
+  w.b[0] = w.b[1] = p.entries * 8 + 128;
   w.b[2] = gs.matrix;
   w.b[3] = gs.partial;
   w.b[4] = gs.segs_a;
@@ -760,6 +769,7 @@
     tmp.opt_assume_subgroup = ctx->opt_assume_subgroup;
     tmp.opt_anchor = ctx->opt_anchor;
     tmp.opt_anchor_wide = ctx->opt_anchor_wide;
+    tmp.opt_entries32 = ctx->opt_entries32;
     tmp.opt_carry = ctx->opt_carry;
     tmp.opt_lane_entries = ctx->opt_lane_entries;
     tmp.opt_seg_entries = ctx->opt_seg_entries;
@@ -1043,6 +1053,7 @@
 template <class G>
 XyzzDevT<typename LawMem<G>::MemT>* accumulate_chunk(mi355_msm_ctx* ctx, const Plan& p, const PartPlan& gp, const PartBuffers& gb, const uint2* entries,
                                                      const BucketCarry* carry, hipStream_t st, hipEvent_t* ev) {
+  const uint32_t e32_rk_off = gb.e32_lane_k ? e32_run_keys_offset(p.entries) : 0u;
   using El = typename LawMem<G>::MemT;
   using XyzzDev = XyzzDevT<El>;
   const size_t nbuckets = (size_t)p.bucket_windows * p.half;
@@ -1053,7 +1064,7 @@
   SegOutT<El> so{ctx->buckets.as<XyzzDev>(), ctx->slots[0].as<XyzzDev>(), ctx->slot_keys[0].as<uint32_t>()};
   so.carry_in = carry_in ? 1u : 0u;
   HIP_OK(walk_form<G>(ctx, 1, false, [&]<class L>() {
-    return WalkLaunch<L>::accumulate(entries, gb.totals, p.K, law_bases<G>(ctx), so, p.nlanes, law_flags<G>(ctx), st);
+    return WalkLaunch<L>::accumulate(entries, gb.totals, p.K, law_bases<G>(ctx), so, p.nlanes, law_flags<G>(ctx), e32_rk_off, st);
   }));
   HIP_OK(hipEventRecord(ev[3], st));
 #ifdef MSM_DEBUG
@@ -1242,6 +1253,8 @@
   HIP_OK(hipEventRecord(ev[0], st));
   PartBuffers gb{};
   gb.wide_flag = p.wide ? ctx->wide_flag.as<uint32_t>() : nullptr;
+  gb.e32_lane_k = (p.e32 && e32_applies(base0, n, use_tables ? p.levels : 1) && p.K % 4 == 0) ? p.K : 0u;
+  ctx->last_e32 = gb.e32_lane_k != 0;
   const uint2* entries = group_chunk(ctx, d_scalars, gp, gb, st, ev[1]);
   XyzzDev* const bucket_src = accumulate_chunk<G>(ctx, p, gp, gb, entries, carry, st, ev);
   HIP_OK(hipEventRecord(ev[4], st));
@@ -2245,6 +2258,10 @@
       ctx->wide_off = false;
       ctx->wide_streak = 0;
       ctx->fitted_chunk = 0;
+    } else if (k == "entries32") {
+      if (value < 0 || value > 1) bad_arg("entries32 %ld out of range [0, 1]", value);
+      ctx->opt_entries32 = value;
+      ctx->fitted_chunk = 0;
     } else if (k == "first_piece_div") {
       if (value != 0 && (value < 2 || value > 64)) bad_arg("first_piece_div %ld out of range [2, 64]", value);
       ctx->opt_first_piece_div = value;
@@ -2333,9 +2350,9 @@
       }
       static const char* const kAll[] = {"twisted_edwards", "assume_subgroup", "carry"};
       static const char* const kMean[] = {"table_levels", "table_window_bits"};
-      static const char* const kFirst[] = {"precompute", "g2_paired", "guard_tail", "te_limb_bits", "anchor", "anchor_wide"};
+      static const char* const kFirst[] = {"precompute", "g2_paired", "guard_tail", "te_limb_bits", "anchor", "anchor_wide", "entries32"};
       static const char* const kMax[] = {"bucket_windows", "l1_bits", "l1_bins", "group_passes", "anchored_window", "anchor_sum_us", "anchor_wide_active",
-                                          "reduce_path", "reduce_chunks", "reduce_row"};
+                                          "reduce_path", "reduce_chunks", "reduce_row", "entries32_active"};
       auto in = [&](const char* const* set, size_t n) {
         for (size_t i = 0; i < n; i++)
           if (k == set[i]) return true;
@@ -2345,7 +2362,7 @@
         *value = all;
       } else if (in(kMean, 2)) {
         *value = sum / ctx->shards.size();
-      } else if (in(kFirst, 6) || in(kMax, 10)) {
+      } else if (in(kFirst, 7) || in(kMax, 11)) {
         uint64_t first = 0, mx = 0;
         for (size_t g = 0; g < ctx->shards.size(); g++) {
           uint64_t v = 0;
@@ -2358,7 +2375,7 @@
           if (g == 0) first = v;
           mx = std::max(mx, v);
         }
-        *value = in(kFirst, 6) ? first : mx;
+        *value = in(kFirst, 7) ? first : mx;
       } else {
         *value = sum;
       }
@@ -2418,6 +2435,10 @@
       *value = (ctx->opt_anchor_wide && !ctx->wide_off) ? 1 : 0;
     else if (k == "anchor_wide_active")
       *value = ctx->last_wide ? 1 : 0;
+    else if (k == "entries32")
+      *value = ctx->opt_entries32 ? 1 : 0;
+    else if (k == "entries32_active")
+      *value = ctx->last_e32 ? 1 : 0;
     else if (k == "anchor_wide_fallbacks")
       *value = ctx->wide_fallbacks;
     else if (k == "anchor_wide_demotions")
diff --git a/2022-entries_amd/csrc/msm_kernels.hpp b/2022-entries_amd/csrc/msm_kernels.hpp
--- a/2022-entries_amd/csrc/msm_kernels.hpp
+++ b/2022-entries_amd/csrc/msm_kernels.hpp
@@ -62,12 +62,78 @@
   if (fresh) G::begin_run(acc);
 }
 
-template <class G>
-__global__ void __launch_bounds__(256, G::ACC_WAVES) k_accumulate(const uint2* __restrict__ entries, const uint32_t* __restrict__ n_real,
+struct Entries64 {
+  static constexpr bool WORD32 = false;
+  static constexpr int PER16 = 2;
+  using Word = uint2;
+  using Ptr = const uint2*;
+  static __device__ __forceinline__ const uint2* words(Ptr p) { return p; }
+  static __device__ __forceinline__ uint32_t index(uint32_t value) { return value & IDX_MASK; }
+};
+struct Entries32Ptr {
+  const uint32_t* words;
+  const uint32_t* run_keys;
+};
+struct Entries32 {
+  static constexpr bool WORD32 = true;
+  static constexpr int PER16 = 4;
+  using Word = uint32_t;
+  using Ptr = Entries32Ptr;
+  static __device__ __forceinline__ const uint32_t* words(Ptr p) { return p.words; }
+  static __device__ __forceinline__ uint32_t index(uint32_t value) { return e32_index(value); }
+};
+
+template <class G, class EF = Entries64>
+__global__ void __launch_bounds__(256, G::ACC_WAVES) k_accumulate(typename EF::Ptr entries_arg, const uint32_t* __restrict__ n_real,
                                                     uint32_t K, const typename G::BaseDev* __restrict__ bases,
                                                     SegOutT<typename G::T> out, uint32_t nlanes, uint32_t* __restrict__ flags) {
   using E = typename G::E;
   static_assert(G::LANES == 1, "the one-lane-per-record walk has no paired form");
+  if constexpr (EF::WORD32) {
+    const uint32_t* __restrict__ words = entries_arg.words;
+    const uint32_t t = blockIdx.x * 256 + threadIdx.x;
+    if (t >= nlanes) return;
+    typename E::Md md;
+    out.slot_keys[2 * (size_t)t] = KEY_NONE;
+    out.slot_keys[2 * (size_t)t + 1] = KEY_NONE;
+    const uint32_t n_entries = *n_real;
+    const uint64_t beg64 = (uint64_t)t * K;
+    if (beg64 >= n_entries) return;
+    const uint32_t beg = (uint32_t)beg64;
+    const uint32_t end = (n_entries - beg > K) ? beg + K : n_entries;
+    uint32_t w_c = words[beg], w_n = 0;
+    if (end - beg > 1) w_n = words[beg + 1];
+    typename G::Base p_c;
+    if (G::PREFETCH_BASE) p_c = G::from_dev(bases[e32_index(w_c)]);
+    uint32_t cur = KEY_NONE;
+    bool first = true, fresh = true, bad = false;
+    XyzzT<typename G::T> acc;
+    G::set_identity(acc);
+    for (uint32_t e = beg; e < end; e++) {
+      const uint32_t val = w_c;
+      if (!G::PREFETCH_BASE) p_c = G::from_dev(bases[e32_index(val)]);
+      const typename G::Base p = p_c;
+      w_c = w_n;
+      if (G::PREFETCH_BASE && end - e > 1) p_c = G::from_dev(bases[e32_index(w_c)]);
+      if (end - e > 2) w_n = words[e + 2];
+      if (e == beg || e32_step(val) != 0) {
+        if (e != beg) {
+          seg_flush<G>(out, t, nlanes, cur, acc, first, false);
+          first = false;
+        }
+        cur = e == beg ? entries_arg.run_keys[e] : e32_next_key(cur, val, entries_arg.run_keys, e);
+        fresh = true;
+        G::begin_run(acc);
+      }
+      G::madd(acc, p, (val >> 31) != 0, fresh, md);
+      if (G::CHECKS) bad |= G::failed(acc);
+      fresh = false;
+    }
+    if (cur != KEY_NONE) seg_flush<G>(out, t, nlanes, cur, acc, first, true);
+    if (G::CHECKS && bad) flags[1] = 1;
+    return;
+  } else {
+  const uint2* __restrict__ entries = entries_arg;
   const uint32_t t = blockIdx.x * 256 + threadIdx.x;
   if (t >= nlanes) return;
   typename E::Md md;
@@ -110,17 +176,20 @@
   }
   if (cur != KEY_NONE) seg_flush<G>(out, t, nlanes, cur, acc, first, true);
   if (G::CHECKS && bad) flags[1] = 1;
+  }
 }
 
 typedef __attribute__((address_space(3))) void* msm_lds_ptr_t;
 typedef const __attribute__((address_space(1))) void* msm_gbl_ptr_t;
-
-template <class G>
-__global__ void __launch_bounds__(256, G::ACC_WAVES) k_accumulate_glds(const uint2* __restrict__ entries, const uint32_t* __restrict__ n_real,
+typedef uint32_t msm_u32x4_t __attribute__((ext_vector_type(4)));
+
+template <class G, class EF = Entries64>
+__global__ void __launch_bounds__(256, G::ACC_WAVES) k_accumulate_glds(typename EF::Ptr entries_arg, const uint32_t* __restrict__ n_real,
                                                          uint32_t K, const typename G::BaseDev* __restrict__ bases,
                                                          SegOutT<typename G::MemT> out, uint32_t nlanes, uint32_t* __restrict__ flags) {
   using E = typename G::E;
   using Base = typename G::Base;
+  const typename EF::Word* __restrict__ entries = EF::words(entries_arg);
   constexpr int LANES = G::LANES, RPQ = 4 / LANES;
   constexpr int SECT = G::GATHER_SECTORS;
   constexpr int RS = 1024;
@@ -157,45 +226,83 @@
   const uint32_t end = has_work ? ((n_entries - beg > K) ? beg + K : n_entries) : 0;
 
   constexpr int EQ = G::ENTRY_Q;
+  constexpr int QCAP = EF::PER16 * EQ;
   uint4 q[EQ > 0 ? EQ : 1];
   uint32_t q_left = 0;
 #define MSM_Q_REFILL(first_entry)                                                   \
   do {                                                                              \
-    const uint4* src_ = reinterpret_cast<const uint4*>(entries + (first_entry));    \
-    _Pragma("unroll") for (int j_ = 0; j_ < EQ; j_++) q[j_] = src_[j_];             \
+    if constexpr (EF::WORD32) {                                                     \
+       \
+      const msm_u32x4_t* src_ = reinterpret_cast<const msm_u32x4_t*>(entries + (first_entry)); \
+      _Pragma("unroll") for (int j_ = 0; j_ < EQ; j_++) {                           \
+        const msm_u32x4_t v_ = src_[j_];                                            \
+        q[j_] = make_uint4(v_.x, v_.y, v_.z, v_.w);                                 \
+      }                                                                             \
+    } else {                                                                        \
+      const uint4* src_ = reinterpret_cast<const uint4*>(entries + (first_entry));  \
+      _Pragma("unroll") for (int j_ = 0; j_ < EQ; j_++) q[j_] = src_[j_];           \
+    }                                                                               \
   } while (0)
 #define MSM_Q_POP(key_out, val_out)                                                 \
   do {                                                                              \
-    key_out = q[0].y;                                                               \
     val_out = q[0].x;                                                               \
-    _Pragma("unroll") for (int j_ = 0; j_ < EQ; j_++) {                             \
-      q[j_].x = q[j_].z;                                                            \
-      q[j_].y = q[j_].w;                                                            \
-      if (j_ + 1 < EQ) {                                                            \
-        q[j_].z = q[j_ + 1].x;                                                      \
-        q[j_].w = q[j_ + 1].y;                                                      \
+    if constexpr (EF::WORD32) {                                                     \
+      _Pragma("unroll") for (int j_ = 0; j_ < EQ; j_++) {                           \
+        q[j_].x = q[j_].y;                                                          \
+        q[j_].y = q[j_].z;                                                          \
+        q[j_].z = q[j_].w;                                                          \
+        if (j_ + 1 < EQ) q[j_].w = q[j_ + 1].x;                                     \
+      }                                                                             \
+    } else {                                                                        \
+      key_out = q[0].y;                                                             \
+      _Pragma("unroll") for (int j_ = 0; j_ < EQ; j_++) {                           \
+        q[j_].x = q[j_].z;                                                          \
+        q[j_].y = q[j_].w;                                                          \
+        if (j_ + 1 < EQ) {                                                          \
+          q[j_].z = q[j_ + 1].x;                                                    \
+          q[j_].w = q[j_ + 1].y;                                                    \
+        }                                                                           \
       }                                                                             \
     }                                                                               \
   } while (0)
   uint32_t key_c = KEY_NONE, val_c = 0, key_n = KEY_NONE, val_n = 0;
   if constexpr (EQ > 0) {
     if (end > beg) MSM_Q_REFILL(beg);
-    MSM_Q_POP(key_c, val_c);
-    MSM_Q_POP(key_n, val_n);
-    q_left = 2 * EQ - 2;
+    if constexpr (EF::WORD32) {
+      val_c = q[0].x;
+      val_n = q[0].y;
+#pragma unroll
+      for (int j = 0; j < EQ; j++) {
+        q[j].x = q[j].z;
+        q[j].y = q[j].w;
+        if (j + 1 < EQ) {
+          q[j].z = q[j + 1].x;
+          q[j].w = q[j + 1].y;
+        }
+      }
+    } else {
+      MSM_Q_POP(key_c, val_c);
+      MSM_Q_POP(key_n, val_n);
+    }
+    q_left = QCAP - 2;
     if (q_left == 0) {
       if (end - beg > 2 && end > beg) MSM_Q_REFILL(beg + 2);
-      q_left = 2 * EQ;
+      q_left = QCAP;
     }
     if (end <= beg) key_c = key_n = KEY_NONE;
   } else if (end > beg) {
-    const uint2 e0 = entries[beg];
-    key_c = e0.y;
-    val_c = e0.x;
-    if (end - beg > 1) {
-      const uint2 e1 = entries[beg + 1];
-      key_n = e1.y;
-      val_n = e1.x;
+    if constexpr (EF::WORD32) {
+      val_c = entries[beg];
+      if (end - beg > 1) val_n = entries[beg + 1];
+    } else {
+      const uint2 e0 = entries[beg];
+      key_c = e0.y;
+      val_c = e0.x;
+      if (end - beg > 1) {
+        const uint2 e1 = entries[beg + 1];
+        key_n = e1.y;
+        val_n = e1.x;
+      }
     }
   }
   bool alive = end > beg;
@@ -208,7 +315,7 @@
   } while (0)
 #define MSM_GLDS_ISSUE(val, valid)                                \
   do {                                                            \
-    const int mine_ = (valid) ? (int)((((val) & IDX_MASK & MSM_ACC_IDX_AND)) << MSM_ACC_IDX_SHL) : 0; \
+    const int mine_ = (valid) ? (int)(((EF::index(val) & MSM_ACC_IDX_AND)) << MSM_ACC_IDX_SHL) : 0; \
     if constexpr (LANES == 1) {                                   \
       MSM_GLDS_ONE(0, 0x00);                                      \
       MSM_GLDS_ONE(1, 0x55);                                      \
@@ -259,18 +366,27 @@
       MSM_Q_POP(key_n, val_n);
       if (--q_left == 0) {
         if (add_now && end - e > 3) MSM_Q_REFILL(e + 3);
-        q_left = 2 * EQ;
+        q_left = QCAP;
       }
     } else if (add_now && end - e > 2) {
-      const uint2 e2 = entries[e + 2];
-      key_n = e2.y;
-      val_n = e2.x;
+      if constexpr (EF::WORD32) {
+        val_n = entries[e + 2];
+      } else {
+        const uint2 e2 = entries[e + 2];
+        key_n = e2.y;
+        val_n = e2.x;
+      }
     }
 #if MSM_ACC_PRIO == 2
     __builtin_amdgcn_s_setprio(0);
 #endif
     if (add_now) {
-      if (key != cur) {
+      bool new_run;
+      if constexpr (EF::WORD32)
+        new_run = k == 0 || e32_step(val) != 0;
+      else
+        new_run = key != cur;
+      if (new_run) {
         const bool lane_first = cur == KEY_NONE;
         if (cur != KEY_NONE) {
 #ifndef MSM_ACC_NO_FLUSH
@@ -278,18 +394,27 @@
 #endif
           first = false;
         }
-        cur = key;
+        if constexpr (EF::WORD32) {
+          const uint32_t step = e32_step(val);
+          cur = (lane_first || step == E32_ESCAPE) ? entries_arg.run_keys[e] : cur + step;
+        } else {
+          cur = key;
+        }
         fresh = true;
         G::begin_run(acc);
         if constexpr (G::CARRY_IN) {
-          if (out.carry_in && !(lane_first && t > 0 && entries[beg - 1].y == key)) carry_begin_run<G>(out, key, acc, fresh, half);
+          if constexpr (EF::WORD32) {
+            if (out.carry_in && !(lane_first && e32_step(val) == 0)) carry_begin_run<G>(out, cur, acc, fresh, half);
+          } else {
+            if (out.carry_in && !(lane_first && t > 0 && entries[beg - 1].y == key)) carry_begin_run<G>(out, key, acc, fresh, half);
+          }
         }
       }
 #if MSM_ACC_PRIO == 1
       __builtin_amdgcn_s_setprio(2);
 #endif
       if (G::madd_loaded(acc, p, (val >> 31) != 0, fresh, md)) {
-        const Base again = G::from_dev_lane(bases[val & IDX_MASK], half);
+        const Base again = G::from_dev_lane(bases[EF::index(val)], half);
         G::madd_same_x(acc, again, (val >> 31) != 0, md);
       }
 #if MSM_ACC_PRIO == 1
diff --git a/2022-entries_amd/csrc/msm_types.hpp b/2022-entries_amd/csrc/msm_types.hpp
--- a/2022-entries_amd/csrc/msm_types.hpp
+++ b/2022-entries_amd/csrc/msm_types.hpp
@@ -5,6 +5,23 @@
 
 constexpr uint32_t KEY_NONE = 0xffffffffu;
 constexpr uint32_t IDX_MASK = 0x7fffffffu;
+
+constexpr uint32_t E32_IDX_BITS = 26;
+constexpr uint32_t E32_IDX_MASK = (1u << E32_IDX_BITS) - 1;
+constexpr uint32_t E32_STEP_MASK = 31u;
+constexpr uint32_t E32_MAX_STEP = 30u;
+constexpr uint32_t E32_ESCAPE = 31u;
+MSM_HD uint32_t e32_pack(uint32_t value, uint32_t step) { return (value & (0x80000000u | E32_IDX_MASK)) | (step << E32_IDX_BITS); }
+MSM_HD uint32_t e32_step(uint32_t word) { return (word >> E32_IDX_BITS) & E32_STEP_MASK; }
+MSM_HD uint32_t e32_index(uint32_t word) { return word & E32_IDX_MASK; }
+MSM_HD uint32_t e32_step_of_gap(uint32_t gap, bool first_of_segment) { return (first_of_segment || gap > E32_MAX_STEP) ? E32_ESCAPE : gap; }
+MSM_HD uint32_t e32_next_key(uint32_t prev_key, uint32_t word, const uint32_t* run_keys, uint32_t pos) {
+  const uint32_t step = e32_step(word);
+  return step == E32_ESCAPE ? run_keys[pos] : prev_key + step;
+}
+MSM_HD uint32_t e32_run_keys_offset(uint64_t capacity) { return (uint32_t)((capacity + 16 + 15) & ~(uint64_t)15); }
+MSM_HD uint32_t e32_first_lane_start(uint32_t pos, uint32_t K) { return (pos + K - 1) / K * K; }
+MSM_HD bool e32_applies(uint64_t idx0, uint64_t n, uint32_t table_levels) { return table_levels <= 1 && n <= (1ull << E32_IDX_BITS) && idx0 + n <= (1ull << E32_IDX_BITS); }
 
 template <class T>
 struct alignas(128) AffineDevT {
diff --git a/2022-entries_amd/csrc/partition.hpp b/2022-entries_amd/csrc/partition.hpp
--- a/2022-entries_amd/csrc/partition.hpp
+++ b/2022-entries_amd/csrc/partition.hpp
@@ -5,6 +5,7 @@
 #include <algorithm>
 
 #include "digits.hpp"
+#include "msm_types.hpp"
 #include "partition_plan.hpp"
 
 namespace msm {
@@ -614,9 +615,12 @@
   uint32_t tmp[32];
 };
 
+template <bool E32>
 __device__ __forceinline__ void pass_scatter_tiles(PassLds& L, const uint2* __restrict__ in, uint2* __restrict__ out, uint32_t beg, uint32_t end,
-                                                   const PassPlan& pp, uint32_t key_base) {
+                                                   const PassPlan& pp, uint32_t key_base, const PassE32& e32 = PassE32{}, uint32_t my_step = 0) {
   const uint32_t nb = 1u << pp.rb, shift = pp.rem - pp.rb, keepmask = (1u << shift) - 1;
+  uint32_t* const out32 = reinterpret_cast<uint32_t*>(out);
+  uint32_t* const run_keys = out32 + e32.rk_off;
   constexpr int PER = PART_PTILE / 1024;
   uint2 nxt[PER];
 #pragma unroll
@@ -651,7 +655,17 @@
       const uint32_t ex = block_excl_scan<false>(v, L.tmp, tot);
       if (threadIdx.x < nb) {
         const uint32_t c0 = L.cur[threadIdx.x];
-        L.tstart[threadIdx.x] = ex;
+        if constexpr (E32) {
+          uint32_t ts = ex;
+          if (v) {
+            ts |= my_step << 16;
+            my_step = 0;
+            for (uint32_t q = e32_first_lane_start(c0, e32.lane_k); q - c0 < v; q += e32.lane_k) run_keys[q] = key_base + threadIdx.x;
+          }
+          L.tstart[threadIdx.x] = ts;
+        } else {
+          L.tstart[threadIdx.x] = ex;
+        }
 #ifdef PART_EXP_PS_ALIGNED
         L.dst[threadIdx.x] = (c0 & ~15u) - ex;
 #else
@@ -665,12 +679,19 @@
     lds_barrier();
 #pragma unroll
     for (int k = 0; k < PER; k++)
-      if (where[k] != 0xffffffffu) L.stage[L.tstart[where[k] >> 16] + (where[k] & 0xffffu)] = ent[k];
+      if (where[k] != 0xffffffffu) L.stage[(E32 ? L.tstart[where[k] >> 16] & 0xffffu : L.tstart[where[k] >> 16]) + (where[k] & 0xffffu)] = ent[k];
     lds_barrier();
     const uint32_t total = L.tstart[nb];
     for (uint32_t j = threadIdx.x; j < total; j += 1024) {
       uint2 e = L.stage[j];
       const uint32_t bin = e.y >> 16;
+      if constexpr (E32) {
+        const uint32_t ts = L.tstart[bin], pos = L.dst[bin] + j;
+        const uint32_t step = (ts & 0xffffu) == j ? ts >> 16 : 0u;
+        out32[pos] = e32_pack(e.x, step);
+        if (step == E32_ESCAPE) run_keys[pos] = key_base + bin;
+        continue;
+      }
       e.y = pp.last ? key_base + bin : (e.y & 0xffffu);
 #if defined(PART_EXP_PS_NOSTORE)
       if (e.x == 0x12345678u && e.y == 0x9abcu) out[0] = e;
@@ -685,10 +706,11 @@
   }
 }
 
+template <bool E32>
 __global__ void __launch_bounds__(1024, PART_PASS_OCC) k_pass_scatter(const uint2* __restrict__ in, const PartSeg* __restrict__ segs,
                                                           const uint32_t* __restrict__ subjob_first, PassPlan pp, uint32_t gen,
                                                           const uint32_t* __restrict__ positions, uint2* __restrict__ out,
-                                                          PartSeg* __restrict__ out_segs) {
+                                                          PartSeg* __restrict__ out_segs, PassE32 e32) {
   __shared__ PassLds L;
   const uint32_t nb = 1u << pp.rb, shift = pp.rem - pp.rb;
   if (blockIdx.x < gen) {
@@ -700,13 +722,15 @@
       const PartSeg sg = segs[seg];
       if (part_fused_takes(sg.len)) continue;
       const uint32_t* row = positions + (size_t)j * nb;
+      uint32_t my_step = 0;
       lds_barrier();
       for (uint32_t b = threadIdx.x; b < nb; b += 1024) {
         L.cur[b] = row[b];
         L.cnt[b] = 0;
+        if constexpr (E32) my_step = row[b] == positions[(size_t)subjob_first[seg] * nb + b] ? E32_ESCAPE : 0u;
       }
       lds_barrier();
-      pass_scatter_tiles(L, in, out, beg, end, pp, sg.key_base);
+      pass_scatter_tiles<E32>(L, in, out, beg, end, pp, sg.key_base, e32, my_step);
     }
     return;
   }
@@ -720,6 +744,7 @@
   }
   const uint32_t beg = sg.start, end = sg.start + sg.len;
   for (uint32_t b = threadIdx.x; b < nb; b += 1024) L.cnt[b] = 0;
+  uint32_t my_step = 0;
   lds_barrier();
   {
     uint32_t e = beg + threadIdx.x;
@@ -742,9 +767,27 @@
       L.cnt[threadIdx.x] = 0;
       if (out_segs) out_segs[(size_t)s * nb + threadIdx.x] = PartSeg{beg + ex, v, sg.key_base + (threadIdx.x << shift), 0};
     }
+    if constexpr (E32) {
+      const uint64_t m = __builtin_amdgcn_ballot_w64(v != 0);
+      const uint32_t wv = threadIdx.x >> 6, ln = threadIdx.x & 63;
+      if (ln == 0) {
+        L.tmp[2 * wv] = (uint32_t)m;
+        L.tmp[2 * wv + 1] = (uint32_t)(m >> 32);
+      }
+      lds_barrier();
+      if (v) {
+        const uint64_t below = m & ((1ull << ln) - 1);
+        int prev = below ? (int)(wv * 64 + 63 - __clzll((long long)below)) : -1;
+        for (int u = (int)wv - 1; u >= 0 && prev < 0; u--) {
+          const uint64_t mu = (uint64_t)L.tmp[2 * u] | ((uint64_t)L.tmp[2 * u + 1] << 32);
+          if (mu) prev = u * 64 + 63 - __clzll((long long)mu);
+        }
+        my_step = e32_step_of_gap(threadIdx.x - (uint32_t)prev, prev < 0);
+      }
+    }
   }
   lds_barrier();
-  pass_scatter_tiles(L, in, out, beg, end, pp, sg.key_base);
+  pass_scatter_tiles<E32>(L, in, out, beg, end, pp, sg.key_base, e32, my_step);
 }
 
 }
@@ -807,6 +850,56 @@
     if (e.y >= key_limit) atomicAdd(&dbg[DBG_KEY_RANGE], 1u);
     const uint32_t idx = e.x & 0x7fffffffu;
     if (idx < idx_lo || idx >= idx_hi) atomicAdd(&dbg[DBG_VALUE_RANGE], 1u);
+  }
+}
+
+__global__ void __launch_bounds__(256) k_dbg_check_sorted_e32(const uint32_t* __restrict__ words, const uint32_t* __restrict__ run_keys, uint32_t K,
+                                                              const uint32_t* __restrict__ totals, uint32_t key_limit, uint32_t idx_lo, uint32_t idx_hi,
+                                                              uint32_t* __restrict__ dbg) {
+  const uint32_t n = totals[0];
+  for (uint64_t beg = ((uint64_t)blockIdx.x * 256 + threadIdx.x) * K; beg < n; beg += (uint64_t)gridDim.x * 256 * K) {
+    const uint32_t end = (uint32_t)(beg + K < n ? beg + K : n);
+    uint32_t key = run_keys[beg];
+    if (key >= key_limit) atomicAdd(&dbg[DBG_KEY_RANGE], 1u);
+    for (uint32_t i = (uint32_t)beg; i < end; i++) {
+      const uint32_t w = words[i];
+      if (i > beg) {
+        const uint32_t next = e32_next_key(key, w, run_keys, i);
+        if (next < key || (next == key) != (e32_step(w) == 0)) atomicAdd(&dbg[DBG_UNSORTED], 1u);
+        if (next >= key_limit) atomicAdd(&dbg[DBG_KEY_RANGE], 1u);
+        key = next;
+      }
+      const uint32_t idx = e32_index(w);
+      if (idx < idx_lo || idx >= idx_hi) atomicAdd(&dbg[DBG_VALUE_RANGE], 1u);
+    }
+    if (end < n) {
+      const uint32_t w = words[end], stored = run_keys[end];
+      const uint32_t step = e32_step(w);
+      const bool ok = step == 0 ? stored == key : (stored > key && (step == E32_ESCAPE || stored == key + step));
+      if (!ok) atomicAdd(&dbg[DBG_UNSORTED], 1u);
+    }
+  }
+}
+
+__global__ void k_dbg_corrupt_e32(uint32_t* __restrict__ words, uint32_t* __restrict__ run_keys, const uint32_t* __restrict__ totals) {
+  const uint32_t n = totals[0];
+  if (n < 2) return;
+  uint32_t key = run_keys[0];
+  for (uint32_t i = 0; i + 1 < n; i++) {
+    const uint32_t next = e32_next_key(key, words[i + 1], run_keys, i + 1);
+    if (next != key) {
+      if (i + 2 < n) {
+        const uint32_t after = e32_next_key(next, words[i + 2], run_keys, i + 2);
+        words[i + 2] = e32_pack(words[i + 2], E32_ESCAPE);
+        run_keys[i + 2] = after;
+      }
+      words[i] = e32_pack(words[i], E32_ESCAPE);
+      run_keys[i] = next;
+      words[i + 1] = e32_pack(words[i + 1], E32_ESCAPE);
+      run_keys[i + 1] = key;
+      return;
+    }
+    key = next;
   }
 }
 
@@ -912,8 +1005,12 @@
       hipLaunchKernelGGL(k_pass_scan, dim3(pp.nsegs), dim3(1024), 0, st, b.segs[seg_cur], b.subjob_first, pp, b.counts, out_segs);
       PART_MARK("pass_scan");
     }
-    hipLaunchKernelGGL(k_pass_scatter, dim3(gen + pp.nsegs), dim3(1024), 0, st, b.entries[cur], b.segs[seg_cur], b.subjob_first, pp, gen, b.counts,
-                       b.entries[cur ^ 1], out_segs);
+    if (pp.last && b.e32_lane_k)
+      hipLaunchKernelGGL(k_pass_scatter<true>, dim3(gen + pp.nsegs), dim3(1024), 0, st, b.entries[cur], b.segs[seg_cur], b.subjob_first, pp, gen, b.counts,
+                         b.entries[cur ^ 1], out_segs, PassE32{b.e32_lane_k, e32_run_keys_offset(entries)});
+    else
+      hipLaunchKernelGGL(k_pass_scatter<false>, dim3(gen + pp.nsegs), dim3(1024), 0, st, b.entries[cur], b.segs[seg_cur], b.subjob_first, pp, gen, b.counts,
+                         b.entries[cur ^ 1], out_segs, PassE32{});
     PART_MARK("pass_scatter");
     cur ^= 1;
     rem -= rb[i];
@@ -928,8 +1025,15 @@
   {
     const uint32_t key_limit = p.bsets * p.half;
     const uint32_t idx_hi = p.idx0 + p.n + (p.levels - 1) * p.table_stride;
-    if (getenv("MI355_MSM_DEBUG_CORRUPT")) hipLaunchKernelGGL(k_dbg_corrupt, dim3(1), dim3(1), 0, st, b.entries[cur], b.totals);
-    hipLaunchKernelGGL(k_dbg_check_sorted, dim3(2048), dim3(256), 0, st, b.entries[cur], b.totals, key_limit, p.idx0, idx_hi, dbg);
+    if (b.e32_lane_k) {
+      uint32_t* const words = reinterpret_cast<uint32_t*>(b.entries[cur]);
+      uint32_t* const run_keys = words + e32_run_keys_offset(entries);
+      if (getenv("MI355_MSM_DEBUG_CORRUPT")) hipLaunchKernelGGL(k_dbg_corrupt_e32, dim3(1), dim3(1), 0, st, words, run_keys, b.totals);
+      hipLaunchKernelGGL(k_dbg_check_sorted_e32, dim3(2048), dim3(256), 0, st, words, run_keys, b.e32_lane_k, b.totals, key_limit, p.idx0, idx_hi, dbg);
+    } else {
+      if (getenv("MI355_MSM_DEBUG_CORRUPT")) hipLaunchKernelGGL(k_dbg_corrupt, dim3(1), dim3(1), 0, st, b.entries[cur], b.totals);
+      hipLaunchKernelGGL(k_dbg_check_sorted, dim3(2048), dim3(256), 0, st, b.entries[cur], b.totals, key_limit, p.idx0, idx_hi, dbg);
+    }
     if (p.fold)
       hipLaunchKernelGGL((k_dbg_count_digits<FR, MODE, true>), dim3(part_ceil_div(p.n, 256)), dim3(256), 0, st, d_scalars, d_inf, p, dbg);
     else
diff --git a/2022-entries_amd/csrc/partition_plan.hpp b/2022-entries_amd/csrc/partition_plan.hpp
--- a/2022-entries_amd/csrc/partition_plan.hpp
+++ b/2022-entries_amd/csrc/partition_plan.hpp
@@ -161,6 +161,11 @@
   uint32_t* counts;
   uint32_t* totals;
   uint32_t* wide_flag;
+  uint32_t e32_lane_k;
+};
+
+struct PassE32 {
+  uint32_t lane_k, rk_off;
 };
 
 
```

Result: faster. 681.3 million (median of 6 runs) (+2.1%).
